# argmaxinc/WhisperKit

Measured on AMD Instinct MI355X. Metric: audio-sec/sec (1/RTF), 30 s chunks: host PCM -> log-mel + encoder + greedy decode -> segments, higher is better.
Workload: dtype f16

## Files before the change

### include/whisperhip.h

```cpp
#ifndef WHISPERHIP_H
#define WHISPERHIP_H

#include <stddef.h>
#include <stdint.h>

#ifdef __cplusplus
extern "C" {
#endif

typedef struct wh_model wh_model;
typedef struct wh_session wh_session;
typedef struct wh_transcription wh_transcription;
typedef struct wh_tokenizer wh_tokenizer;

typedef enum wh_status {
    WH_OK = 0,
    WH_ERR_TOKENIZER_UNAVAILABLE = 1,
    WH_ERR_MODELS_UNAVAILABLE = 2,
    WH_ERR_PREFILL_FAILED = 3,
    WH_ERR_AUDIO_PROCESSING_FAILED = 4,
    WH_ERR_DECODING_LOGITS_FAILED = 5,
    WH_ERR_SEGMENTING_FAILED = 6,
    WH_ERR_LOAD_AUDIO_FAILED = 7,
    WH_ERR_PREPARE_DECODER_INPUTS_FAILED = 8,
// ... 88 lines not shown

typedef struct wh_word_timing {
    int32_t token_offset, n_tokens;
    float start, end, probability;
} wh_word_timing;

typedef struct wh_timings {
    double audio_processing, logmels, encoding, decoding_init, decoding_predictions, decoding_filtering,
        decoding_sampling, decoding_kv_caching, decoding_word_timestamps, decoding_fallback, decoding_windowing,
        decoding_loop, full_pipeline, input_audio_seconds;
    double total_decoding_loops, total_decoding_windows, total_decoding_fallbacks, total_encoding_runs,
        total_logmel_runs;
    double pipeline_start, first_token_time, model_loading, prewarm_load_time, encoder_load_time, decoder_load_time,
        encoder_specialization_time, decoder_specialization_time, tokenizer_load_time, audio_loading, decoding_non_prediction,
        total_audio_processing_runs, total_kv_update_runs, total_timestamp_alignment_runs;
} wh_timings;

const char* wh_last_error(void);
const char* wh_version(void);

int wh_model_create(const void* blob, size_t nbytes, int device, wh_model** out);
int wh_model_load(const char* path, int device, wh_model** out);
void wh_model_destroy(wh_model* m);
int wh_model_dims(const wh_model* m, wh_dims* out);
int wh_model_set_alignment_heads(wh_model* m, const int32_t* layer_head_pairs, int n_pairs);

int wh_mel_count(const wh_model* m);
int wh_window_samples(const wh_model* m);
int wh_embed_size(const wh_model* m);
int wh_logits_size(const wh_model* m);
int wh_kv_cache_embed_dim(const wh_model* m);
int wh_kv_cache_max_sequence_length(const wh_model* m);
int wh_window_size(const wh_model* m);
int wh_is_model_multilingual(const wh_model* m);
int wh_supports_word_timestamps(const wh_model* m);
int wh_special_tokens_default(const wh_model* m, wh_special_tokens* out);
void wh_decoding_options_default(wh_decoding_options* out);

int wh_session_create(wh_model* m, int max_batch , wh_session** out);
void wh_session_destroy(wh_session* s);
int wh_session_max_batch(const wh_session* s);
int wh_session_cross_attention_mode(const wh_session* s);
int wh_xabs_auto_min_slots(void);
int wh_xabs_auto_splits(int max_batch);
int wh_xabs_supports(int n_state, int n_head);
int wh_session_cross_attention_splits(const wh_session* s);
int wh_session_create_with_mode(wh_model* m, int max_batch, int cross_attention_mode, wh_session** out);
int wh_session_create_tuned(wh_model* m, int max_batch, int cross_attention_mode, int cross_attention_splits, wh_session** out);
typedef struct wh_session_options {
    int32_t cross_attention_mode;
    int32_t cross_attention_splits;
    int32_t cross_attention_slots_per_workgroup;
    int32_t encoder_precision;
    int32_t reserved_[3];
    int32_t fallback_compaction;
} wh_session_options;
void wh_session_options_default(wh_session_options* out);
int wh_session_create_with_options(wh_model* m, int max_batch, const wh_session_options* opt, wh_session** out);
int wh_session_cross_attention_slots_per_workgroup(const wh_session* s);
int wh_session_encoder_precision(const wh_session* s);
int wh_debug_peek(wh_session* s, const char* name, void* out_host, size_t nbytes);
long long wh_debug_live_allocations(void);
int wh_session_step_graph_count(const wh_session* s);
int wh_session_synchronize(wh_session* s);
void* wh_session_stream(wh_session* s);

int wh_set_audio(wh_session* s, int b, const float* pcm_host, int n_samples);
int wh_set_audio_device(wh_session* s, int b, const float* pcm_device, int n_samples);

int wh_log_mel_spectrogram(wh_session* s, int batch);
int wh_get_mel(wh_session* s, int b, float* out_host );
int wh_set_mel(wh_session* s, int b, const float* mel_host );

int wh_encode_features(wh_session* s, int batch);
int wh_get_encoder_output(wh_session* s, int b, float* out_host );
int wh_set_encoder_output(wh_session* s, int b, const float* enc_host );

int wh_prepare_decoder_inputs(wh_session* s, int batch);
int wh_reset_decoder_inputs(wh_session* s, int batch);

int wh_predict_logits(wh_session* s, int batch, const int32_t* tokens, const int32_t* positions,
                      float* logits_out_host );
int wh_get_alignment_weights(wh_session* s, int b, float* out_host );

int wh_session_set_alignment_postprocess(wh_session* s, int z_normalize, int median_filter_width);

int wh_session_set_word_alignment(wh_session* s, int mode);
int wh_session_word_alignment(const wh_session* s);
int wh_alignment_paths(wh_session* s, int batch, const int32_t* rows, int32_t* text_idx, int32_t* time_idx, int32_t* lengths,
                       int capacity_per_slot);
int wh_session_word_alignment_stats(const wh_session* s, int64_t* dtw_launches, int64_t* alignment_d2h_bytes);

enum { WH_DTYPE_F32 = 0, WH_DTYPE_F16 = 1 };
typedef struct wh_tensor {
    void* data;
    int32_t dtype;
    int32_t ndim;
    int64_t shape[4];
    int32_t device;
    int32_t reserved_;
} wh_tensor;
int wh_get_mel_tensor(wh_session* s, int b, wh_tensor* out);
int wh_get_encoder_output_tensor(wh_session* s, int b, int dtype, wh_tensor* out);
int wh_get_logits_tensor(wh_session* s, wh_tensor* out);
int wh_get_mel_device(wh_session* s, int b, const float** mel_dev);
int wh_get_encoder_output_device(wh_session* s, int b, const float** enc_f32_dev, const void** enc_f16_dev);
int wh_get_logits_device(wh_session* s, const float** logits_dev);
int wh_session_set_cancel_flag(wh_session* s, const volatile int32_t* flag);

int wh_filter_logits(wh_session* s, const wh_decoding_options* opt, const wh_special_tokens* st,
                     const int32_t* tokens, int n_tokens, int prefilled_index, int initial_prompt_index,
                     int language_filter, float* logits_inout_host, int n_logits);
int wh_sample_token(wh_session* s, const float* logits_host, int n_logits, float temperature, int top_k,
// ... 256 lines not shown
```

### whisperkit_amd/_lib.py

```python
from __future__ import annotations

import ctypes as C
import os

HERE = os.path.dirname(os.path.abspath(__file__))
LIB_PATH = os.environ.get("WHISPERHIP_LIB") or os.path.join(HERE, "libwhisperhip.so")

WH_MAX_RESULT_TOKENS = 232
WINDOW_SAMPLES = 480000
MEL_FRAMES = 3000
AUDIO_CTX = 1500
MAX_TOKEN_CONTEXT = 224


class WhDims(C.Structure):
    _fields_ = [(n, C.c_int32) for n in ("n_mels", "n_audio_ctx", "n_audio_state", "n_audio_head", "n_audio_layer",
                                           "n_vocab", "n_text_ctx", "n_text_state", "n_text_head", "n_text_layer")]


class WhSpecialTokens(C.Structure):
    _fields_ = [(n, C.c_int32) for n in ("end_token", "english_token", "no_speech_token", "no_timestamps_token",
                                           "special_token_begin", "start_of_previous_token", "start_of_transcript_token",
                                           "time_token_begin", "transcribe_token", "translate_token", "whitespace_token",
                                           "language_token_begin", "n_language_tokens")]


class WhDecodingOptions(C.Structure):
    _fields_ = [
        ("task", C.c_int32), ("language_token", C.c_int32), ("temperature", C.c_float),
        ("temperature_increment_on_fallback", C.c_float), ("temperature_fallback_count", C.c_int32),
        ("sample_length", C.c_int32), ("top_k", C.c_int32), ("use_prefill_prompt", C.c_int32),
        ("detect_language", C.c_int32), ("skip_special_tokens", C.c_int32), ("without_timestamps", C.c_int32),
        ("word_timestamps", C.c_int32), ("max_initial_timestamp", C.c_float), ("max_window_seek", C.c_int32),
        ("clip_timestamps", C.POINTER(C.c_float)), ("n_clip_timestamps", C.c_int32), ("window_clip_time", C.c_float),
        ("prompt_tokens", C.POINTER(C.c_int32)), ("n_prompt_tokens", C.c_int32),
        ("prefix_tokens", C.POINTER(C.c_int32)), ("n_prefix_tokens", C.c_int32),
        ("suppress_blank", C.c_int32), ("suppress_tokens", C.POINTER(C.c_int32)), ("n_suppress_tokens", C.c_int32),
        ("compression_ratio_threshold", C.c_float), ("log_prob_threshold", C.c_float),
        ("first_token_log_prob_threshold", C.c_float), ("no_speech_threshold", C.c_float), ("seed", C.c_uint64),
        ("float16_logits", C.c_int32), ("beam_size", C.c_int32), ("beam_patience", C.c_float), ("reserved_", C.c_int32),
    ]


class WhDecodingResult(C.Structure):
    _fields_ = [
        ("n_tokens", C.c_int32), ("tokens", C.c_int32 * WH_MAX_RESULT_TOKENS), ("token_logprobs", C.c_float * WH_MAX_RESULT_TOKENS),
        ("avg_logprob", C.c_float), ("no_speech_prob", C.c_float), ("temperature", C.c_float), ("compression_ratio", C.c_float),
        ("language_token", C.c_int32), ("fallback_reason", C.c_int32), ("needs_fallback", C.c_int32),
        ("is_first_token_logprob_too_low", C.c_int32), ("steps", C.c_int32),
    ]


class WhSessionOptions(C.Structure):
    _fields_ = [("cross_attention_mode", C.c_int32), ("cross_attention_splits", C.c_int32), ("cross_attention_slots_per_workgroup", C.c_int32),
                ("encoder_precision", C.c_int32), ("reserved_", C.c_int32 * 3), ("fallback_compaction", C.c_int32)]


class WhTensor(C.Structure):
    _fields_ = [("data", C.c_void_p), ("dtype", C.c_int32), ("ndim", C.c_int32), ("shape", C.c_int64 * 4), ("device", C.c_int32),
                ("reserved_", C.c_int32)]


class WhSegment(C.Structure):
    _fields_ = [("id", C.c_int32), ("seek", C.c_int32), ("start", C.c_float), ("end", C.c_float),
                ("token_offset", C.c_int32), ("n_tokens", C.c_int32), ("temperature", C.c_float), ("avg_logprob", C.c_float),
                ("compression_ratio", C.c_float), ("no_speech_prob", C.c_float), ("word_offset", C.c_int32), ("n_words", C.c_int32)]


class WhWordTiming(C.Structure):
    _fields_ = [("token_offset", C.c_int32), ("n_tokens", C.c_int32), ("start", C.c_float), ("end", C.c_float), ("probability", C.c_float)]


class WhProgress(C.Structure):
    _fields_ = [("slot", C.c_int32), ("n_tokens", C.c_int32), ("tokens", C.POINTER(C.c_int32)), ("avg_logprob", C.c_float),
                ("compression_ratio", C.c_float), ("text", C.c_char_p)]


PROGRESS_FN = C.CFUNCTYPE(C.c_int, C.c_void_p, C.POINTER(WhProgress))
WINDOW_PRE_FN = C.CFUNCTYPE(None, C.c_void_p, C.c_int, C.POINTER(C.c_float), C.c_int, C.c_int)
WINDOW_POST_FN = C.CFUNCTYPE(C.c_int, C.c_void_p, C.c_int, C.c_int, C.c_int, C.c_void_p, C.c_int, C.c_int)
SEGMENT_DISCOVERY_FN = C.CFUNCTYPE(None, C.c_void_p, C.c_int, C.c_void_p, C.c_int, C.c_int)


class WhWindowHooks(C.Structure):
    _fields_ = [("window_preprocess", WINDOW_PRE_FN), ("window_postprocess", WINDOW_POST_FN), ("segment_discovery", SEGMENT_DISCOVERY_FN),
                ("user", C.c_void_p)]
LOGITS_FILTER_FN = C.CFUNCTYPE(None, C.c_void_p, C.POINTER(C.c_float), C.c_int32, C.POINTER(C.c_int32), C.c_int32)
TOKEN_SAMPLER_FN = C.CFUNCTYPE(C.c_int32, C.c_void_p, C.POINTER(C.c_float), C.c_int32, C.POINTER(C.c_int32), C.POINTER(C.c_float), C.c_int32,
                               C.POINTER(C.c_int32), C.POINTER(C.c_float))


class WhChunkRecord(C.Structure):
    _fields_ = [("tokens", C.c_int32 * 232), ("n_tokens", C.c_int32), ("chunk_index", C.c_int32), ("seek", C.c_int32), ("steps", C.c_int32),
                ("avg_logprob", C.c_float), ("temperature", C.c_float), ("compression_ratio", C.c_float), ("no_speech_prob", C.c_float)]


COMM_RCCL, COMM_TCP, COMM_ID_BYTES = 0, 1, 128


class WhTimings(C.Structure):
    _fields_ = [(n, C.c_double) for n in (
        "audio_processing", "logmels", "encoding", "decoding_init", "decoding_predictions", "decoding_filtering",
        "decoding_sampling", "decoding_kv_caching", "decoding_word_timestamps", "decoding_fallback", "decoding_windowing",
        "decoding_loop", "full_pipeline", "input_audio_seconds", "total_decoding_loops", "total_decoding_windows",
        "total_decoding_fallbacks", "total_encoding_runs", "total_logmel_runs",
        "pipeline_start", "first_token_time", "model_loading", "prewarm_load_time", "encoder_load_time", "decoder_load_time",
        "encoder_specialization_time", "decoder_specialization_time", "tokenizer_load_time", "audio_loading",
        "decoding_non_prediction", "total_audio_processing_runs", "total_kv_update_runs", "total_timestamp_alignment_runs")]


VP, I, F, U64 = C.c_void_p, C.c_int, C.c_float, C.c_uint64
PF, PI32, PU8 = C.POINTER(C.c_float), C.POINTER(C.c_int32), C.POINTER(C.c_uint8)
PVP = C.POINTER(C.c_void_p)
POPT, PST = C.POINTER(WhDecodingOptions), C.POINTER(WhSpecialTokens)
SYMBOLS = {
    "wh_last_error": (C.c_char_p, []),
    "wh_version": (C.c_char_p, []),
    "wh_model_create": (I, [VP, C.c_size_t, I, PVP]),
    "wh_model_load": (I, [C.c_char_p, I, PVP]),
    "wh_model_destroy": (None, [VP]),
    "wh_model_dims": (I, [VP, C.POINTER(WhDims)]),
    "wh_model_set_alignment_heads": (I, [VP, PI32, I]),
    "wh_mel_count": (I, [VP]), "wh_window_samples": (I, [VP]), "wh_embed_size": (I, [VP]), "wh_logits_size": (I, [VP]),
    "wh_kv_cache_embed_dim": (I, [VP]), "wh_kv_cache_max_sequence_length": (I, [VP]), "wh_window_size": (I, [VP]),
    "wh_is_model_multilingual": (I, [VP]), "wh_supports_word_timestamps": (I, [VP]),
    "wh_special_tokens_default": (I, [VP, PST]),
    "wh_decoding_options_default": (None, [POPT]),
    "wh_session_create": (I, [VP, I, PVP]),
    "wh_session_destroy": (None, [VP]),
    "wh_session_max_batch": (I, [VP]),
    "wh_session_cross_attention_mode": (I, [VP]),
    "wh_session_cross_attention_splits": (I, [VP]),
    "wh_xabs_auto_min_slots": (I, []),
    "wh_xabs_auto_splits": (I, [I]),
    "wh_xabs_supports": (I, [I, I]),
    "wh_session_step_graph_count": (I, [VP]),
    "wh_session_set_window_hooks": (I, [VP, C.POINTER(WhWindowHooks)]),
    "wh_transcription_set_segment_times": (I, [VP, I, F, F]),
    "wh_session_create_with_mode": (I, [VP, I, I, PVP]),
    "wh_session_create_tuned": (I, [VP, I, I, I, PVP]),
    "wh_session_options_default": (None, [C.POINTER(WhSessionOptions)]),
    "wh_session_create_with_options": (I, [VP, I, C.POINTER(WhSessionOptions), PVP]),
    "wh_session_cross_attention_slots_per_workgroup": (I, [VP]),
    "wh_session_encoder_precision": (I, [VP]),
    "wh_debug_peek": (I, [VP, C.c_char_p, VP, C.c_size_t]),
    "wh_debug_live_allocations": (C.c_longlong, []),
    "wh_session_synchronize": (I, [VP]),
    "wh_session_stream": (VP, [VP]),
    "wh_set_audio": (I, [VP, I, VP, I]),
    "wh_set_audio_device": (I, [VP, I, VP, I]),
    "wh_log_mel_spectrogram": (I, [VP, I]),
    "wh_get_mel": (I, [VP, I, VP]),
    "wh_set_mel": (I, [VP, I, VP]),
    "wh_encode_features": (I, [VP, I]),
    "wh_get_encoder_output": (I, [VP, I, VP]),
    "wh_set_encoder_output": (I, [VP, I, VP]),
    "wh_prepare_decoder_inputs": (I, [VP, I]),
    "wh_reset_decoder_inputs": (I, [VP, I]),
    "wh_predict_logits": (I, [VP, I, PI32, PI32, VP]),
    "wh_get_alignment_weights": (I, [VP, I, VP]),
    "wh_filter_logits": (I, [VP, POPT, PST, PI32, I, I, I, I, VP, I]),
    "wh_sample_token": (I, [VP, VP, I, F, I, U64, I, PI32, PF]),
    "wh_decode_text": (I, [VP, I, POPT, PST, PI32, I, PF, PI32, U64, C.POINTER(WhDecodingResult)]),
    "wh_decode_text_languages": (I, [VP, I, POPT, PST, PI32, I, PI32, PF, PI32, U64, C.POINTER(WhDecodingResult)]),
    "wh_decode_text_custom": (I, [VP, POPT, PST, PI32, I, F, U64, C.POINTER(LOGITS_FILTER_FN), PVP, I, TOKEN_SAMPLER_FN, VP,
                                  C.POINTER(WhDecodingResult)]),
    "wh_detect_language": (I, [VP, I, PST, PI32, PF]),
    "wh_decode_text_beam": (I, [VP, I, I, F, POPT, PST, PI32, I, PI32, C.POINTER(WhDecodingResult)]),
    "wh_beam_sampler_create": (I, [I, C.c_int32, F, PVP]),
    "wh_beam_sampler_destroy": (None, [VP]),
    "wh_beam_sampler_reset": (None, [VP]),
    "wh_beam_sampler_max_candidates": (I, [VP]),
    "wh_beam_sampler_finished_count": (I, [VP]),
    "wh_beam_sampler_update": (I, [VP, I, I, PI32, PF, PF, PF, PI32, I, PI32, PF, PF, PI32, PI32, PI32]),
    "wh_beam_sampler_finalize": (I, [VP, I, I, PI32, PF, PF, I, I, PI32, PF, PI32, PF, PI32]),
    "wh_get_mel_device": (I, [VP, I, PVP]),
    "wh_get_mel_tensor": (I, [VP, I, C.POINTER(WhTensor)]),
    "wh_get_encoder_output_tensor": (I, [VP, I, I, C.POINTER(WhTensor)]),
    "wh_get_logits_tensor": (I, [VP, C.POINTER(WhTensor)]),
    "wh_get_encoder_output_device": (I, [VP, I, PVP, PVP]),
    "wh_get_logits_device": (I, [VP, PVP]),
    "wh_session_set_cancel_flag": (I, [VP, VP]),
    "wh_session_set_alignment_postprocess": (I, [VP, I, I]),
    "wh_session_set_fallback_compaction": (I, [VP, I]),
# ... 136 lines not shown
```

### whisperkit_amd/api.py

```python
from __future__ import annotations

import ctypes as C
import dataclasses
import math
import weakref
from typing import List, Optional, Sequence, Tuple, Union

import numpy as np

from . import _lib as L
from .weights import MODEL_DIMS, WhisperDims, pack_blob, synthetic_state_dict


class WhisperError(RuntimeError):

    def __init__(self, code: int, message: str):
        super().__init__(f"[wh_status {code}] {message}")
        self.code = code


def _check(code: int):
    if code != 0:
        raise WhisperError(code, L.load().wh_last_error().decode())

# ... 342 lines not shown
        if blob is None:
            blob = pack_blob(dims, state_dict, alignment_heads=alignment_heads)
        self.handle = C.c_void_p()
        arr = np.frombuffer(blob, dtype=np.uint8)
        _check(self.lib.wh_model_create(C.c_void_p(arr.ctypes.data), arr.nbytes, device, C.byref(self.handle)))
        st = L.WhSpecialTokens()
        _check(self.lib.wh_special_tokens_default(self.handle, C.byref(st)))
        self.specialTokens = st

    @classmethod
    def from_pretrained(cls, src: str, device: int = 0):
        from .checkpoint import load_checkpoint
        dims, sd, heads = load_checkpoint(src)
        return cls(dims, sd, device=device, alignment_heads=heads)

    @classmethod
    def synthetic(cls, name: str, seed: int = 0, device: int = 0, **kw):
        dims = MODEL_DIMS[name]
        return cls(dims, synthetic_state_dict(dims, seed=seed, **kw), device=device)

    melCount = property(lambda s: s.lib.wh_mel_count(s.handle))
    windowSamples = property(lambda s: s.lib.wh_window_samples(s.handle))
    embedSize = property(lambda s: s.lib.wh_embed_size(s.handle))
    logitsSize = property(lambda s: s.lib.wh_logits_size(s.handle))
    kvCacheEmbedDim = property(lambda s: s.lib.wh_kv_cache_embed_dim(s.handle))
    kvCacheMaxSequenceLength = property(lambda s: s.lib.wh_kv_cache_max_sequence_length(s.handle))
    windowSize = property(lambda s: s.lib.wh_window_size(s.handle))
    isModelMultilingual = property(lambda s: bool(s.lib.wh_is_model_multilingual(s.handle)))
    supportsWordTimestamps = property(lambda s: bool(s.lib.wh_supports_word_timestamps(s.handle)))

    def setAlignmentHeads(self, pairs):
        a = np.ascontiguousarray(np.array(list(pairs), dtype=np.int32).reshape(-1))
        _check(self.lib.wh_model_set_alignment_heads(self.handle, a.ctypes.data_as(L.PI32), len(a) // 2))

    def close(self):
        if self.handle:
            self.lib.wh_model_destroy(self.handle)
            self.handle = C.c_void_p()

    def __del__(self):
        try:
            self.close()
        except Exception:
            pass


def xabsSupports(nState: int, nHead: int) -> bool:
    return bool(L.load().wh_xabs_supports(int(nState), int(nHead)))


class Session:

    ENCODER_PRECISIONS = {None: 0, "f16": 0, "split": 1}

    def __init__(self, model: Model, maxBatch: int = 1, crossAttentionMode: Optional[int] = None, crossAttentionSplits: Optional[int] = None,
                 crossAttentionSlotsPerWorkgroup: Optional[int] = None, encoderPrecision: Optional[str] = None):
        self.model, self.lib, self.B = model, model.lib, maxBatch
        self.handle = C.c_void_p()
        if encoderPrecision not in self.ENCODER_PRECISIONS:
            raise ValueError(f"encoderPrecision {encoderPrecision!r}: expected None, 'f16' or 'split'")
        if crossAttentionSlotsPerWorkgroup is not None or encoderPrecision is not None:
            o = L.WhSessionOptions()
            self.lib.wh_session_options_default(C.byref(o))
            o.cross_attention_mode = -1 if crossAttentionMode is None else int(crossAttentionMode)
            o.cross_attention_splits = 0 if crossAttentionSplits is None else int(crossAttentionSplits)
            o.cross_attention_slots_per_workgroup = int(crossAttentionSlotsPerWorkgroup or 0)
            o.encoder_precision = self.ENCODER_PRECISIONS[encoderPrecision]
            _check(self.lib.wh_session_create_with_options(model.handle, maxBatch, C.byref(o), C.byref(self.handle)))
        elif crossAttentionMode is None and crossAttentionSplits is None:
            _check(self.lib.wh_session_create(model.handle, maxBatch, C.byref(self.handle)))
        else:
            _check(self.lib.wh_session_create_tuned(model.handle, maxBatch, -1 if crossAttentionMode is None else int(crossAttentionMode),
                                                    int(crossAttentionSplits or 0), C.byref(self.handle)))

    @staticmethod
    def xabsAutoMinSlots() -> int:
        return int(L.load().wh_xabs_auto_min_slots())

    @staticmethod
    def xabsAutoSplits(maxBatch: int) -> int:
        return int(L.load().wh_xabs_auto_splits(int(maxBatch)))

    @staticmethod
    def xabsSupports(nState: int, nHead: int) -> bool:
        return xabsSupports(nState, nHead)

    @property
    def crossAttentionSlotsPerWorkgroup(self) -> int:
        return int(self.lib.wh_session_cross_attention_slots_per_workgroup(self.handle))

    @property
    def encoderPrecision(self) -> str:
        return {0: "f16", 1: "split"}[int(self.lib.wh_session_encoder_precision(self.handle))]

    @property
    def crossAttentionMode(self) -> int:
        return int(self.lib.wh_session_cross_attention_mode(self.handle))

    @property
    def crossAttentionSplits(self) -> int:
        return int(self.lib.wh_session_cross_attention_splits(self.handle))

    @property
    def stepGraphCount(self) -> int:
        return int(self.lib.wh_session_step_graph_count(self.handle))

    def close(self):
        if self.handle:
            self.lib.wh_session_destroy(self.handle)
            self.handle = C.c_void_p()

    def __del__(self):
        try:
            self.close()
        except Exception:
            pass

    def synchronize(self):
        _check(self.lib.wh_session_synchronize(self.handle))

    def _stash(self, exc: BaseException):
        if getattr(self, "_callback_error", None) is None:
            self._callback_error = exc

    def _raise_pending(self):
        exc, self._callback_error = getattr(self, "_callback_error", None), None
        if exc is not None:
            raise exc

    def _guarded(self, fn, *args) -> int:
        self._callback_error = None
        rc = fn(*args)
        self._raise_pending()
        _check(rc)
        return rc

    def setTokenizer(self, tokenizer: Optional["Tokenizer"]):
        self.tokenizer = tokenizer
        _check(self.lib.wh_session_set_tokenizer(self.handle, tokenizer.handle if tokenizer is not None else None))

    def setProgressCallback(self, callback):
        if callback is None:
            self._progress = None
            _check(self.lib.wh_session_set_progress_callback(self.handle, L.PROGRESS_FN(0), None))
            return

# ... 896 lines not shown
```

### whisperkit_amd/csrc/capi.hip

```cpp
#include <math.h>
#include <stdarg.h>
#include <stdio.h>
#include <string.h>

#include <algorithm>
#include <cstdlib>

#include "internal.h"
#include "knobs.h"

using namespace wh;

namespace wh { thread_local KernelProfiler* g_prof = nullptr; unsigned long long* debug_buffer(); }

namespace whi {
static thread_local char g_err[512] = "";
int set_error(int code, const char* fmt, ...) {
    va_list ap;
    va_start(ap, fmt);
    vsnprintf(g_err, sizeof(g_err), fmt, ap);
    va_end(ap);
    return code;
}
}
// ... 325 lines not shown
    o->end_token = eot; o->english_token = lang0; o->no_speech_token = translate + 4; o->no_timestamps_token = translate + 5;
    o->special_token_begin = eot; o->start_of_previous_token = translate + 3; o->start_of_transcript_token = sot;
    o->time_token_begin = translate + 6; o->transcribe_token = translate + 1; o->translate_token = translate; o->whitespace_token = 220;
    o->language_token_begin = lang0; o->n_language_tokens = nlang;
    return WH_OK;
}

extern "C" void wh_decoding_options_default(wh_decoding_options* o) {
    if (!o) return;
    memset(o, 0, sizeof(*o));
    o->task = 0; o->language_token = -1; o->temperature = 0.0f; o->temperature_increment_on_fallback = 0.2f;
    o->temperature_fallback_count = 5; o->sample_length = WH_MAX_TOKEN_CONTEXT; o->top_k = 5; o->use_prefill_prompt = 1;
    o->detect_language = -1; o->skip_special_tokens = 0; o->without_timestamps = 0; o->word_timestamps = 0;
    o->max_initial_timestamp = NAN; o->max_window_seek = -1; o->clip_timestamps = nullptr; o->n_clip_timestamps = 0;
    o->window_clip_time = 1.0f; o->prompt_tokens = nullptr; o->n_prompt_tokens = 0; o->prefix_tokens = nullptr; o->n_prefix_tokens = 0;
    o->suppress_blank = 0; o->suppress_tokens = nullptr; o->n_suppress_tokens = 0;
    o->compression_ratio_threshold = 2.4f; o->log_prob_threshold = -1.0f; o->first_token_log_prob_threshold = -1.5f;
    o->no_speech_threshold = 0.6f; o->seed = 0; o->float16_logits = 0; o->beam_size = 0; o->beam_patience = 1.0f;
}

#define DALLOC(ptr, n) WH_HIP(s->mem.alloc(&(ptr), (size_t)(n), true))

static int session_create_impl(wh_model* m, int max_batch, int cross_attention_mode, int cross_attention_splits, int slots_per_workgroup, wh_session** out,
                               int encoder_precision = 0);
extern "C" int wh_session_create(wh_model* m, int max_batch, wh_session** out) { return session_create_impl(m, max_batch, -1, 0, 0, out); }
extern "C" int wh_session_create_tuned(wh_model* m, int max_batch, int cross_attention_mode, int cross_attention_splits, wh_session** out) {
    wh_session_options o{};
    o.cross_attention_mode = cross_attention_mode; o.cross_attention_splits = cross_attention_splits;
    return wh_session_create_with_options(m, max_batch, &o, out);
}
extern "C" void wh_session_options_default(wh_session_options* o) {
    if (!o) return;
    memset(o, 0, sizeof(*o));
    o->cross_attention_mode = -1;
}
extern "C" int wh_session_create_with_options(wh_model* m, int max_batch, const wh_session_options* opt, wh_session** out) {
    wh_session_options dflt;
    wh_session_options_default(&dflt);
    if (!opt) opt = &dflt;
    const int cross_attention_mode = opt->cross_attention_mode, cross_attention_splits = opt->cross_attention_splits;
    if (opt->cross_attention_slots_per_workgroup < 0 || opt->cross_attention_slots_per_workgroup > kXabsMaxSlotsPerWorkgroup)
        return set_error(WH_ERR_INVALID_ARGUMENT, "wh_session_create: cross_attention_slots_per_workgroup %d (expected 0 auto, 1 .. %d)", opt->cross_attention_slots_per_workgroup, kXabsMaxSlotsPerWorkgroup);
    if (cross_attention_mode < -1 || cross_attention_mode > 1)
        return set_error(WH_ERR_INVALID_ARGUMENT, "wh_session_create: cross_attention_mode %d (expected -1 auto, 0 K / V rows, 1 absorbed)", cross_attention_mode);
    if (cross_attention_splits < 0 || cross_attention_splits > kXabsSplits)
        return set_error(WH_ERR_INVALID_ARGUMENT, "wh_session_create: cross_attention_splits %d (expected 0 auto, 1 .. %d)", cross_attention_splits, kXabsSplits);
    if (opt->encoder_precision < 0 || opt->encoder_precision > 1)
        return set_error(WH_ERR_INVALID_ARGUMENT, "wh_session_create: encoder_precision %d (expected 0 Float16 operands, 1 split hi | lo)", opt->encoder_precision);
    if (opt->encoder_precision == 1 && cross_attention_mode == 1)
        return set_error(WH_ERR_INVALID_ARGUMENT, "wh_session_create: encoder_precision 1 (split) needs the K / V-row cross-attention (cross_attention_mode -1 or 0): "
                         "the absorbed kernel streams the Float16 encoder output, and a hi | lo stream would double its bytes");
    if (opt->fallback_compaction < 0 || opt->fallback_compaction > 1)
        return set_error(WH_ERR_INVALID_ARGUMENT, "wh_session_create: fallback_compaction %d (expected 0 off, 1 on)", opt->fallback_compaction);
    if (cross_attention_mode == 1 && m && !xabs_supported(m->dims.n_text_state, m->dims.n_text_head))
        return set_error(WH_ERR_INVALID_ARGUMENT, "wh_session_create: the absorbed cross-attention needs a model width of 384 / 512 / 768 / 1024 / 1280 (this model: %d)", m->dims.n_text_state);
    const int r = session_create_impl(m, max_batch, opt->encoder_precision == 1 ? 0 : cross_attention_mode, cross_attention_splits,
                                      opt->cross_attention_slots_per_workgroup, out, opt->encoder_precision);
    if (r == WH_OK) (*out)->fallback_compaction = opt->fallback_compaction;
    return r;
}
extern "C" int wh_session_create_with_mode(wh_model* m, int max_batch, int cross_attention_mode, wh_session** out) {
    return wh_session_create_tuned(m, max_batch, cross_attention_mode, 0, out);
}

static hipError_t create_session_stream(hipStream_t* st) {
    static std::atomic<int> counter{0};
    const int parts = knob::now<knob::WH_CU_PARTS>();
    if (const char* pr = knob::text<knob::WH_STREAM_PRIORITIES>()) {
        int p[8], n = 0;
        for (const char* c = pr; *c && n < 8;) { p[n++] = atoi(c); while (*c && *c != ',') ++c; if (*c == ',') ++c; }
        if (n > 0) return hipStreamCreateWithPriority(st, hipStreamNonBlocking, p[counter.fetch_add(1) % n]);
    }
    if (parts < 2) return hipStreamCreateWithFlags(st, hipStreamNonBlocking);
    int dev = 0, n_cu = 256;
    (void)hipGetDevice(&dev);
    (void)hipDeviceGetAttribute(&n_cu, hipDeviceAttributeMultiprocessorCount, dev);
    const int extra = knob::now<knob::WH_CU_PART_EXTRA>(), k = counter.fetch_add(1) % parts, w = n_cu / parts;
    uint32_t mask[16] = {};
    for (int i = k * w; i < k * w + w + extra; ++i) { const int c = ((i % n_cu) + n_cu) % n_cu; mask[c >> 5] |= 1u << (c & 31); }
    return hipExtStreamCreateWithCUMask(st, (uint32_t)((n_cu + 31) / 32), mask);
}
static int session_build(wh_session* s, wh_model* m, int max_batch, int cross_attention_mode, int cross_attention_splits, int slots_per_workgroup, int encoder_precision) {
    s->B = max_batch;
    const wh_dims& D = m->dims;
    const size_t B = max_batch, d = D.n_audio_state, L = D.n_text_layer, V = D.n_vocab, H = D.n_text_head;
    if (create_session_stream(&s->st) != hipSuccess) return set_error(WH_ERR_HIP, "hipStreamCreate failed");
    s->m = m;
    m->n_sessions.fetch_add(1);
    DALLOC(s->pcm, B * kWindowSamples); DALLOC(s->n_valid, B);
    DALLOC(s->logspec, B * D.n_mels * kFrames); DALLOC(s->maxkey, B);
    DALLOC(s->mel_t, B * kFramesPad * D.n_mels); DALLOC(s->mel_f32, B * D.n_mels * kFrames);
    DALLOC(s->h1, B * kFramesPad * d); DALLOC(s->x, B * kCtx * d); DALLOC(s->xn, B * kCtx * d);
    DALLOC(s->q16, B * kCtx * d); DALLOC(s->k16, B * kCtx * d); DALLOC(s->vt16, B * d * kCtxPad); DALLOC(s->att16, B * kCtx * d);
    DALLOC(s->hmlp, B * kCtx * 4 * d); DALLOC(s->enc16, B * kCtx * d); DALLOC(s->enc32, B * kCtx * d);
    s->encoder_precision = encoder_precision;
    if (encoder_precision == 1) {
        DALLOC(s->mel_t_lo, B * kFramesPad * D.n_mels); DALLOC(s->h1_lo, B * kFramesPad * d); DALLOC(s->xn_lo, B * kCtx * d);
        DALLOC(s->att_lo, B * kCtx * d); DALLOC(s->hmlp_lo, B * kCtx * 4 * d); DALLOC(s->enc_lo, B * kCtx * d);
    }
    {
        const int xabs_mode = knob::now<knob::WH_XABS>();
        if (cross_attention_mode >= 0) s->use_xabs = cross_attention_mode != 0 && xabs_supported((int)d, (int)H);
        else {
            s->use_xabs = xabs_auto_width((int)d, (int)H) && (xabs_mode < 0 ? max_batch >= wh_xabs_auto_min_slots() : xabs_mode != 0);
        }
        if (s->use_xabs) { const int r_ = build_xabs(m); if (r_) return r_; }
    }
    if (s->use_xabs) {
        Xabs probe{};
        const size_t bytes = mem::carve_session_xabs(nullptr, d, H, B, probe);
        char* blob = nullptr;
// ... 2 lines not shown
        s->xabs.layers_host = m->xabs.data();
        s->xabs.n_split = cross_attention_splits > 0 ? cross_attention_splits : xabs_splits(max_batch);
        s->xabs.spw = slots_per_workgroup > 0 ? slots_per_workgroup : 1;
        if (const int v = knob::now<knob::WH_XABS_SPW>()) s->xabs.spw = v;
    } else {
        DALLOC(s->cross_k_hi, L * B * kCtx * d); DALLOC(s->cross_v_hi, L * B * kCtx * d);
        DALLOC(s->cross_k_lo, L * B * kCtx * d); DALLOC(s->cross_v_lo, L * B * kCtx * d);
    }
    DALLOC(s->self_k, L * B * kMaxTok * d); DALLOC(s->self_v, L * B * kMaxTok * d);
    DALLOC(s->part, B * H * kMaxSplit * kPartStride); DALLOC(s->ticket, B * H);
    DALLOC(s->logits, B * V);
    DALLOC(s->align_mean, B * kMaxTok * kCtx);
    DALLOC(s->seq, B); DALLOC(s->cfg_dev, kMaxOptionClasses); DALLOC(s->suppress_dev, kMaxOptionClasses * kMaxSuppress); DALLOC(s->sup_mask_dev, kMaxOptionClasses * (size_t)plan::option_mask_stride((int)V)); DALLOC(s->stats, B * kStatBlocks * 8);
    DALLOC(s->tok_out_dev, B); DALLOC(s->lp_out_dev, B); DALLOC(s->scratch_logits, V);
    {
        Dec32& q = s->d32;
        Dec32 probe{};
        const size_t bytes = mem::carve_session_d32(nullptr, d, B, probe);
        char* blob = nullptr;
        if (s->mem.alloc(&blob, bytes, true) != hipSuccess) return set_error(WH_ERR_HIP, "hipMalloc(%zu) for the decode-step buffers failed", bytes);
        mem::carve_session_d32(blob, d, B, q);
        q.layers_host = m->dec32.data(); q.emb_t = m->emb_t; q.lg_g = m->lg_g; q.lg_c = m->lg_c; q.n_bt = (int)((B + 31) / 32);
        q.part_floats = kD32PartFloats;
    }
    if (s->mem.alloc_pinned(&s->seq_host, B) != hipSuccess) return set_error(WH_ERR_HIP, "hipHostMalloc failed");
    for (auto& e : s->ev) hipEventCreate(&e);
    (void)wh::debug_buffer();
    if (hipDeviceSynchronize() != hipSuccess) return set_error(WH_ERR_HIP, "hipDeviceSynchronize failed after session allocation");
    return WH_OK;
}
static int session_create_impl(wh_model* m, int max_batch, int cross_attention_mode, int cross_attention_splits, int slots_per_workgroup, wh_session** out,
                               int encoder_precision) {
    if (!m || !out) return set_error(WH_ERR_MODELS_UNAVAILABLE, "wh_session_create: model is null");
    if (max_batch < 1 || max_batch > kMaxSessionSlots) return set_error(WH_ERR_INVALID_ARGUMENT, "max_batch %d out of range [1, %d]", max_batch, kMaxSessionSlots);
    WH_HIP(hipSetDevice(m->device));
    wh_session* s = new wh_session();
    const int r = session_build(s, m, max_batch, cross_attention_mode, cross_attention_splits, slots_per_workgroup, encoder_precision);
    if (r) { wh_session_destroy(s); return r; }
    *out = s;
    return WH_OK;
}

extern "C" void wh_session_destroy(wh_session* s) {
    if (!s) return;
    if (s->m) s->m->n_sessions.fetch_sub(1);
    if (s->st) hipStreamSynchronize(s->st);
    whi::drop_session_graphs(s);
    for (auto& e : s->ev) if (e) hipEventDestroy(e);
    if (s->st) hipStreamDestroy(s->st);
    delete s;
}
extern "C" int wh_session_max_batch(const wh_session* s) { return s ? s->B : -1; }
extern "C" int wh_session_cross_attention_mode(const wh_session* s) { return s ? (s->use_xabs ? 1 : 0) : -1; }
extern "C" int wh_session_encoder_precision(const wh_session* s) { return s ? s->encoder_precision : -1; }
extern "C" int wh_session_step_graph_count(const wh_session* s) { return s ? (int)s->graphs.size() : -1; }
extern "C" int wh_session_cross_attention_splits(const wh_session* s) { return s ? (s->use_xabs ? s->xabs.n_split : 0) : -1; }
extern "C" int wh_session_cross_attention_slots_per_workgroup(const wh_session* s) { return s ? (s->use_xabs ? s->xabs.spw : 0) : -1; }
extern "C" int wh_xabs_auto_splits(int max_batch) { return wh::xabs_auto_splits(max_batch); }
extern "C" int wh_xabs_supports(int n_state, int n_head) { return wh::xabs_supported(n_state, n_head) ? 1 : 0; }
extern "C" int wh_xabs_auto_min_slots(void) { return knob::now<knob::WH_XABS_MIN_SLOTS>(); }
static_assert(knob::kTable[knob::WH_XABS_MIN_SLOTS].dflt == wh::kXabsAutoMinSlots && knob::kTable[knob::WH_XABS_SPW].hi == wh::kXabsMaxSlotsPerWorkgroup &&
              knob::kTable[knob::WH_XABS_SPLITS].hi == wh::kXabsSplits, "knobs.h: the ranges of the absorbed cross-attention knobs");
extern "C" int wh_debug_peek(wh_session* s, const char* name, void* out, size_t nbytes) {
    CHECK_SESSION(s);
    if (!name || !out) return set_error(WH_ERR_INVALID_ARGUMENT, "wh_debug_peek: null argument");
    const std::string n(name);
    const void* src = nullptr;
    size_t have = 0;
    const size_t R = (size_t)s->d32.n_bt * 32, d = (size_t)s->m->dims.n_text_state, H = (size_t)s->m->dims.n_text_head, B = (size_t)s->B;
    const size_t nht = H > 16 ? 2 : 1;
    if (n == "x") { src = s->d32.x; have = R * d * 4; } else if (n == "q") { src = s->d32.q; have = R * d * 4; }
    else if (n == "za_hi") { src = s->d32.za_hi; have = R * d * 2; } else if (n == "za_lo") { src = s->d32.za_lo; have = R * d * 2; }
    else if (n == "zb_hi") { src = s->d32.zb_hi; have = R * d * 2; } else if (n == "zb_lo") { src = s->d32.zb_lo; have = R * d * 2; }
    else if (s->use_xabs && n == "qf_hi") { src = s->xabs.qf_hi; have = B * nht * 16 * d * 2; }
    else if (s->use_xabs && n == "qf_lo") { src = s->xabs.qf_lo; have = B * nht * 16 * d * 2; }
    else if (s->use_xabs && n == "part") { src = s->xabs.part; have = (size_t)kXabsSplits * H * d * B * 4; }
    else if (s->use_xabs && n == "ml") { src = s->xabs.ml; have = (size_t)kXabsSplits * H * B * 8; }
    else if (n == "enc16") { src = s->enc16; have = B * kCtx * d * 2; }
    else if (s->enc_lo && n == "enc_lo") { src = s->enc_lo; have = B * kCtx * (size_t)s->m->dims.n_audio_state * 2; }
    if (!src) return set_error(WH_ERR_INVALID_ARGUMENT, "wh_debug_peek: no buffer named '%s' in this session", name);
    if (nbytes > have) return set_error(WH_ERR_INVALID_ARGUMENT, "wh_debug_peek: '%s' holds %zu bytes, %zu requested", name, have, nbytes);
    WH_HIP(hipStreamSynchronize(s->st));
    WH_HIP(hipMemcpy(out, src, nbytes, hipMemcpyDeviceToHost));
    return WH_OK;
}
extern "C" long long wh_debug_live_allocations(void) { return wh::mem::g_live.load(std::memory_order_relaxed); }
extern "C" int wh_session_synchronize(wh_session* s) {
    if (!s) return set_error(WH_ERR_INVALID_ARGUMENT, "session is null");
    WH_HIP(hipStreamSynchronize(s->st));
    return WH_OK;
}
extern "C" void* wh_session_stream(wh_session* s) { return s ? (void*)s->st : nullptr; }


static int set_audio_common(wh_session* s, int b, const float* pcm, int n, hipMemcpyKind kind) {
    CHECK_SESSION(s); CHECK_SLOT(s, b);
    if (n < 0 || (!pcm && n > 0)) return set_error(WH_ERR_AUDIO_PROCESSING_FAILED, "wh_set_audio: invalid buffer (n=%d)", n);
    int m = std::min(n, kWindowSamples);
    float* dst = s->pcm + (size_t)b * kWindowSamples;
    if (m > 0) WH_HIP(hipMemcpyAsync(dst, pcm, sizeof(float) * m, kind, s->st));
    if (m < kWindowSamples) WH_HIP(hipMemsetAsync(dst + m, 0, sizeof(float) * (kWindowSamples - m), s->st));
    WH_HIP(hipMemcpyAsync(s->n_valid + b, &m, sizeof(int), hipMemcpyHostToDevice, s->st));
    WH_HIP(hipStreamSynchronize(s->st));
    return WH_OK;
}
extern "C" int wh_set_audio(wh_session* s, int b, const float* pcm_host, int n) { return set_audio_common(s, b, pcm_host, n, hipMemcpyHostToDevice); }
// ... 98 lines not shown
        g = GemmArgs{};
        g.A = s->att16; g.W = w.o_w; g.bias = w.o_b; g.M = M; g.N = d; g.K = d; g.lda = d; g.a_rows_per_batch = M; g.ldc = d; g.out32 = s->x;
        g.prof_kind = KK_ENC_O;
        launch_gemm(EPI_RESID_F32, g, st);
        launch_layernorm(s->x, w.ln2_g, w.ln2_b, M, d, s->xn, nullptr, st);
        g = GemmArgs{};
        g.A = s->xn; g.W = w.fc1_w; g.bias = w.fc1_b; g.M = M; g.N = 4 * d; g.K = d; g.lda = d; g.a_rows_per_batch = M; g.ldc = 4 * d; g.out16 = s->hmlp;
        g.prof_kind = KK_ENC_FC1;
        launch_gemm(EPI_GELU_F16, g, st);
        g = GemmArgs{};
        g.A = s->hmlp; g.W = w.fc2_w; g.bias = w.fc2_b; g.M = M; g.N = d; g.K = 4 * d; g.lda = 4 * d; g.a_rows_per_batch = M; g.ldc = d; g.out32 = s->x;
        g.prof_kind = KK_ENC_FC2;
        launch_gemm(EPI_RESID_F32, g, st);
    }
    launch_layernorm(s->x, m->lnp_g, m->lnp_b, M, d, s->enc16, s->enc32, st);
    WH_CHECK_LAUNCH();
    return WH_OK;
}
extern "C" int wh_get_encoder_output(wh_session* s, int b, float* out) {
    CHECK_SESSION(s); CHECK_SLOT(s, b);
    if (!out) return set_error(WH_ERR_INVALID_ARGUMENT, "wh_get_encoder_output: null output");
    size_t n = (size_t)kCtx * s->m->dims.n_audio_state;
    WH_HIP(hipMemcpyAsync(out, s->enc32 + b * n, n * 4, hipMemcpyDeviceToHost, s->st));
    WH_HIP(hipStreamSynchronize(s->st));
    return WH_OK;
}
extern "C" int wh_set_encoder_output(wh_session* s, int b, const float* enc) {
    CHECK_SESSION(s); CHECK_SLOT(s, b);
    if (!enc) return set_error(WH_ERR_INVALID_ARGUMENT, "wh_set_encoder_output: null input");
    size_t n = (size_t)kCtx * s->m->dims.n_audio_state;
    WH_HIP(hipMemcpyAsync(s->enc32 + b * n, enc, n * 4, hipMemcpyHostToDevice, s->st));
    if (s->enc_lo) launch_f32_to_f16_split(s->enc32 + b * n, s->enc16 + b * n, s->enc_lo + b * n, n, s->st);
    else launch_f32_to_f16(s->enc32 + b * n, s->enc16 + b * n, n, s->st);
    WH_CHECK_LAUNCH();
    WH_HIP(hipStreamSynchronize(s->st));
    return WH_OK;
}

constexpr bool kXattnGateDefault = false;
namespace whi {
DecodeBuffers decode_buffers(wh_session* s, int batch, int max_position) {
    const wh_model* m = s->m;
    DecodeBuffers db{};
    db.cross_div = 1;
    db.self_rows = std::min(std::max(max_position, 0), kMaxTok - 1) + 1;
    db.self_owner = nullptr;
    db.batch = batch; db.max_batch = s->B; db.d = m->dims.n_text_state; db.n_head = m->dims.n_text_head; db.n_layer = m->dims.n_text_layer; db.n_vocab = m->dims.n_vocab;
    db.emb = m->emb; db.pos = m->dec_pos; db.layers_host = m->dec.data(); db.lnf_g = m->lnf_g; db.lnf_b = m->lnf_b;
    db.self_k = s->self_k; db.self_v = s->self_v; db.cross_k_hi = s->cross_k_hi; db.cross_v_hi = s->cross_v_hi; db.cross_k_lo = s->cross_k_lo; db.cross_v_lo = s->cross_v_lo;
    db.part = s->part; db.ticket = s->ticket; db.logits = s->logits; db.seq = s->seq;
    db.mixed = s->pass_mixed ? 1 : 0; db.stats = s->stats; db.sup_mask = s->sup_mask_dev; db.fused_greedy = s->fused_greedy ? 1 : 0;
    db.align = s->align_enabled ? s->align : nullptr; db.align_slot = m->align_slot_dev; db.n_align = s->n_align_alloc;
    db.d32 = &s->d32; db.x = s->d32.x; db.q = s->d32.q;
    if (s->use_xabs) { s->xabs.enc = s->enc16; db.xabs = &s->xabs; }
    if (s->pass_mapped) {
        db.slot_home = s->slot_home_dev;
        if (s->use_xabs) { s->xabs_pass = s->xabs; s->xabs_pass.spw = s->pass_spw; db.xabs = &s->xabs_pass; }
    }
    if (s->pass_owner) { db.self_owner = s->inpass_dev + s->B; db.owner_slots = s->B; }
    const int gate_mode = knob::once<knob::WH_XATT_GATE>();
    const bool gate_on = gate_mode < 0 ? kXattnGateDefault && m->n_sessions.load() > 1 : gate_mode != 0;
    db.xattn_gate = gate_on ? m->xattn_gate : nullptr;
    return db;
}
}

namespace whi {
int ensure_align(wh_session* s) {
    if (s->align && s->n_align_alloc != s->m->n_align) {
        WH_HIP(hipStreamSynchronize(s->st));
        drop_session_graphs(s);
        s->mem.release(s->align);
        s->align = nullptr;
        s->n_align_alloc = 0;
    }
    if (!s->align && s->m->n_align > 0) {
        size_t n = (size_t)s->B * kMaxTok * s->m->n_align * kCtx;
        WH_HIP(s->mem.alloc(&s->align, n, false));
        WH_HIP(hipMemsetAsync(s->align, 0, n * sizeof(float), s->st));
        s->n_align_alloc = s->m->n_align;
    }
    return WH_OK;
}

int reset_decoder_inputs_masked(wh_session* s, int batch, const int32_t* active) {
    for (int b = 0; b < batch; ++b) {
        if (active && !active[b]) continue;
        WH_HIP(hipMemsetAsync(s->seq + b, 0, sizeof(SeqState), s->st));
        if (s->align) WH_HIP(hipMemsetAsync(s->align + (size_t)b * kMaxTok * s->n_align_alloc * kCtx, 0, (size_t)kMaxTok * s->n_align_alloc * kCtx * sizeof(float), s->st));
    }
    return WH_OK;
}
}
using whi::ensure_align;

extern "C" int wh_reset_decoder_inputs(wh_session* s, int batch) {
    CHECK_SESSION(s); CHECK_BATCH(s, batch);
    return whi::reset_decoder_inputs_masked(s, batch, nullptr);
}

extern "C" int wh_prepare_decoder_inputs(wh_session* s, int batch) {
    CHECK_SESSION(s); CHECK_BATCH(s, batch);
    const wh_model* m = s->m;
    const int d = m->dims.n_text_state, L = m->dims.n_text_layer;
    if (!s->use_xabs) {
        GemmArgs g{};
// ... 370 lines not shown
```

### whisperkit_amd/csrc/decoder.hip

```cpp
#include <algorithm>
#include <cstdlib>

#include "dec_shared.h"
#include "knobs.h"

namespace wh {

__device__ __forceinline__ void compute_filter_rules(const SamplerCfg& cfg, const SeqState* sq, int n_tok, int V, int* r, int last_ts_hint = -2) {
    const int tb = cfg.time_token_begin;
    int blank = 0, ts_active = 0, r1lo = 0, r1hi = 0, r2lo = 0, r2hi = 0;
    blank = cfg.suppress_blank && (n_tok == cfg.prefilled_index);
    if (cfg.timestamp_rules) {
        int sb = -1;
        if (cfg.is_multilingual) {
            for (int i = 0; i < 3 && i < n_tok; ++i)
                if (sq->tokens[i] == cfg.transcribe_token || sq->tokens[i] == cfg.translate_token) { sb = max(i + 1, cfg.initial_prompt_index); break; }
        } else sb = cfg.initial_prompt_index;
        if (sb >= 0 && sb <= n_tok) {
            ts_active = 1;
            if (n_tok > sb) {
                int cnt = n_tok - sb;
                bool lastTs = sq->tokens[n_tok - 1] >= tb;
                bool penTs = cnt < 2 || sq->tokens[n_tok - 2] >= tb;
                if (lastTs) {
// ... 658 lines not shown
    const int nofence = knob::once<knob::WH_XATT_NOFENCE>();
    AttnArgs at = at_in;
    at.no_fence = nofence;
    ProfScope ps_(KK_DEC_CROSS_ATTN, st);
    const dim3 grid(S, H, B);
    const int gate_lead = knob::once<knob::WH_XATT_GATE_LEAD>();
    at.gate_wg = std::max(0, S * H * B - 1 - gate_lead);
    const int xlds = knob::once<knob::WH_XATT_LDS>();
    const int nt = knob::once<knob::WH_XATT_NT>();
    const bool ntl = nt && at.cross_div <= 1;
#define XATT(P_) do { if (at.mapped) { if (nt) dec_cross_attn_kernel<P_, true, true><<<grid, 256, xlds, st>>>(at); else dec_cross_attn_kernel<P_, false, true><<<grid, 256, xlds, st>>>(at); } \
                      else if (ntl) dec_cross_attn_kernel<P_, true><<<grid, 256, xlds, st>>>(at); else dec_cross_attn_kernel<P_, false><<<grid, 256, xlds, st>>>(at); } while (0)
    if (S == 6) XATT(8);
    else if (S == 8) XATT(6);
    else if (S == 12) XATT(4);
    else XATT(2);
#undef XATT
}

void launch_decoder_step(const DecodeBuffers& db, const SamplerCfg* cfg_dev, const int* suppress_dev, bool sample, hipStream_t st) {
    const Dec32& D = *db.d32;
    const int d = db.d, B = db.batch, H = db.n_head, L = db.n_layer, V = db.n_vocab;
    const int n_bt = (B + 31) / 32;
    const size_t self_stride = (size_t)db.max_batch * H * kMaxTok * kHeadDim;
    const size_t cross_stride = (size_t)db.max_batch * H * kCtx * kHeadDim;
    const int S = plan::cross_attn_plan(H, knob::once<knob::WH_XATT_PASSES>(), kCtx).splits;
    launch_dec32_embed(db.emb, db.pos, db.seq, B, d, V, n_bt, D.x, db.layers_host[0].ln1_g, D.za_hi, D.za_lo, D.stat, st);
    P32Args base{};
    base.batch = B; base.d = d; base.n_head = H; base.n_vocab = V; base.seq = db.seq; base.part = D.part; base.ticket = D.ticket;
    base.x = D.x; base.stat_in = D.stat; base.n_stat = d / 32;
    for (int l = 0; l < L; ++l) {
        const DecLayerW& w = db.layers_host[l];
        const Dec32LayerW& t = D.layers_host[l];
        P32Args a = base;
        a.N = 3 * d; a.K = d; a.Wt = t.qkv_t; a.zhi = D.za_hi; a.zlo = D.za_lo; a.fold_g = t.qkv_g; a.fold_c = t.qkv_c; a.q = D.q;
        a.self_k = db.self_k + (size_t)l * self_stride; a.self_v = db.self_v + (size_t)l * self_stride; a.prof_kind = KK_DEC_QKV;
        launch_dec32_proj(P32_QKV, a, n_bt, st);
        AttnArgs at{};
        at.batch = B; at.d = d; at.n_head = H; at.layer = l; at.n_layer = L; at.n_split = S; at.q = D.q; at.cross_div = db.cross_div;
        at.self_k = a.self_k; at.self_v = a.self_v;
        at.cross_k_hi = db.cross_k_hi + (size_t)l * cross_stride; at.cross_k_lo = db.cross_k_lo + (size_t)l * cross_stride;
        at.cross_v_hi = db.cross_v_hi + (size_t)l * cross_stride; at.cross_v_lo = db.cross_v_lo + (size_t)l * cross_stride;
        at.att_hi = D.zb_hi; at.att_lo = D.zb_lo; at.part = db.part; at.ticket = db.ticket; at.seq = db.seq;
        at.align = db.align; at.align_slot = db.align_slot; at.n_align = db.n_align; at.gate = db.xattn_gate;
        at.self_rows = db.self_rows; at.self_owner = db.self_owner;
        if (db.self_owner && db.owner_slots > B) {
            AttnArgs sa = at;
            sa.batch = db.owner_slots;
            launch_self_attn(sa, H, B, st);
        } else launch_self_attn(at, H, B, st);
        a = base;
        a.N = d; a.K = d; a.Wt = t.o_t; a.zhi = D.zb_hi; a.zlo = D.zb_lo; a.bias = w.o_b; a.gamma_next = w.ln2_g;
        a.zhi_out = D.za_hi; a.zlo_out = D.za_lo; a.stat_out = D.stat; a.prof_kind = KK_DEC_OPROJ;
        launch_dec32_proj(P32_RESID, a, n_bt, st);
        a = base;
        a.N = d; a.K = d; a.Wt = t.cq_t; a.zhi = D.za_hi; a.zlo = D.za_lo; a.fold_g = t.cq_g; a.fold_c = t.cq_c; a.q = D.q; a.prof_kind = KK_DEC_CQ;
        a.gate = db.xabs ? nullptr : db.xattn_gate;
        launch_dec32_proj(P32_Q, a, n_bt, st);
        if (db.xabs) {
            const Xabs& X = *db.xabs;
            XabsArgs xa{};
            xa.batch = B; xa.max_batch = db.max_batch; xa.d = d; xa.n_head = H; xa.layer = l; xa.n_split = X.n_split; xa.cross_div = db.cross_div;
            xa.enc = X.enc; xa.q = D.q; xa.wkT = X.layers_host[l].wkT; xa.wv_t = X.layers_host[l].wv_t; xa.bv = X.layers_host[l].bv;
            xa.qf_hi = X.qf_hi; xa.qf_lo = X.qf_lo; xa.part = X.part; xa.ml = X.ml; xa.att_hi = D.zb_hi; xa.att_lo = D.zb_lo;
            xa.align = db.align; xa.align_slot = db.align_slot; xa.n_align = db.n_align; xa.seq = db.seq; xa.kpart = D.part; xa.ticket = D.ticket;
            xa.gate = db.xattn_gate;
            xa.spw = X.spw;
            xa.dbg = debug_buffer() ? debug_buffer() + (size_t)KK_DEC_CROSS_ATTN * 4096 * 8 : nullptr;
            if (db.slot_home) { xa.mapped = 1; xa.slot_home = db.slot_home; }
            launch_xabs_qk(xa, n_bt, st);
            launch_xabs_attn(xa, st);
            launch_xabs_vup(xa, n_bt, st);
        } else {
            at.dbg = debug_buffer() ? debug_buffer() + (size_t)KK_DEC_CROSS_ATTN * 4096 * 8 : nullptr;
            if (db.slot_home) { at.mapped = 1; at.slot_home = db.slot_home; }
            launch_cross_attn(at, S, H, B, st);
        }
        a = base;
        a.N = d; a.K = d; a.Wt = t.co_t; a.zhi = D.zb_hi; a.zlo = D.zb_lo; a.bias = w.co_b; a.gamma_next = w.ln3_g;
        a.zhi_out = D.za_hi; a.zlo_out = D.za_lo; a.stat_out = D.stat; a.prof_kind = KK_DEC_COPROJ;
        launch_dec32_proj(P32_RESID, a, n_bt, st);
        a = base;
        a.N = 4 * d; a.K = d; a.Wt = t.fc1_t; a.zhi = D.za_hi; a.zlo = D.za_lo; a.fold_g = t.fc1_g; a.fold_c = t.fc1_c; a.h_out = D.h; a.h_out_lo = D.h_lo; a.prof_kind = KK_DEC_FC1;
        launch_dec32_proj(P32_FC1, a, n_bt, st);
        a = base;
        a.N = d; a.K = 4 * d; a.Wt = t.fc2_t; a.zhi = D.h; a.zlo = D.h_lo; a.bias = w.fc2_b;
        a.gamma_next = (l + 1 < L) ? db.layers_host[l + 1].ln1_g : db.lnf_g;
        a.zhi_out = D.za_hi; a.zlo_out = D.za_lo; a.stat_out = D.stat; a.prof_kind = KK_DEC_FC2;
        launch_dec32_proj(P32_RESID, a, n_bt, st);
    }
    const bool fused = sample && db.fused_greedy;
    P32Args a = base;
    a.N = V; a.K = d; a.Wt = D.emb_t; a.zhi = D.za_hi; a.zlo = D.za_lo; a.fold_g = D.lg_g; a.fold_c = D.lg_c;
    a.logits = fused ? nullptr : db.logits; a.prof_kind = KK_DEC_LOGITS;
    if (sample) a.cfg = cfg_dev;
    if (fused) { a.stats = db.stats; a.sup_mask = db.sup_mask; }
    const bool mixed = sample && db.mixed;
    launch_dec32_proj(P32_LOGITS, a, n_bt, st, mixed && fused);
    if (fused) {
        ProfScope ps_(KK_SAMPLER, st);
        if (mixed) sampler_final_mixed_kernel<<<B, 256, 0, st>>>(cfg_dev, db.seq, db.stats, (V + 31) / 32);
        else sampler_final_kernel<<<B, 256, 0, st>>>(cfg_dev, db.seq, db.stats, (V + 31) / 32);
    } else if (sample) {
        ProfScope ps_(KK_SAMPLER, st);
        if (mixed) sampler_kernel<1, 1, 2, 0><<<B, SAMP_T, 0, st>>>(cfg_dev, suppress_dev, db.seq, db.logits, 0, nullptr, nullptr);
        else sampler_kernel<1, 1, 1, 0><<<B, SAMP_T, 0, st>>>(cfg_dev, suppress_dev, db.seq, db.logits, 0, nullptr, nullptr);
    }
}

void launch_filter_only(const SamplerCfg* cfg_dev, const int* suppress_dev, SeqState* seq, float* logits, int n_vocab, hipStream_t st) {
    sampler_kernel<1, 0, 0, 1><<<1, SAMP_T, 0, st>>>(cfg_dev, suppress_dev, seq, logits, 0, nullptr, nullptr);
}
void launch_sample_only(const SamplerCfg* cfg_dev, SeqState* seq, float* logits, int n_vocab, int counter, int* token_out, float* logprob_out, hipStream_t st) {
    sampler_kernel<0, 1, 0, 0><<<1, SAMP_T, 0, st>>>(cfg_dev, nullptr, seq, logits, counter, token_out, logprob_out);
}


void launch_beam_filter_topk(const SamplerCfg* cfg_dev, const int* suppress_dev, SeqState* seq, float* logits, int batch, int K, float* lp_out,
                             int* tok_out, hipStream_t st) {
    sampler_kernel<1, 0, 0, 0, 1><<<batch, SAMP_T, 0, st>>>(cfg_dev, suppress_dev, seq, logits, K, tok_out, lp_out);
}

void launch_filter_sample(const SamplerCfg* cfg_dev, const int* suppress_dev, SeqState* seq, float* logits, int batch, int* token_out, float* logprob_out, hipStream_t st) {
    sampler_kernel<1, 1, 0, 0><<<batch, SAMP_T, 0, st>>>(cfg_dev, suppress_dev, seq, logits, 0, token_out, logprob_out);
}

__global__ __launch_bounds__(256) void alignment_mean_kernel(const float* __restrict__ align, int n_align, float* __restrict__ out) {
    __shared__ float acc[4][kCtx];
    const size_t row = blockIdx.x;
    const int lane = threadIdx.x & 63, wave = threadIdx.x >> 6;
    const float* src = align + row * n_align * kCtx;
    for (int t = lane; t < kCtx; t += 64) acc[wave][t] = 0.0f;
    for (int j = wave; j < n_align; j += 4) {
        const float* sp = src + (size_t)j * kCtx;
        float v[24];
        float mx = -INFINITY, amax = 0.0f;
#pragma unroll
        for (int i = 0; i < 24; ++i) {
            int t = lane + 64 * i;
            v[i] = t < kCtx ? sp[t] : -INFINITY;
            mx = fmaxf(mx, v[i]);
            if (t < kCtx) amax = fmaxf(amax, fabsf(v[i]));
// ... 115 lines not shown
```

### whisperkit_amd/csrc/decoder32.hip

```cpp
#include "dec_shared.h"
#include "knobs.h"

namespace wh {

typedef unsigned u32x4 __attribute__((ext_vector_type(4)));

__global__ void d32_tile_weights_kernel(const f16* __restrict__ W, int N, int K, u32x4* __restrict__ out, size_t n_out) {
    const size_t o = (size_t)blockIdx.x * blockDim.x + threadIdx.x;
    if (o >= n_out) return;
    const int KT = K >> 4;
    const int lane = (int)(o & 63);
    const size_t tile = o >> 6;
    const int kt = (int)(tile % KT), rt = (int)(tile / KT);
    const int row = rt * 32 + (lane & 31), k = kt * 16 + 8 * (lane >> 5);
    u32x4 v = {0, 0, 0, 0};
    if (row < N) v = *reinterpret_cast<const u32x4*>(W + (size_t)row * K + k);
    out[o] = v;
}
void dec32_tile_weights(const f16* W, int N, int K, f16* out, hipStream_t st) {
    const size_t n_out = (size_t)((N + 31) / 32) * (K / 16) * 64;
    d32_tile_weights_kernel<<<(unsigned)((n_out + 255) / 256), 256, 0, st>>>(W, N, K, reinterpret_cast<u32x4*>(out), n_out);
}

__global__ __launch_bounds__(256) void d32_fold_kernel(const f16* __restrict__ W, int N, int K, const float* __restrict__ gamma,
                                                       const float* __restrict__ beta, const float* __restrict__ bias,
                                                       float* __restrict__ g, float* __restrict__ c) {
    const int lane = threadIdx.x & 63, row = blockIdx.x * 4 + (threadIdx.x >> 6);
    if (row >= N) return;
    double sg = 0.0, sc = 0.0;
    for (int k = lane; k < K; k += 64) {
        const double w = (double)(float)W[(size_t)row * K + k];
        sg += w * (double)gamma[k];
        sc += w * (double)beta[k];
    }
#pragma unroll
    for (int o = 32; o > 0; o >>= 1) { sg += __shfl_xor(sg, o, 64); sc += __shfl_xor(sc, o, 64); }
    if (lane == 0) { g[row] = (float)sg; c[row] = (float)(sc + (bias ? (double)bias[row] : 0.0)); }
}
void dec32_fold_vectors(const f16* W, int N, int K, const float* gamma, const float* beta, const float* bias, float* g, float* c, hipStream_t st) {
    d32_fold_kernel<<<(N + 3) / 4, 256, 0, st>>>(W, N, K, gamma, beta, bias, g, c);
}

__device__ __forceinline__ void d32_resid_tail(const float (&xn)[4], bool valid, int bt, int rt, int n_rt, int n, int j, int gb, int tid,
                                               int d, float* x, const float* gamma_next, f16* zhi, f16* zlo, float2* stat_out,
                                               float (*xs)[33]) {
    const float4 gm = *reinterpret_cast<const float4*>(gamma_next + n);
    if (valid) {
        *reinterpret_cast<float4*>(x + (size_t)gb * d + n) = float4{xn[0], xn[1], xn[2], xn[3]};
        const float z[4] = {gm.x * xn[0], gm.y * xn[1], gm.z * xn[2], gm.w * xn[3]};
        f16x4 hi, lo;
#pragma unroll
        for (int i = 0; i < 4; ++i) { f16 h_, l_; split_hilo(z[i], h_, l_); hi[i] = h_; lo[i] = l_; }
        const size_t o = plane_index(gb, n, d);
        *reinterpret_cast<f16x4*>(zhi + o) = hi;
        *reinterpret_cast<f16x4*>(zlo + o) = lo;
    }
    const int nl = n & 31;
#pragma unroll
    for (int i = 0; i < 4; ++i) xs[nl + i][j] = xn[i];
    __syncthreads();
    if (tid < 32) {
        float s = 0.0f;
#pragma unroll
        for (int r = 0; r < 32; ++r) s += xs[r][tid];
        const float mean = s * (1.0f / 32.0f);
        float m2 = 0.0f;
#pragma unroll
        for (int r = 0; r < 32; ++r) { const float e = xs[r][tid] - mean; m2 = fmaf(e, e, m2); }
        stat_out[((size_t)bt * n_rt + rt) * 32 + tid] = float2{mean, m2};
    }
}

template <int K>
__device__ __forceinline__ void chan32_k(float& cm, float& cM2, float mb, float M2b) {
    constexpr float w = 1.0f / (float)(K + 1), w2 = 32.0f * (float)K / (float)(K + 1);
    const float delta = mb - cm;
    cm = fmaf(delta, w, cm);
    cM2 += fmaf(delta * delta, w2, M2b);
}
__device__ __forceinline__ void chan_merge(float& cn, float& cm, float& cM2, float nb, float mb, float M2b) {
    if (nb == 0.0f) return;
    const float nn = cn + nb, rn = __frcp_rn(nn);
    const float delta = mb - cm;
    cm = fmaf(delta, nb * rn, cm);
    cM2 += fmaf(delta * delta, cn * nb * rn, M2b);
    cn = nn;
}

template <int MODE, bool HILO, int TC, bool NTW, int RT>
__global__ __launch_bounds__(256, 2) void dec32_proj_kernel(const P32Args a) {
    constexpr bool kMix = MODE == P32_LOGITS_MIXED, kLogits = MODE == P32_LOGITS || kMix;
    constexpr bool kLN = MODE == P32_QKV || MODE == P32_Q || MODE == P32_FC1 || kLogits;
    constexpr int kXs = kLogits ? 256 * 6 : 32 * 33;
    __shared__ float red[RT][4][16][64];
    __shared__ float st_l[8][32][3];
    __shared__ float xs_raw[kXs];
    __shared__ int last_flag;
    const int tid = threadIdx.x, lane = tid & 63, wave = tid >> 6;
    const int n_rt = (a.N + 31) >> 5;
    const int n_rtp = (n_rt + RT - 1) / RT;
    const int grp8 = blockIdx.x / (8 * a.n_bt), in8 = blockIdx.x % (8 * a.n_bt);
    const int xw = grp8 * 8 + (in8 & 7), bt = in8 >> 3;
    if (xw >= n_rtp * a.ks) return;
    const int rt0 = (xw % n_rtp) * RT, ksi = xw / n_rtp;
    const int n_mine = min(RT, n_rt - rt0);
    const int KT = a.K >> 4;
    const int kt0 = (ksi * 4 + wave) * a.tw;
    const u32x4* wp[RT];
#pragma unroll
    for (int t = 0; t < RT; ++t) wp[t] = reinterpret_cast<const u32x4*>(a.Wt) + ((size_t)min(rt0 + t, n_rt - 1) * KT + kt0) * 64 + lane;
    const size_t zoff = ((size_t)bt * KT + kt0) * 64 + lane;
    const u32x4* hp = reinterpret_cast<const u32x4*>(a.zhi) + zoff;
    const u32x4* lp = HILO ? reinterpret_cast<const u32x4*>(a.zlo) + zoff : nullptr;
    const int j = tid & 31, sub = tid >> 5;
    const int gb = bt * 32 + j;
    const bool valid = gb < a.batch;
    const int xw_dbg = xw;

#define D32_STAMP(i) do { if (a.dbg && tid == 0 && bt == 0) a.dbg[(size_t)(xw_dbg & 4095) * 8 + (i)] = wall_clock64(); } while (0)
    D32_STAMP(0);
    float2 sp[5] = {};
    if constexpr (kLN) {
#pragma unroll
        for (int i = 0; i < 5; ++i) {
            const int idx = min(sub + 8 * i, a.n_stat - 1);
            sp[i] = a.stat_in[((size_t)bt * a.n_stat + idx) * 32 + j];
        }
    }
    constexpr bool kLateOperands = RT >= 4;
    constexpr int NB = RT >= 4 ? 3 : 2;
    float4 e0[RT], e1[RT];
    int pos_l = 0, live_l = 0;
    auto load_operands = [&]() {
#pragma unroll
        for (int t = 0; t < RT; ++t) {
            const int n = min(rt0 + t, n_rt - 1) * 32 + 4 * sub;
            if constexpr (kLN) {
                e0[t] = *reinterpret_cast<const float4*>(a.fold_g + n);
                e1[t] = *reinterpret_cast<const float4*>(a.fold_c + n);
            } else {
                e0[t] = *reinterpret_cast<const float4*>(a.bias + n);
                e1[t] = *reinterpret_cast<const float4*>(a.x + (size_t)gb * a.d + n);
            }
        }
    };
    if constexpr (!kLateOperands) load_operands();
    if (valid) { live_l = slot_live(a.seq + gb); if constexpr (MODE == P32_QKV) pos_l = a.seq[gb].token_index; }
    int rules[6] = {0, 0, 0, 0, 0, 0};
    unsigned masked4[RT];
    int tb = 0, ws_tok = 0, eot_tok = 0, nots_tok = 0, r16 = 0;
#pragma unroll
    for (int t = 0; t < RT; ++t) masked4[t] = 0xffffffffu;
    if constexpr (kLogits) {
        if (a.cfg) r16 = a.cfg->f16_logits;
        if (a.stats) {
            if (valid) {
#pragma unroll
                for (int i = 0; i < 6; ++i) rules[i] = a.seq[gb].f_rules[i];
            }
            const unsigned char* sup_mask = a.sup_mask;
            if constexpr (kMix) { if (valid) sup_mask += (size_t)seq_class(a.seq[gb].rng_lane) * plan::option_mask_stride(a.N); }
#pragma unroll
            for (int t = 0; t < RT; ++t) {
                const int n = min(rt0 + t, n_rt - 1) * 32 + 4 * sub;
                if (n + 3 < a.N) masked4[t] = *reinterpret_cast<const unsigned*>(sup_mask + n);
                else {
                    masked4[t] = 0;
#pragma unroll
                    for (int i = 0; i < 4; ++i) masked4[t] |= (unsigned)(n + i < a.N ? sup_mask[n + i] : 1) << (8 * i);
                }
            }
            tb = a.cfg->time_token_begin; ws_tok = a.cfg->whitespace_token; eot_tok = a.cfg->end_token; nots_tok = a.cfg->no_timestamps_token;
        }
    }

    f32x16 acc_h[RT], acc_l[RT];
#pragma unroll
    for (int t = 0; t < RT; ++t)
#pragma unroll
        for (int r = 0; r < 16; ++r) { acc_h[t][r] = 0.0f; acc_l[t][r] = 0.0f; }
    auto stats_to_lds = [&]() {
        if constexpr (kLN) {
            float cm = sp[0].x, cM2 = sp[0].y;
            const int mine = sub < a.n_stat ? (a.n_stat - sub + 7) >> 3 : 0;
            if (mine > 1) chan32_k<1>(cm, cM2, sp[1].x, sp[1].y);
            if (mine > 2) chan32_k<2>(cm, cM2, sp[2].x, sp[2].y);
            if (mine > 3) chan32_k<3>(cm, cM2, sp[3].x, sp[3].y);
            if (mine > 4) chan32_k<4>(cm, cM2, sp[4].x, sp[4].y);
            st_l[sub][j][0] = 32.0f * (float)mine; st_l[sub][j][1] = cm; st_l[sub][j][2] = cM2;
        }
    };
    {
        u32x4 w_[NB][RT][TC], h_[NB][TC], l_[NB][HILO ? TC : 1];
        auto ld = [&](u32x4 (&w)[RT][TC], u32x4 (&h)[TC], u32x4 (&l)[HILO ? TC : 1], int c) {
#pragma unroll
            for (int t = 0; t < RT; ++t)
#pragma unroll
                for (int i = 0; i < TC; ++i) w[t][i] = NTW ? __builtin_nontemporal_load(wp[t] + (size_t)(c * TC + i) * 64) : wp[t][(size_t)(c * TC + i) * 64];
#pragma unroll
            for (int i = 0; i < TC; ++i) h[i] = hp[(size_t)(c * TC + i) * 64];
            if constexpr (HILO) {
#pragma unroll
                for (int i = 0; i < TC; ++i) l[i] = lp[(size_t)(c * TC + i) * 64];
            }
        };
        auto mm = [&](const u32x4 (&w)[RT][TC], const u32x4 (&h)[TC], const u32x4 (&l)[HILO ? TC : 1]) {
#pragma unroll
            for (int i = 0; i < TC; ++i) {
#pragma unroll
                for (int t = 0; t < RT; ++t) {
                    const f16x8 wf = __builtin_bit_cast(f16x8, w[t][i]);
                    acc_h[t] = __builtin_amdgcn_mfma_f32_32x32x16_f16(wf, __builtin_bit_cast(f16x8, h[i]), acc_h[t], 0, 0, 0);
                    if constexpr (HILO) acc_l[t] = __builtin_amdgcn_mfma_f32_32x32x16_f16(wf, __builtin_bit_cast(f16x8, l[i]), acc_l[t], 0, 0, 0);
                }
            }
        };
        const int nch = a.tw / TC;
#pragma unroll
        for (int u = 0; u + 1 < NB; ++u)
            if (u < nch) ld(w_[u], h_[u], l_[u], u);
        D32_STAMP(1);
#pragma unroll 1
        for (int c = 0; c < nch; c += NB) {
#pragma unroll
            for (int u = 0; u < NB; ++u) {
                constexpr int kAhead = NB - 1;
                if (c + u + kAhead < nch) ld(w_[(u + kAhead) % NB], h_[(u + kAhead) % NB], l_[(u + kAhead) % NB], c + u + kAhead);
                __builtin_amdgcn_sched_barrier(0);
                if (c + u < nch) mm(w_[u], h_[u], l_[u]);
                if (u == 0 && c == 0) D32_STAMP(2);
            }
        }
    }
    if constexpr (kLateOperands) load_operands();
    stats_to_lds();
    D32_STAMP(3);
#pragma unroll
    for (int t = 0; t < RT; ++t)
#pragma unroll
        for (int r = 0; r < 16; ++r) red[t][wave][r][lane] = HILO ? fmaf(acc_l[t][r], 1.0f / 2048.0f, acc_h[t][r]) : acc_h[t][r];
    __syncthreads();
    D32_STAMP(4);
    float v[RT][4];
#pragma unroll
    for (int t = 0; t < RT; ++t)
#pragma unroll
        for (int i = 0; i < 4; ++i) v[t][i] = ((red[t][0][4 * wave + i][lane] + red[t][1][4 * wave + i][lane]) + red[t][2][4 * wave + i][lane]) + red[t][3][4 * wave + i][lane];

    if (a.ks > 1) {
        float* base = a.part + (((size_t)bt * n_rt + rt0) * a.ks) * 1024 + tid * 4;
#pragma unroll
        for (int t = 0; t < RT; ++t) {
            if (t < n_mine) {
                const f32x4 pv4 = {v[t][0], v[t][1], v[t][2], v[t][3]};
                float* mine = base + ((size_t)t * a.ks + ksi) * 1024;
                asm volatile("global_store_dwordx4 %0, %1, off sc1\n\ts_nop 1" ::"v"(mine), "v"(pv4) : "memory");
            }
        }
        asm volatile("s_waitcnt vmcnt(0)" ::: "memory");
        __syncthreads();
        if (tid == 0) {
            int* cnt = a.ticket + bt * n_rt + rt0;
            const int t = __hip_atomic_fetch_add(cnt, 1, __ATOMIC_RELAXED, __HIP_MEMORY_SCOPE_AGENT);
            const int last = (t == a.ks - 1);
            if (last) __hip_atomic_store(cnt, 0, __ATOMIC_RELAXED, __HIP_MEMORY_SCOPE_AGENT);
            last_flag = last;
        }
        __syncthreads();
        if (!last_flag) {
            if constexpr (MODE == P32_Q) { if (a.gate && blockIdx.x == 0 && tid == 0) xattn_gate_acquire(a.gate); }
            return;
        }
        float pv[RT][8][4];
#pragma unroll
        for (int t = 0; t < RT; ++t)
#pragma unroll
            for (int s = 0; s < 8; ++s) {
                const float* p = base + ((size_t)(t < n_mine ? t : 0) * a.ks + (s < a.ks ? s : 0)) * 1024;
#pragma unroll
                for (int i = 0; i < 4; ++i) pv[t][s][i] = __hip_atomic_load(p + i, __ATOMIC_RELAXED, __HIP_MEMORY_SCOPE_AGENT);
            }
#pragma unroll
        for (int t = 0; t < RT; ++t)
#pragma unroll
            for (int i = 0; i < 4; ++i) {
                float x_ = pv[t][0][i];
#pragma unroll
                for (int s = 1; s < 8; ++s) x_ += (s < a.ks) ? pv[t][s][i] : 0.0f;
                v[t][i] = x_;
            }
    }

    D32_STAMP(5);
    float mu = 0.0f, rstd = 0.0f;
    if constexpr (kLN) {
        float cn = 0.0f, cm = 0.0f, cM2 = 0.0f;
#pragma unroll
        for (int s = 0; s < 8; ++s) chan_merge(cn, cm, cM2, st_l[s][j][0], st_l[s][j][1], st_l[s][j][2]);
        mu = cm; rstd = rsqrtf(cM2 / (float)a.d + 1e-5f);
    }
#pragma unroll
  for (int t = 0; t < RT; ++t) {
    if (t >= n_mine) break;
    if constexpr (MODE == P32_RESID || kLogits) { if (t > 0) __syncthreads(); }
    const int rt = rt0 + t, n = rt * 32 + 4 * sub;
    float y[4];
    if constexpr (kLN) {
        const float g4[4] = {e0[t].x, e0[t].y, e0[t].z, e0[t].w}, c4[4] = {e1[t].x, e1[t].y, e1[t].z, e1[t].w};
#pragma unroll
        for (int i = 0; i < 4; ++i) y[i] = fmaf(rstd, v[t][i] - mu * g4[i], c4[i]);
    }
    if constexpr (MODE == P32_QKV) {
        if (valid && live_l) {
            const int d = a.d;
            if (n < d) *reinterpret_cast<float4*>(a.q + (size_t)gb * d + n) = float4{y[0], y[1], y[2], y[3]};
            else {
                int c = n - d;
                f16* dst = a.self_k;
                if (c >= d) { c -= d; dst = a.self_v; }
                const int pos = min(max(pos_l, 0), kMaxTok - 1);
                *reinterpret_cast<f16x4*>(dst + (((size_t)gb * a.n_head + (c >> 6)) * kMaxTok + pos) * kHeadDim + (c & 63)) =
                    f16x4{(f16)y[0], (f16)y[1], (f16)y[2], (f16)y[3]};
            }
        }
    } else if constexpr (MODE == P32_Q) {
        if (valid && live_l) *reinterpret_cast<float4*>(a.q + (size_t)gb * a.d + n) = float4{y[0], y[1], y[2], y[3]};
    } else if constexpr (MODE == P32_FC1) {
        if (valid) {
            f16x4 hi, lo;
#pragma unroll
            for (int i = 0; i < 4; ++i) { f16 h_, l_; split_hilo(gelu_erf(y[i]), h_, l_); hi[i] = h_; lo[i] = l_; }
            const size_t o = plane_index(gb, n, a.N);
            *reinterpret_cast<f16x4*>(a.h_out + o) = hi;
            *reinterpret_cast<f16x4*>(a.h_out_lo + o) = lo;
        }
    } else if constexpr (MODE == P32_RESID) {
        const float b4[4] = {e0[t].x, e0[t].y, e0[t].z, e0[t].w}, x4[4] = {e1[t].x, e1[t].y, e1[t].z, e1[t].w};
        float xn[4];
#pragma unroll
        for (int i = 0; i < 4; ++i) xn[i] = x4[i] + (v[t][i] + b4[i]);
        d32_resid_tail(xn, valid && live_l, bt, rt, n_rt, n, j, gb, tid, a.d, a.x, a.gamma_next, a.zhi_out, a.zlo_out, a.stat_out,
                       reinterpret_cast<float (*)[33]>(xs_raw));
    } else {
        if (r16) {
#pragma unroll
            for (int i = 0; i < 4; ++i) y[i] = (float)(f16)y[i];
        }
        if (a.logits && valid && live_l) {
            float* lo = a.logits + (size_t)gb * a.N + n;
            if (n + 3 < a.N) {
                *reinterpret_cast<float2*>(lo) = float2{y[0], y[1]};
                *reinterpret_cast<float2*>(lo + 2) = float2{y[2], y[3]};
            } else {
#pragma unroll
                for (int i = 0; i < 4; ++i) if (n + i < a.N) lo[i] = y[i];
            }
        }
        if (a.stats) {
            SoftStat t_{-INFINITY, 0.0f, 0x7fffffff}, u_{-INFINITY, 0.0f, 0x7fffffff};
            const int blank = rules[0], ts_active = rules[1];
#pragma unroll
            for (int i = 0; i < 4; ++i) {
                const int id = n + i;
                bool masked = ((masked4[t] >> (8 * i)) & 0xff) != 0 || id >= a.N;
                masked |= blank && (id == ws_tok || id == eot_tok);
                masked |= ts_active && (id == nots_tok || (id >= rules[2] && id < rules[3]) || (id >= rules[4] && id < rules[5]));
                if (!masked) { if (id < tb) stat_merge(t_, y[i], 1.0f, id); else stat_merge(u_, y[i], 1.0f, id); }
            }
            float* xr = xs_raw;
            float* rec = xr + (size_t)(sub * 32 + j) * 6;
            rec[0] = t_.m; rec[1] = t_.s; rec[2] = __int_as_float(t_.i); rec[3] = u_.m; rec[4] = u_.s; rec[5] = __int_as_float(u_.i);
            __syncthreads();
            if (tid < 32 && valid && live_l) {
                SoftStat T{-INFINITY, 0.0f, 0x7fffffff}, U{-INFINITY, 0.0f, 0x7fffffff};
#pragma unroll
                for (int s = 0; s < 8; ++s) {
                    const float* r_ = xr + (size_t)(s * 32 + tid) * 6;
                    stat_merge(T, r_[0], r_[1], __float_as_int(r_[2]));
                    stat_merge(U, r_[3], r_[4], __float_as_int(r_[5]));
                }
                float* o = a.stats + ((size_t)gb * kStatBlocks + rt) * 8;
                *reinterpret_cast<float4*>(o) = float4{T.m, T.s, __int_as_float(T.i), U.m};
                *reinterpret_cast<float2*>(o + 4) = float2{U.s, __int_as_float(U.i)};
            }
        }
    }
  }
    D32_STAMP(6);
    if constexpr (MODE == P32_Q) { if (a.gate && blockIdx.x == 0 && tid == 0) xattn_gate_acquire(a.gate); }
}


__global__ __launch_bounds__(256) void dec32_embed_kernel(const f16* __restrict__ emb, const float* __restrict__ pos, const SeqState* __restrict__ seq,
                                                          int batch, int d, int n_vocab, float* x, const float* gamma_next, f16* zhi, f16* zlo,
                                                          float2* stat_out) {
    __shared__ float xs[32][33];
    const int tid = threadIdx.x, j = tid & 31, sub = tid >> 5;
    const int rt = blockIdx.x, bt = blockIdx.y, n_rt = gridDim.x;
    const int n = rt * 32 + 4 * sub, gb = bt * 32 + j;
    const bool valid = gb < batch;
    float xn[4] = {0, 0, 0, 0};
    bool live = false;
    if (valid) {
        live = slot_live(seq + gb);
        const int tok = min(max(seq[gb].next_token, 0), n_vocab - 1);
        const int p = min(max(seq[gb].token_index, 0), kMaxTok - 1);
        const f16x4 e = *reinterpret_cast<const f16x4*>(emb + (size_t)tok * d + n);
        const float4 pz = *reinterpret_cast<const float4*>(pos + (size_t)p * d + n);
        xn[0] = (float)e[0] + pz.x; xn[1] = (float)e[1] + pz.y; xn[2] = (float)e[2] + pz.z; xn[3] = (float)e[3] + pz.w;
    }
    d32_resid_tail(xn, valid && live, bt, rt, n_rt, n, j, gb, tid, d, x, gamma_next, zhi, zlo, stat_out, xs);
}
void launch_dec32_embed(const f16* emb, const float* pos, const SeqState* seq, int batch, int d, int n_vocab, int n_bt, float* x,
                        const float* gamma_next, f16* zhi, f16* zlo, float2* stat, hipStream_t st) {
    ProfScope ps_(KK_DEC_EMBED, st);
    dec32_embed_kernel<<<dim3(d / 32, n_bt), 256, 0, st>>>(emb, pos, seq, batch, d, n_vocab, x, gamma_next, zhi, zlo, stat);
}

template <int MODE, bool HILO>
static void launch_planned(const P32Args& a, const plan::Dec32Plan& p, hipStream_t st) {
    const dim3 grid(p.grid);
#define D32_GO(TC_, RT_) do { \
        if (p.ntw) dec32_proj_kernel<MODE, HILO, TC_, true, RT_><<<grid, 256, 0, st>>>(a); \
        else dec32_proj_kernel<MODE, HILO, TC_, false, RT_><<<grid, 256, 0, st>>>(a); \
        return; } while (0)
    if constexpr (MODE != P32_LOGITS && MODE != P32_LOGITS_MIXED && MODE != P32_Q) {
        if (p.rt == 4) D32_GO(1, 4);
    }
    if (p.rt >= 2) {
        if (p.tc == 4) D32_GO(4, 2);
        if (p.tc == 2) D32_GO(2, 2);
        D32_GO(1, 2);
    }
    switch (p.tc) {
        case 5: D32_GO(5, 1);
        case 4: D32_GO(4, 1);
        case 3: D32_GO(3, 1);
        case 2: D32_GO(2, 1);
        default: D32_GO(1, 1);
    }
#undef D32_GO
}

unsigned long long* debug_buffer();
void launch_dec32_proj(int mode, const P32Args& a_in, int n_bt, hipStream_t st, bool mixed) {
    using namespace knob;
    P32Args a = a_in;
    a.dbg = (debug_buffer() && a.prof_kind >= 0) ? debug_buffer() + (size_t)a.prof_kind * 4096 * 8 : nullptr;
    const plan::Dec32Knobs k{once<WH_D32_KS_RESID>(), once<WH_D32_KS_FC2>(), once<WH_D32_KS_Q>(), once<WH_D32_KS_WIDE>(), once<WH_D32_TILE_KB>(), once<WH_D32_TC>(),
                             once<WH_D32_TC_BT>(), once<WH_D32_RT2_TC>(), once<WH_D32_NTW>(), once<WH_D32_RT_BT>(), once<WH_D32_RT4_BT>(), once<WH_D32_RT4_MODES>()};
    const plan::Dec32Plan p = plan::dec32_plan(mode, a.N, a.K, n_bt, k);
    a.ks = p.ks; a.tw = p.tw; a.rt = p.rt; a.n_bt = n_bt;
    ProfScope ps_(a.prof_kind, st);
    switch (mode) {
        case P32_QKV: launch_planned<P32_QKV, true>(a, p, st); break;
        case P32_Q: launch_planned<P32_Q, true>(a, p, st); break;
        case P32_FC1: launch_planned<P32_FC1, true>(a, p, st); break;
        case P32_LOGITS:
            if (mixed && a.stats && a.sup_mask) launch_planned<P32_LOGITS_MIXED, true>(a, p, st);
            else launch_planned<P32_LOGITS, true>(a, p, st);
            break;
        default:
            if (a.zlo != nullptr) launch_planned<P32_RESID, true>(a, p, st);
            else launch_planned<P32_RESID, false>(a, p, st);
    }
}

}
```

### whisperkit_amd/csrc/internal.h

```cpp
#pragma once
#include <map>
#include <new>
#include <stdexcept>
#include <string>
#include <tuple>
#include <unordered_map>
#include <vector>

#include "devmem.h"
#include "kernels.h"
#include "text.h"
#include "whisperhip.h"

struct HipMem {
    using Err = hipError_t;
    static constexpr Err ok = hipSuccess, out_of_memory = hipErrorOutOfMemory;
    static Err dev_malloc(void** p, size_t n) { return hipMalloc(p, n); }
    static Err dev_free(void* p) { return hipFree(p); }
    static Err host_malloc(void** p, size_t n) { return hipHostMalloc(p, n); }
    static Err host_free(void* p) { return hipHostFree(p); }
    static Err dev_memset(void* p, int v, size_t n) { return hipMemset(p, v, n); }
};
using DevMem = wh::mem::Owned<HipMem>;

// ... 56 lines not shown

struct wh_session {
    DevMem mem;
    wh_model* m = nullptr;
    int B = 0;
    hipStream_t st = nullptr;
    float* pcm = nullptr; int* n_valid = nullptr;
    float* logspec = nullptr; unsigned* maxkey = nullptr; f16* mel_t = nullptr; float* mel_f32 = nullptr;
    f16* h1 = nullptr; float* x = nullptr; f16* xn = nullptr; f16 *q16 = nullptr, *k16 = nullptr, *vt16 = nullptr, *att16 = nullptr;
    f16* hmlp = nullptr; f16* enc16 = nullptr; float* enc32 = nullptr;
    int encoder_precision = 0;
    f16 *mel_t_lo = nullptr, *h1_lo = nullptr, *xn_lo = nullptr, *att_lo = nullptr, *hmlp_lo = nullptr, *enc_lo = nullptr;
    f16 *cross_k_hi = nullptr, *cross_v_hi = nullptr;
    signed char *cross_k_lo = nullptr, *cross_v_lo = nullptr;
    f16 *self_k = nullptr, *self_v = nullptr;
    float *part = nullptr, *logits = nullptr;
    int* ticket = nullptr;
    float *align = nullptr, *align_mean = nullptr;
    int n_align_alloc = 0;
    int align_znorm = 0, align_median = 0;
    float* align_tmp = nullptr; int align_tmp_heads = 0;
    int word_alignment = 0;
    int* dtw_dev = nullptr;
    int32_t* dtw_host = nullptr;
    long long dtw_launches = 0, align_d2h_bytes = 0;
    std::map<WhGraphKey, hipGraphExec_t> graphs;
    std::map<WhGraphKey, unsigned long long> graph_use;
    unsigned long long graph_tick = 0;
    const volatile int32_t* cancel_flag = nullptr;
    bool use_xabs = false;
    wh::Xabs xabs{};
    wh::Dec32 d32{};
    wh::SeqState* seq = nullptr;
    wh::SeqState* seq_host = nullptr;
    wh::SamplerCfg* cfg_dev = nullptr;
    int* suppress_dev = nullptr;
    unsigned char* sup_mask_dev = nullptr;
    int option_mixing = 0;
    bool pass_mixed = false;
    long long mix_groups_run = 0, mix_mixed_passes = 0, mix_max_classes = 0;
    float* stats = nullptr;
    bool fused_greedy = false;
    int *tok_out_dev = nullptr; float* lp_out_dev = nullptr;
    float* scratch_logits = nullptr;
    int *beam_owner = nullptr, *beam_tok = nullptr; float* beam_lp = nullptr;
    int beam_ranking = 0;
    wh::SeqState* beam_seq_alt = nullptr; int* beam_owner_alt = nullptr; float* beam_sum = nullptr;
    wh::BeamAudioState* beam_audio = nullptr;
    wh::BeamAudioState* beam_audio_host = nullptr;
    int* beam_fin_tok = nullptr; float *beam_fin_lp = nullptr, *beam_fin_sum = nullptr;
    int* beam_fin_len = nullptr;
    long long beam_rank_launches = 0, beam_loop_syncs = 0;
    int fallback_compaction = 0;
    int32_t *slot_home_dev = nullptr, *slot_home_host = nullptr;
    bool pass_mapped = false; int pass_spw = 1;
    wh::Xabs xabs_pass{};
    long long decode_passes = 0, compacted_passes = 0, slot_steps = 0;
    int inpass_compaction = 0;
    wh::SeqState *seq_home = nullptr, *seq_snap = nullptr;
    int32_t *inpass_dev = nullptr, *inpass_stage = nullptr;
    bool pass_owner = false;
    long long inpass_switches = 0, inpass_slot_steps_saved = 0;
    hipEvent_t ev[8]{};
    bool align_enabled = false;
    wh_timings last_timings{};
    const wh_tokenizer* tok = nullptr;
    wh_progress_fn progress_cb = nullptr;
    void* progress_user = nullptr;
    wh_window_hooks hooks{};
    bool skip_special_in_progress = false;
    const int32_t* skip_special_by_slot = nullptr;
    int special_begin_in_progress = 1 << 30;
    std::vector<int> item_status;
    std::vector<std::string> item_error;
};

struct wh_device_audio {
    DevMem mem;
    int device = 0;
    int n = 0;
    float* data = nullptr;
    hipStream_t st = nullptr;
    double *sums_dev = nullptr, *sums_pin = nullptr; size_t sums_cap = 0;
    long long vad_launches = 0;
    mutable long long d2h_bytes = 0;
};

namespace whi {
int set_error(int code, const char* fmt, ...);
int device_audio_new(int device, int n, wh_device_audio** out);
int vad_chunks_device(wh_device_audio* a, int max_chunk, const wh_decoding_options* opt, std::vector<std::pair<int, int>>& out);
#define WH_HIP(expr)                                                                               \
    do {                                                                                           \
        hipError_t _e = (expr);                                                                    \
        if (_e != hipSuccess) return whi::set_error(WH_ERR_HIP, "%s failed: %s", #expr, hipGetErrorString(_e)); \
    } while (0)
#define WH_CHECK_LAUNCH() WH_HIP(hipGetLastError())
#define CHECK_SESSION(s) do { if (!(s) || !(s)->m) return whi::set_error(WH_ERR_MODELS_UNAVAILABLE, "%s: session/model is null (modelsUnavailable)", __func__); \
                              if (hipSetDevice((s)->m->device) != hipSuccess) return whi::set_error(WH_ERR_HIP, "%s: hipSetDevice(%d) failed", __func__, (s)->m->device); } while (0)
#define CHECK_SLOT(s, b) do { if ((b) < 0 || (b) >= (s)->B) return whi::set_error(WH_ERR_INVALID_ARGUMENT, "%s: slot %d out of range [0,%d)", __func__, (b), (s)->B); } while (0)
#define CHECK_BATCH(s, n) do { if ((n) < 1 || (n) > (s)->B) return whi::set_error(WH_ERR_INVALID_ARGUMENT, "%s: batch %d out of range [1,%d]", __func__, (n), (s)->B); } while (0)
#define WH_TRY try {
#define WH_CATCH(name) } catch (const std::bad_alloc&) { return whi::set_error(WH_ERR_OUT_OF_MEMORY, "%s: out of host memory", name); } \
                         catch (const std::exception& e_) { return whi::set_error(WH_ERR_INVALID_ARGUMENT, "%s: %s", name, e_.what()); }

wh::DecodeBuffers decode_buffers(wh_session* s, int batch, int max_position = wh::kMaxTok - 1);
// ... 9 lines not shown
```

### whisperkit_amd/csrc/kernels.h

```cpp
#pragma once
#include "common.h"
#include "launch_plan.h"
#include "option_mix.h"

#include <atomic>
#include <mutex>
#include <vector>

namespace wh {

struct PerDeviceOnce {
    std::atomic<unsigned long long> done{0};
    std::mutex mu;
    template <class F> void run(F f) {
        int dev = 0;
        (void)hipGetDevice(&dev);
        const unsigned long long bit = 1ull << (dev & 63);
        if (done.load(std::memory_order_acquire) & bit) return;
        std::lock_guard<std::mutex> lk(mu);
        if (done.load(std::memory_order_relaxed) & bit) return;
        f();
        done.fetch_or(bit, std::memory_order_release);
    }
};
// ... 119 lines not shown
constexpr int kMaxPrompt = 232;

struct SeqState {
    int tokens[kMaxTok + 8];
    float logprobs[kMaxTok + 8];
    int n_tokens;
    int token_index;
    int next_token;
    int done;
    int first_token_too_low;
    int steps;
    int active;
    float temperature;
    int prompt_len;
    int f_rules[6];
    int rng_lane;
};
constexpr int kSeqClassShift = 16;
constexpr int seq_lane(int rng_lane) { return rng_lane & ((1 << kSeqClassShift) - 1); }
constexpr int seq_class(int rng_lane) { return (rng_lane >> kSeqClassShift) & (kMaxOptionClasses - 1); }
constexpr int seq_pack_lane(int lane, int cls) { return lane | (cls << kSeqClassShift); }

struct DecodeBuffers {
    int batch, max_batch, d, n_head, n_layer, n_vocab;
    const f16* emb;
    const float* pos;
    const DecLayerW* layers_host;
    const float *lnf_g, *lnf_b;
    f16* self_k;
    f16* self_v;
    const f16 *cross_k_hi, *cross_v_hi;
    const signed char *cross_k_lo, *cross_v_lo;
    float* x;
    float* q;
    float* part;
    int* ticket;
    float* logits;
    float* stats;
    const unsigned char* sup_mask;
    int fused_greedy;
    float* align;
    const int* align_slot;
    int n_align;
    SeqState* seq;
    int cross_div;
    int* xattn_gate;
    int self_rows;
    const int* self_owner;
    const struct Dec32* d32;
    const struct Xabs* xabs;
    const int* slot_home;
    int mixed;
    int owner_slots;
};
constexpr int kStatBlocks = 1792;
constexpr int kMaxVocab = 52224;
static_assert(kMaxVocab <= kStatBlocks * 32, "fused greedy sampler: one statistics record per 32-row logits tile");
constexpr int kMaxSplit = 24;
constexpr int kPartStride = 96;

struct Dec32LayerW {
    const f16 *qkv_t, *o_t, *cq_t, *co_t, *fc1_t, *fc2_t;
    const float *qkv_g, *qkv_c, *cq_g, *cq_c, *fc1_g, *fc1_c;
};
struct Dec32 {
    const Dec32LayerW* layers_host;
    const f16* emb_t; const float *lg_g, *lg_c;
    int n_bt;
    float* x;
    float* q;
    f16 *za_hi, *za_lo;
    f16 *zb_hi, *zb_lo;
    f16 *h, *h_lo;
    float2* stat;
    float* part; int* ticket;
    size_t part_floats;
};
struct P32Args {
    int batch, N, K, d, n_head, n_vocab;
    int ks, tw;
    int n_bt;
    int rt;
    const f16* Wt;
    const f16 *zhi, *zlo;
    const float2* stat_in; int n_stat; const float *fold_g, *fold_c;
    const float* bias; float* x; const float* gamma_next; f16 *zhi_out, *zlo_out; float2* stat_out;
    float* q; f16 *self_k, *self_v;
    f16 *h_out, *h_out_lo;
    float* logits; float* stats; const unsigned char* sup_mask; const SamplerCfg* cfg;
    float* part; int* ticket;
    const SeqState* seq;
    int* gate;
    int prof_kind;
    unsigned long long* dbg;
};
void launch_dec32_proj(int mode, const P32Args& a, int n_bt, hipStream_t st, bool mixed = false);
void launch_dec32_embed(const f16* emb, const float* pos, const SeqState* seq, int batch, int d, int n_vocab, int n_bt, float* x,
                        const float* gamma_next, f16* zhi, f16* zlo, float2* stat, hipStream_t st);
void dec32_tile_weights(const f16* W, int N, int K, f16* out, hipStream_t st);
void dec32_fold_vectors(const f16* W, int N, int K, const float* gamma, const float* beta, const float* bias, float* g, float* c, hipStream_t st);

constexpr int kXabsMaxSlotsPerWorkgroup = 16;
constexpr int kMaxSessionSlots = 256;
static_assert((kMaxOptionClasses & (kMaxOptionClasses - 1)) == 0 && kMaxSessionSlots <= (1 << kSeqClassShift), "SeqState.rng_lane: lane | class");
constexpr int kXabsAutoMinSlots = 28;
int xabs_splits(int max_batch);
using plan::xabs_auto_splits;
struct XabsLayerW {
    const f16* wkT;
    const f16* wv_t;
    const float* bv;
};
struct Xabs {
    const XabsLayerW* layers_host;
    const f16* enc;
    f16 *qf_hi, *qf_lo;
    float* part;
    float2* ml;
    int n_split;
    int spw;
};
struct XabsArgs {
    int batch, max_batch, d, n_head, layer, n_split, cross_div;
    int mapped;
    const f16* enc; const float* q;
    const f16 *wkT, *wv_t; const float* bv;
    f16 *qf_hi, *qf_lo; float* part; float2* ml;
    f16 *att_hi, *att_lo;
    float* align; const int* align_slot; int n_align;
    const SeqState* seq;
    float* kpart; int* ticket;
    union { unsigned long long* dbg; const int* slot_home; };
    int ablate;
    int* gate;
    int spw;
};
using plan::xabs_supported;
using plan::xabs_auto_width;
void xabs_tile_wk(const f16* Wk, int d, int H, f16* out, hipStream_t st);
void launch_xabs_qk(const XabsArgs& a, int n_bt, hipStream_t st);
void launch_xabs_attn(const XabsArgs& a, hipStream_t st);
void launch_xabs_vup(const XabsArgs& a, int n_bt, hipStream_t st);

void launch_decoder_step(const DecodeBuffers& db, const SamplerCfg* cfg_dev, const int* suppress_dev, bool sample, hipStream_t st);
void launch_rules_init(const SamplerCfg* cfg_dev, SeqState* seq, int batch, hipStream_t st, bool mixed = false);
void launch_seq_park(const SeqState* seq, SeqState* seq_home, const int* home, int width, int n_slots, hipStream_t st);
void launch_seq_gather(const SeqState* seq_home, SeqState* seq, const int* home, const int* live, int width, int n_slots, hipStream_t st);
void launch_filter_only(const SamplerCfg* cfg_dev, const int* suppress_dev, SeqState* seq, float* logits, int n_vocab, hipStream_t st);
void launch_sample_only(const SamplerCfg* cfg_dev, SeqState* seq, float* logits, int n_vocab, int counter, int* token_out, float* logprob_out, hipStream_t st);
void launch_filter_sample(const SamplerCfg* cfg_dev, const int* suppress_dev, SeqState* seq, float* logits, int batch, int* token_out, float* logprob_out, hipStream_t st);
constexpr int kBeamTopK = 16;
void launch_beam_filter_topk(const SamplerCfg* cfg_dev, const int* suppress_dev, SeqState* seq, float* logits, int batch, int K, float* lp_out,
                             int* tok_out, hipStream_t st);
constexpr int kBeamRankThreads = 256;
constexpr int kBeamFinishedCap = 32;
constexpr int kBeamSeqStride = kMaxTok + 8;
struct BeamAudioState {
    int live;
    int n_beams;
    int finished;
    int steps, first_token_too_low;
    int parity;
    int n_added, completed;
};
struct BeamRankArgs {
    int n_audio, beam_size, max_candidates, eot, len, topk_stride;
    const float* topk_lp; const int* topk_tok;
    const int* tok_in; const float* lp_in; const float* sum_in;
    int* tok_out; float* lp_out; float* sum_out;
    long long in_stride, out_stride;
    BeamAudioState* audio;
    int* sources;
    int* fin_tok; float* fin_lp; float* fin_sum; int* fin_len;
    int fin_cap, fin_stride, fin_append;
    const SeqState* seq_in; SeqState* seq_out;
    const int* owner_in; int* owner_out;
    int token_index, prompt_len, parity_out;
    int has_first_token_threshold, threshold_position; float first_token_log_prob_threshold;
};
int launch_beam_rank(const BeamRankArgs& a, hipStream_t st);
void launch_alignment_mean(const float* align, int batch, int n_align, float* out, hipStream_t st);
void launch_alignment_postprocess(const float* align, int n_align, float* prob_tmp, float* stat_tmp, int* row_written, int znorm, int median_width,
                                  float* out, hipStream_t st);
constexpr int kDtwThreads = 256, kDtwMaxRows = 256, kDtwMaxCols = 1500;
constexpr int kDtwPathCap = kDtwMaxRows + kDtwMaxCols;
int launch_dtw_batch(const float* m, const int* rows_dev, int n, int max_rows, int rows_stride, int cols, int* text_idx, int* time_idx, int* lengths,
                     int capacity, hipStream_t st);
void launch_f32_to_f16(const float* in, f16* out, size_t n, hipStream_t st);
void launch_f32_to_f16_split(const float* in, f16* hi, f16* lo, size_t n, hipStream_t st);
void launch_f16_to_f32(const f16* in, float* out, size_t n, hipStream_t st);

}
```

### whisperkit_amd/csrc/launch_plan.h

```cpp
#pragma once
#include <cstdint>

namespace wh {

enum GemmEpi {
    EPI_F16 = 0,
    EPI_GELU_F16 = 1,
    EPI_RESID_F32 = 2,
    EPI_QKV_ENC = 3,
    EPI_CONV1 = 4,
    EPI_CONV2 = 5,
    EPI_F32 = 6,
    EPI_CROSS_KV = 7,
};

constexpr int kD32PartFloats = 2 * 1024 * 1024;
enum { P32_QKV = 0, P32_Q = 1, P32_RESID = 2, P32_FC1 = 3, P32_LOGITS = 4,
       P32_LOGITS_MIXED = 5 };

constexpr int kXabsSplits = 4;

namespace plan {

constexpr bool has_staged_epilogue(int epi) { return epi == EPI_F16 || epi == EPI_GELU_F16 || epi == EPI_RESID_F32 || epi == EPI_QKV_ENC; }

enum GemmFamily { GEMM_256, GEMM_256P, GEMM_128, GEMM_64 };
struct GemmKnobs { int no256, epi_mode, persist, persist_wgs, cus; };
struct GemmPlan { GemmFamily family; int mode; unsigned grid_x, grid_y; long long tiles256; };

inline GemmPlan gemm_plan(int M, int N, int K, int lda, long long a_batch_stride, int ldc, int d_model, int epi, bool split, uintptr_t out_bases,
                          const GemmKnobs& k) {
    GemmPlan p{};
    p.tiles256 = (long long)((M + 255) / 256) * ((N + 255) / 256);
    const int k_tile = split ? 32 : 64;
    if (!k.no256 && p.tiles256 >= 64 && K % k_tile == 0 && lda % 8 == 0 && a_batch_stride % 8 == 0 && N % 4 == 0) {
        p.family = (k.persist && !split) ? GEMM_256P : GEMM_256;
        p.mode = 0;
        if (has_staged_epilogue(epi)) {
            const bool aligned = (out_bases & 15) == 0;
            const bool shape_ok = aligned && N % 64 == 0 && M % 4 == 0 && ldc % 8 == 0 && d_model % 64 == 0;
            if (shape_ok && (k.epi_mode == 1 || k.epi_mode == 2)) p.mode = k.epi_mode;
        }
        const long long tiles8 = (p.tiles256 + 7) / 8 * 8;
        const long long want = k.persist_wgs ? k.persist_wgs : k.cus;
        p.grid_x = (unsigned)(p.family == GEMM_256P ? (want < tiles8 ? want : tiles8) : p.tiles256);
        p.grid_y = 1;
        return p;
    }
    const long long tiles128 = (long long)((M + 127) / 128) * ((N + 127) / 128);
    const int t = tiles128 >= 192 ? 128 : 64;
    p.family = t == 128 ? GEMM_128 : GEMM_64;
    p.grid_x = (unsigned)((N + t - 1) / t);
    p.grid_y = (unsigned)((M + t - 1) / t);
    return p;
}

enum LnKernel { LN_SCALAR, LN_V4, LN_V4_NT };
inline LnKernel layernorm_plan(int d, uintptr_t f32_bases, uintptr_t y16, uintptr_t y16_lo, bool has_lo, int v4) {
    bool aligned = d % 4 == 0 && f32_bases % 16 == 0 && y16 % 8 == 0;
    if (has_lo) aligned = aligned && y16_lo % 8 == 0;
    if (v4 == 2 && aligned) return LN_V4_NT;
    if (v4 && aligned) return LN_V4;
    return LN_SCALAR;
}

struct Dec32Knobs { int ks_resid, ks_fc2, ks_q, ks_wide, tile_kb, tc, tc_bt, rt2_tc, ntw, rt_bt, rt4_bt, rt4_modes; };
struct Dec32Plan { int ks, tw, rt, tc; bool ntw; unsigned grid; };
inline Dec32Plan dec32_plan(int mode, int N, int K, int n_bt, const Dec32Knobs& k) {
    Dec32Plan p{};
    const bool fc2 = mode == P32_RESID && K > N;
    const int n_rt = (N + 31) / 32;
    {
        int want = (mode == P32_RESID) ? (fc2 ? k.ks_fc2 : k.ks_resid) : (mode == P32_Q ? k.ks_q : k.ks_wide);
        if (want <= 0) want = (K / 16 + k.tile_kb - 1) / k.tile_kb;
        const int groups = K / 64;
        want = want < 1 ? 1 : (want > 8 ? 8 : want);
        while (want > 1 && groups % want) --want;
        if ((long long)n_rt * want * 1024 > kD32PartFloats) want = 1;
        p.ks = want;
    }
    p.tw = K / (64 * p.ks);
    p.rt = n_bt >= k.rt_bt ? 2 : 1;
    {
        const int bit = mode == P32_QKV ? 1 : mode == P32_FC1 ? 2 : fc2 ? 4 : 0;
        if (n_bt >= k.rt4_bt && (k.rt4_modes & bit) && n_rt % 4 == 0) p.rt = 4;
    }
    if (p.rt == 4) {
        p.tc = 1;
    } else if (p.rt == 2) {
        p.tc = (p.tw % 4 == 0 && k.rt2_tc >= 4) ? 4 : (p.tw % 2 == 0 && k.rt2_tc >= 2) ? 2 : 1;
    } else {
        const int tc_cap = k.tc > 0 ? k.tc : (n_bt >= k.tc_bt ? 2 : 5);
        p.tc = (p.tw % 5 == 0 && tc_cap >= 5) ? 5 : (p.tw % 4 == 0 && tc_cap >= 4) ? 4 : (p.tw % 3 == 0 && tc_cap >= 3) ? 3 : (p.tw % 2 == 0) ? 2 : 1;
    }
    p.ntw = k.ntw < 0 ? n_bt == 1 : k.ntw != 0;
    const int nx = ((n_rt + p.rt - 1) / p.rt) * p.ks;
    p.grid = (unsigned)(((nx + 7) / 8) * 8 * n_bt);
    return p;
}

inline int self_attn_passes(int self_rows) {
    const int passes = self_rows > 0 ? (self_rows + 31) / 32 : 7;
    return passes > 7 ? 7 : passes;
}
struct CrossAttnPlan { int passes, splits; };
inline CrossAttnPlan cross_attn_plan(int n_head, int forced, int ctx) {
    int passes = forced ? forced : (n_head >= 12 ? 4 : 2);
    passes = passes > 6 ? 8 : passes > 4 ? 6 : passes > 2 ? 4 : 2;
    return {passes, (ctx + passes * 32 - 1) / (passes * 32)};
}

inline bool xabs_supported(int d, int n_head) { return (d == 384 || (d % 256 == 0 && d >= 512 && d <= 1280)) && n_head <= 32 && n_head * 64 == d; }
inline bool xabs_auto_width(int d, int n_head) { return xabs_supported(d, n_head) && d >= 512; }

inline int xabs_auto_splits(int max_batch) {
    const int s = 256 / (max_batch > 0 ? max_batch : 1);
    return s < 1 ? 1 : (s > kXabsSplits ? kXabsSplits : s);
}
inline unsigned xabs_attn_grid(int batch, int spw, int n_split) {
    const int s = spw > 1 ? spw : 1, b1 = (batch + s - 1) / s;
    const int n_grp = (b1 + 3) / 4 * n_split;
    return (unsigned)((n_grp + 7) / 8 * 32);
}
struct XabsVupPlan { int ks; unsigned grid; };
inline XabsVupPlan xabs_vup_plan(int d, int n_head, int n_bt) {
    const int ks = d == 384 ? 3 : 4;
    const int nx = n_head * ks;
    return {ks, (unsigned)(((nx + 7) / 8) * 8 * n_bt)};
}

constexpr int kCompactLadder[] = {32, 64, 128};
constexpr int kCompactRungs = (int)(sizeof(kCompactLadder) / sizeof(kCompactLadder[0]));
struct CompactPassPlan { bool compact; int width, spw; };
inline CompactPassPlan compact_pass_plan(int n_live, int batch, int max_batch, int slots_per_workgroup) {
    const int spw0 = slots_per_workgroup > 1 ? slots_per_workgroup : 1;
    CompactPassPlan p{false, batch, spw0};
    if (n_live < 1 || n_live >= batch) return p;
    for (int r = 0; r < kCompactRungs; ++r) {
        const int w = kCompactLadder[r];
        if (w < n_live) continue;
        if ((w + 31) / 32 >= (batch + 31) / 32) break;
        const int wgs = ((max_batch > batch ? max_batch : batch) + spw0 - 1) / spw0;
        p.compact = true; p.width = w; p.spw = (w + wgs - 1) / wgs;
        break;
    }
    return p;
}
inline int compact_slot_map(const int32_t* active, int batch, int width, int32_t* home, int32_t* live) {
    int n = 0;
    for (int b = 0; b < batch; ++b) {
        if (active && !active[b]) continue;
        if (n >= width) return -1;
        home[n] = b; live[n] = 1; ++n;
    }
    for (int i = n; i < width; ++i) { home[i] = i < batch ? i : 0; live[i] = 0; }
    return n;
}

constexpr int kInpassMinStepsLeft = 16;
constexpr int kInpassMaxSwitches = kCompactRungs;
inline CompactPassPlan inpass_compact_plan(int n_live, int width_now, int max_batch, int slots_per_workgroup, int steps_left) {
    const int spw0 = slots_per_workgroup > 1 ? slots_per_workgroup : 1;
    const CompactPassPlan none{false, width_now, spw0};
    if (steps_left < kInpassMinStepsLeft) return none;
    const CompactPassPlan p = compact_pass_plan(n_live, width_now, max_batch, spw0);
    return (p.compact && p.width < width_now) ? p : none;
}
inline int inpass_compose(const int32_t* home_old, const int32_t* live_old, const int32_t* owner_old, int width_old, const int32_t* keep, int width_new,
                          int t, int rows, int n_slots, int32_t* home_new, int32_t* live_new, int32_t* owner_new) {
    if (width_new < 1 || width_new > n_slots || width_old > n_slots || rows < 1) return -1;
    const int tt = t < 0 ? 0 : (t > rows ? rows : t);
    int n = 0;
    for (int i = 0; i < width_old; ++i) {
        if (!keep[i] || (live_old && !live_old[i])) continue;
        if (n >= width_new) return -1;
        const int h = home_old ? home_old[i] : i;
        if (h < 0 || h >= n_slots) return -1;
        home_new[n] = h; live_new[n] = 1;
        for (int r = 0; r < rows; ++r) {
            const int own = r >= tt ? n : (owner_old ? owner_old[(long long)i * rows + r] : i);
            if (own < 0 || own >= n_slots) return -1;
// ... 14 lines not shown
```

### whisperkit_amd/csrc/xabs.hip

```cpp
#include "dec_shared.h"
#include "knobs.h"

namespace wh {

typedef unsigned u32x4 __attribute__((ext_vector_type(4)));
typedef short s16x4 __attribute__((ext_vector_type(4)));
typedef f16 f16x2 __attribute__((ext_vector_type(2)));

__host__ __device__ __forceinline__ int xswz(int key) { return ((key & 3) << 2) | ((0x78 >> (2 * ((key >> 2) & 3))) & 3); }

__global__ void xabs_tile_wk_kernel(const f16* __restrict__ Wk, int d, int H, f16* __restrict__ out, size_t n_units) {
    const size_t o = (size_t)blockIdx.x * blockDim.x + threadIdx.x;
    if (o >= n_units) return;
    const int lane = (int)(o & 63);
    size_t t = o >> 6;
    const int kt = (int)(t & 3); t >>= 2;
    const int RT = d >> 5;
    const int rt = (int)(t % RT), h = (int)(t / RT);
    const int c = rt * 32 + (lane & 31), j0 = h * 64 + kt * 16 + 8 * (lane >> 5);
    f16x8 v;
#pragma unroll
    for (int i = 0; i < 8; ++i) v[i] = Wk[(size_t)(j0 + i) * d + c];
    *reinterpret_cast<f16x8*>(out + o * 8) = v;
}
// ... 283 lines not shown
    __syncthreads();
    s_phase(s_base(0), sreg);
    write_partials(sreg);
    if (n > 1) wait_tile(1);
    __syncthreads();
    XPHASE(11);
#define XSTAMP(k) do { if constexpr (DBG) if (a.dbg && (i == 10 || i == 11) && lane == 0 && (wave == 0 || wave == 5) && blockIdx.x < 64) \
        a.dbg[((blockIdx.x * 2 + (wave == 5)) * 2 + (i - 10)) * 16 + (k)] = __builtin_amdgcn_s_memtime(); } while (0)
    for (int i = 0; i < n; ++i) {
        XSTAMP(0);
        const bool work = !DBG || !(a.ablate & 2), fetch = !DBG || !(a.ablate & 1);
        if (work && i + 1 < n) s_phase(s_base(i + 1), sreg);
        XSTAMP(1);
        if (work && owner) softmax(i);
        XSTAMP(2);
        __syncthreads();
        XSTAMP(3);
        if (work && i + 1 < n) write_partials(sreg);
        XSTAMP(4);
        if (work) pv(t_base(i));
        XSTAMP(5);
        if (fetch && i + 2 < n) wait_tile(i + 2);
        XSTAMP(6);
        __syncthreads();
        XSTAMP(7);
        const int nx = i + 3 + (1 - half_w);
        if (fetch && nx < n) issue(nx);
        XSTAMP(8);
    }
#undef XSTAMP
    asm volatile("s_waitcnt vmcnt(0)" ::: "memory");
    XPHASE(12);
    if (owner && o_key == 0 && o_head < H) a.ml[((size_t)sp * H + o_head) * a.max_batch + b] = float2{m_run, l_run};
    {
        const int head = lane & 31, hl = lane >> 5;
        if (head < H) {
            float* pb = a.part + (((size_t)sp * H + head) * (D / 8)) * a.max_batch * 8 + (size_t)b * 8 + 4 * hl;
#pragma unroll
            for (int mt = 0; mt < CW; ++mt)
#pragma unroll
                for (int g = 0; g < 4; ++g) {
                    const int c8 = (wave * CW + mt) * 4 + g;
                    *reinterpret_cast<float4*>(pb + (size_t)c8 * a.max_batch * 8) = float4{acc[mt][4 * g], acc[mt][4 * g + 1], acc[mt][4 * g + 2], acc[mt][4 * g + 3]};
                }
        }
    }
    if constexpr (DBG) asm volatile("s_waitcnt vmcnt(0)" ::: "memory");
    XPHASE(13);
  }
#undef XPHASE
}


template <int S, int TW>
__global__ __launch_bounds__(256, 1) void xabs_vup_kernel(const XabsArgs a, int ks, int n_bt) {
    __shared__ float red[4][2][16][64];
    __shared__ int last_flag;
    const int tid = threadIdx.x, lane = tid & 63, wave = tid >> 6;
    const int d = a.d, H = a.n_head, KT = d >> 4;
    const int grp8 = blockIdx.x / (8 * n_bt), in8 = blockIdx.x % (8 * n_bt);
    const int xw = grp8 * 8 + (in8 & 7), bt = in8 >> 3;
    if (xw >= H * ks) return;
    const int h = xw % H, ksi = xw / H;
    const int kt0 = (ksi * 4 + wave) * TW;
    const int j = lane & 31, hl = lane >> 5;
    const int gbl = min(bt * 32 + j, a.max_batch - 1);
    float2 ml[S];
#pragma unroll
    for (int s = 0; s < S; ++s) ml[s] = a.ml[((size_t)s * H + h) * a.max_batch + gbl];
    const u32x4* wp = reinterpret_cast<const u32x4*>(a.wv_t) + ((size_t)(2 * h) * KT + kt0) * 64 + lane;
    const size_t sstride = (size_t)H * (d / 8) * a.max_batch * 8;
    const float* pp = a.part + ((size_t)h * (d / 8) + kt0 * 2 + hl) * a.max_batch * 8 + (size_t)gbl * 8;
    u32x4 w0[TW], w1[TW];
    f32x4 p0[TW][S], p1[TW][S];
#pragma unroll
    for (int i = 0; i < TW; ++i) { w0[i] = __builtin_nontemporal_load(wp + (size_t)i * 64); w1[i] = __builtin_nontemporal_load(wp + ((size_t)KT + i) * 64); }
#pragma unroll
    for (int i = 0; i < TW; ++i)
#pragma unroll
        for (int s = 0; s < S; ++s) {
            const float* q = pp + (size_t)s * sstride + (size_t)i * 2 * a.max_batch * 8;
            p0[i][s] = *reinterpret_cast<const f32x4*>(q);
            p1[i][s] = *reinterpret_cast<const f32x4*>(q + 4);
        }
#pragma unroll
    for (int i = 0; i < TW; ++i) {
        asm volatile("" : "+v"(w0[i]), "+v"(w1[i]));
#pragma unroll
        for (int s = 0; s < S; ++s) asm volatile("" : "+v"(p0[i][s]), "+v"(p1[i][s]));
    }
    float wn[S];
    {
        float mg = ml[0].x;
#pragma unroll
        for (int s = 1; s < S; ++s) mg = fmaxf(mg, ml[s].x);
        float lg = 0.0f;
#pragma unroll
        for (int s = 0; s < S; ++s) { wn[s] = __expf(ml[s].x - mg); lg = fmaf(wn[s], ml[s].y, lg); }
        const float inv = 1.0f / lg;
#pragma unroll
        for (int s = 0; s < S; ++s) wn[s] *= inv;
    }
    f32x16 acc_h[2] = {{0}, {0}}, acc_l[2] = {{0}, {0}};
#pragma unroll
    for (int i = 0; i < TW; ++i) {
        float z[8] = {0, 0, 0, 0, 0, 0, 0, 0};
#pragma unroll
        for (int s = 0; s < S; ++s) {
#pragma unroll
            for (int e = 0; e < 4; ++e) { z[e] = fmaf(wn[s], p0[i][s][e], z[e]); z[4 + e] = fmaf(wn[s], p1[i][s][e], z[4 + e]); }
        }
        f16x8 zh, zl;
#pragma unroll
        for (int e = 0; e < 8; ++e) { f16 h_, l_; split_hilo(z[e], h_, l_); zh[e] = h_; zl[e] = l_; }
        const f16x8 wf0 = __builtin_bit_cast(f16x8, w0[i]), wf1 = __builtin_bit_cast(f16x8, w1[i]);
        acc_h[0] = __builtin_amdgcn_mfma_f32_32x32x16_f16(wf0, zh, acc_h[0], 0, 0, 0);
        acc_l[0] = __builtin_amdgcn_mfma_f32_32x32x16_f16(wf0, zl, acc_l[0], 0, 0, 0);
        acc_h[1] = __builtin_amdgcn_mfma_f32_32x32x16_f16(wf1, zh, acc_h[1], 0, 0, 0);
        acc_l[1] = __builtin_amdgcn_mfma_f32_32x32x16_f16(wf1, zl, acc_l[1], 0, 0, 0);
    }
#pragma unroll
    for (int t = 0; t < 2; ++t)
#pragma unroll
        for (int r = 0; r < 16; ++r) red[wave][t][r][lane] = fmaf(acc_l[t][r], 1.0f / 2048.0f, acc_h[t][r]);
    __syncthreads();
    const int sub = tid >> 5, gb = bt * 32 + (tid & 31);
    float v[2][4];
#pragma unroll
    for (int t = 0; t < 2; ++t)
#pragma unroll
        for (int i = 0; i < 4; ++i) v[t][i] = ((red[0][t][4 * wave + i][lane] + red[1][t][4 * wave + i][lane]) + red[2][t][4 * wave + i][lane]) + red[3][t][4 * wave + i][lane];
    if (ks > 1) {
        float* base = a.kpart + (((size_t)bt * H + h) * ks) * 2048 + tid * 4;
#pragma unroll
        for (int t = 0; t < 2; ++t) {
            const f32x4 pv4 = {v[t][0], v[t][1], v[t][2], v[t][3]};
            float* mine = base + (size_t)ksi * 2048 + t * 1024;
            asm volatile("global_store_dwordx4 %0, %1, off sc1\n\ts_nop 1" ::"v"(mine), "v"(pv4) : "memory");
        }
        asm volatile("s_waitcnt vmcnt(0)" ::: "memory");
        __syncthreads();
        if (tid == 0) {
            int* cnt = a.ticket + bt * H + h;
            const int t = __hip_atomic_fetch_add(cnt, 1, __ATOMIC_RELAXED, __HIP_MEMORY_SCOPE_AGENT);
            const int last = (t == ks - 1);
            if (last) __hip_atomic_store(cnt, 0, __ATOMIC_RELAXED, __HIP_MEMORY_SCOPE_AGENT);
            last_flag = last;
        }
        __syncthreads();
        if (!last_flag) return;
        float pv[4][2][4];
#pragma unroll
        for (int s = 0; s < 4; ++s)
#pragma unroll
            for (int t = 0; t < 2; ++t) {
                const float* p = base + (size_t)(s < ks ? s : 0) * 2048 + t * 1024;
#pragma unroll
                for (int i = 0; i < 4; ++i) pv[s][t][i] = __hip_atomic_load(p + i, __ATOMIC_RELAXED, __HIP_MEMORY_SCOPE_AGENT);
            }
#pragma unroll
        for (int t = 0; t < 2; ++t)
#pragma unroll
            for (int i = 0; i < 4; ++i) {
                float x = pv[0][t][i];
#pragma unroll
                for (int s = 1; s < 4; ++s) x += (s < ks) ? pv[s][t][i] : 0.0f;
                v[t][i] = x;
            }
    }
    if (gb < a.batch && slot_live(a.seq + gb)) {
#pragma unroll
        for (int t = 0; t < 2; ++t) {
            const int nn = (2 * h + t) * 32 + 4 * sub;
            const float4 bv = *reinterpret_cast<const float4*>(a.bv + nn);
            const float y[4] = {v[t][0] + bv.x, v[t][1] + bv.y, v[t][2] + bv.z, v[t][3] + bv.w};
            f16x4 hi, lo;
#pragma unroll
            for (int i = 0; i < 4; ++i) { f16 h_, l_; split_hilo(y[i], h_, l_); hi[i] = h_; lo[i] = l_; }
            const size_t o = plane_index(gb, nn, d);
            *reinterpret_cast<f16x4*>(a.att_hi + o) = hi;
            *reinterpret_cast<f16x4*>(a.att_lo + o) = lo;
        }
    }
}

int xabs_splits(int max_batch) {
    const int e = knob::now<knob::WH_XABS_SPLITS>();
    return e ? e : xabs_auto_splits(max_batch);
}

void launch_xabs_qk(const XabsArgs& a, int n_bt, hipStream_t st) {
    ProfScope ps_(KK_DEC_XQK, st);
    if (a.d == 384) { xabs_qk_kernel<1, 2><<<dim3(3, a.n_head, n_bt), 128, 0, st>>>(a); return; }
    const dim3 grid(a.d / 256, a.n_head, n_bt);
    if (a.n_head > 16) xabs_qk_kernel<2><<<grid, 256, 0, st>>>(a);
    else xabs_qk_kernel<1><<<grid, 256, 0, st>>>(a);
}

template <int CW, int NHT, bool DBG, bool NTL, bool MAP = false>
static void launch_attn_k(const XabsArgs& a, hipStream_t st) {
    constexpr int lds = xabs_lds_bytes(CW);
    static PerDeviceOnce once;
    once.run([] { (void)hipFuncSetAttribute(reinterpret_cast<const void*>(&xabs_attn_kernel<CW, NHT, DBG, NTL, 8, MAP>), hipFuncAttributeMaxDynamicSharedMemorySize, lds); });
    xabs_attn_kernel<CW, NHT, DBG, NTL, 8, MAP><<<dim3(plan::xabs_attn_grid(a.batch, a.spw, a.n_split)), 512, lds, st>>>(a);
}
template <int KSW, bool DBG, bool NTL, bool MAP = false>
static void launch_attn_w4_k(const XabsArgs& a, hipStream_t st) {
    constexpr int lds = xabs_lds_bytes_w(4, KSW);
    static PerDeviceOnce once;
    once.run([] { (void)hipFuncSetAttribute(reinterpret_cast<const void*>(&xabs_attn_kernel<KSW, 1, DBG, NTL, 4, MAP>), hipFuncAttributeMaxDynamicSharedMemorySize, lds); });
    xabs_attn_kernel<KSW, 1, DBG, NTL, 4, MAP><<<dim3(plan::xabs_attn_grid(a.batch, a.spw, a.n_split)), 256, lds, st>>>(a);
}
template <int CW, int NHT, bool DBG, bool NTL, bool MAP = false>
static void launch_attn_any(const XabsArgs& a, hipStream_t st) {
    if constexpr (CW == 0) launch_attn_w4_k<3, DBG, NTL, MAP>(a, st); else launch_attn_k<CW, NHT, DBG, NTL, MAP>(a, st);
}
template <int CW, int NHT>
static void launch_attn_t(const XabsArgs& a, hipStream_t st) {
    const int nt = knob::once<knob::WH_XABS_NT>();
    const int ablate = knob::once<knob::WH_XABS_ABLATE>();
    if (a.mapped) { if (nt) launch_attn_any<CW, NHT, false, true, true>(a, st); else launch_attn_any<CW, NHT, false, false, true>(a, st); return; }
    if (a.dbg || ablate) { XabsArgs b = a; b.ablate = ablate; launch_attn_any<CW, NHT, true, false>(b, st); return; }
    if (nt && a.cross_div <= 1) launch_attn_any<CW, NHT, false, true>(a, st); else launch_attn_any<CW, NHT, false, false>(a, st);
}
void launch_xabs_attn(const XabsArgs& a, hipStream_t st) {
    ProfScope ps_(KK_DEC_CROSS_ATTN, st);
    const bool two = a.n_head > 16;
    switch (a.d / 256) {
        case 1: launch_attn_t<0, 1>(a, st); break;
        case 2: two ? launch_attn_t<2, 2>(a, st) : launch_attn_t<2, 1>(a, st); break;
        case 3: two ? launch_attn_t<3, 2>(a, st) : launch_attn_t<3, 1>(a, st); break;
        case 4: two ? launch_attn_t<4, 2>(a, st) : launch_attn_t<4, 1>(a, st); break;
        default: two ? launch_attn_t<5, 2>(a, st) : launch_attn_t<5, 1>(a, st); break;
    }
}

void launch_xabs_vup(const XabsArgs& a, int n_bt, hipStream_t st) {
    ProfScope ps_(KK_DEC_XVUP, st);
    const plan::XabsVupPlan p = plan::xabs_vup_plan(a.d, a.n_head, n_bt);
    const int ks = p.ks;
    const unsigned grid = p.grid;
#define XVUP(S_) do { switch (a.d / 256) { \
        case 1: xabs_vup_kernel<S_, 2><<<grid, 256, 0, st>>>(a, ks, n_bt); break; \
        case 2: xabs_vup_kernel<S_, 2><<<grid, 256, 0, st>>>(a, ks, n_bt); break; \
        case 3: xabs_vup_kernel<S_, 3><<<grid, 256, 0, st>>>(a, ks, n_bt); break; \
        case 4: xabs_vup_kernel<S_, 4><<<grid, 256, 0, st>>>(a, ks, n_bt); break; \
        default: xabs_vup_kernel<S_, 5><<<grid, 256, 0, st>>>(a, ks, n_bt); break; } } while (0)
    switch (a.n_split) {
        case 1: XVUP(1); break;
        case 2: XVUP(2); break;
        case 3: XVUP(3); break;
        default: XVUP(4); break;
    }
#undef XVUP
}

}
```

Measured before the change: 2645.

## Fold split-K slices into a single workgroup for decoder residual and V-up projections

```diff
diff --git a/include/whisperhip.h b/include/whisperhip.h
--- a/include/whisperhip.h
+++ b/include/whisperhip.h
@@ -164,13 +164,15 @@
     int32_t cross_attention_splits;
     int32_t cross_attention_slots_per_workgroup;
     int32_t encoder_precision;
-    int32_t reserved_[3];
+    int32_t reserved_[2];
+    int32_t k_slice_folding;
     int32_t fallback_compaction;
 } wh_session_options;
 void wh_session_options_default(wh_session_options* out);
 int wh_session_create_with_options(wh_model* m, int max_batch, const wh_session_options* opt, wh_session** out);
 int wh_session_cross_attention_slots_per_workgroup(const wh_session* s);
 int wh_session_encoder_precision(const wh_session* s);
+int wh_session_k_slice_folding(const wh_session* s);
 int wh_debug_peek(wh_session* s, const char* name, void* out_host, size_t nbytes);
 long long wh_debug_live_allocations(void);
 int wh_session_step_graph_count(const wh_session* s);
diff --git a/whisperkit_amd/_lib.py b/whisperkit_amd/_lib.py
--- a/whisperkit_amd/_lib.py
+++ b/whisperkit_amd/_lib.py
@@ -53,7 +53,7 @@
 
 class WhSessionOptions(C.Structure):
     _fields_ = [("cross_attention_mode", C.c_int32), ("cross_attention_splits", C.c_int32), ("cross_attention_slots_per_workgroup", C.c_int32),
-                ("encoder_precision", C.c_int32), ("reserved_", C.c_int32 * 3), ("fallback_compaction", C.c_int32)]
+                ("encoder_precision", C.c_int32), ("reserved_", C.c_int32 * 2), ("k_slice_folding", C.c_int32), ("fallback_compaction", C.c_int32)]
 
 
 class WhTensor(C.Structure):
@@ -130,6 +130,7 @@
     "wh_session_destroy": (None, [VP]),
     "wh_session_max_batch": (I, [VP]),
     "wh_session_cross_attention_mode": (I, [VP]),
+    "wh_session_k_slice_folding": (I, [VP]),
     "wh_session_cross_attention_splits": (I, [VP]),
     "wh_xabs_auto_min_slots": (I, []),
     "wh_xabs_auto_splits": (I, [I]),
diff --git a/whisperkit_amd/api.py b/whisperkit_amd/api.py
--- a/whisperkit_amd/api.py
+++ b/whisperkit_amd/api.py
@@ -418,20 +418,24 @@
 class Session:
 
     ENCODER_PRECISIONS = {None: 0, "f16": 0, "split": 1}
+    K_SLICE_FOLDINGS = {None: 0, "auto": 0, "off": 1, "on": 2}
 
     def __init__(self, model: Model, maxBatch: int = 1, crossAttentionMode: Optional[int] = None, crossAttentionSplits: Optional[int] = None,
-                 crossAttentionSlotsPerWorkgroup: Optional[int] = None, encoderPrecision: Optional[str] = None):
+                 crossAttentionSlotsPerWorkgroup: Optional[int] = None, encoderPrecision: Optional[str] = None, kSliceFolding: Optional[str] = None):
+        if kSliceFolding not in self.K_SLICE_FOLDINGS:
+            raise ValueError(f"kSliceFolding {kSliceFolding!r}: expected None, 'auto', 'off' or 'on'")
         self.model, self.lib, self.B = model, model.lib, maxBatch
         self.handle = C.c_void_p()
         if encoderPrecision not in self.ENCODER_PRECISIONS:
             raise ValueError(f"encoderPrecision {encoderPrecision!r}: expected None, 'f16' or 'split'")
-        if crossAttentionSlotsPerWorkgroup is not None or encoderPrecision is not None:
+        if crossAttentionSlotsPerWorkgroup is not None or encoderPrecision is not None or kSliceFolding is not None:
             o = L.WhSessionOptions()
             self.lib.wh_session_options_default(C.byref(o))
             o.cross_attention_mode = -1 if crossAttentionMode is None else int(crossAttentionMode)
             o.cross_attention_splits = 0 if crossAttentionSplits is None else int(crossAttentionSplits)
             o.cross_attention_slots_per_workgroup = int(crossAttentionSlotsPerWorkgroup or 0)
             o.encoder_precision = self.ENCODER_PRECISIONS[encoderPrecision]
+            o.k_slice_folding = self.K_SLICE_FOLDINGS[kSliceFolding]
             _check(self.lib.wh_session_create_with_options(model.handle, maxBatch, C.byref(o), C.byref(self.handle)))
         elif crossAttentionMode is None and crossAttentionSplits is None:
             _check(self.lib.wh_session_create(model.handle, maxBatch, C.byref(self.handle)))
@@ -458,6 +462,10 @@
     @property
     def encoderPrecision(self) -> str:
         return {0: "f16", 1: "split"}[int(self.lib.wh_session_encoder_precision(self.handle))]
+
+    @property
+    def kSliceFolding(self) -> str:
+        return {0: "auto", 1: "off", 2: "on"}[int(self.lib.wh_session_k_slice_folding(self.handle))]
 
     @property
     def crossAttentionMode(self) -> int:
diff --git a/whisperkit_amd/csrc/capi.hip b/whisperkit_amd/csrc/capi.hip
--- a/whisperkit_amd/csrc/capi.hip
+++ b/whisperkit_amd/csrc/capi.hip
@@ -401,11 +401,13 @@
                          "the absorbed kernel streams the Float16 encoder output, and a hi | lo stream would double its bytes");
     if (opt->fallback_compaction < 0 || opt->fallback_compaction > 1)
         return set_error(WH_ERR_INVALID_ARGUMENT, "wh_session_create: fallback_compaction %d (expected 0 off, 1 on)", opt->fallback_compaction);
+    if (opt->k_slice_folding < 0 || opt->k_slice_folding > 2)
+        return set_error(WH_ERR_INVALID_ARGUMENT, "wh_session_create: k_slice_folding %d (expected 0 automatic, 1 off, 2 on)", opt->k_slice_folding);
     if (cross_attention_mode == 1 && m && !xabs_supported(m->dims.n_text_state, m->dims.n_text_head))
         return set_error(WH_ERR_INVALID_ARGUMENT, "wh_session_create: the absorbed cross-attention needs a model width of 384 / 512 / 768 / 1024 / 1280 (this model: %d)", m->dims.n_text_state);
     const int r = session_create_impl(m, max_batch, opt->encoder_precision == 1 ? 0 : cross_attention_mode, cross_attention_splits,
                                       opt->cross_attention_slots_per_workgroup, out, opt->encoder_precision);
-    if (r == WH_OK) (*out)->fallback_compaction = opt->fallback_compaction;
+    if (r == WH_OK) { (*out)->fallback_compaction = opt->fallback_compaction; (*out)->k_slice_folding = opt->k_slice_folding; }
     return r;
 }
 extern "C" int wh_session_create_with_mode(wh_model* m, int max_batch, int cross_attention_mode, wh_session** out) {
@@ -514,6 +516,7 @@
 }
 extern "C" int wh_session_max_batch(const wh_session* s) { return s ? s->B : -1; }
 extern "C" int wh_session_cross_attention_mode(const wh_session* s) { return s ? (s->use_xabs ? 1 : 0) : -1; }
+extern "C" int wh_session_k_slice_folding(const wh_session* s) { return s ? s->k_slice_folding : -1; }
 extern "C" int wh_session_encoder_precision(const wh_session* s) { return s ? s->encoder_precision : -1; }
 extern "C" int wh_session_step_graph_count(const wh_session* s) { return s ? (int)s->graphs.size() : -1; }
 extern "C" int wh_session_cross_attention_splits(const wh_session* s) { return s ? (s->use_xabs ? s->xabs.n_split : 0) : -1; }
@@ -718,6 +721,7 @@
     db.mixed = s->pass_mixed ? 1 : 0; db.stats = s->stats; db.sup_mask = s->sup_mask_dev; db.fused_greedy = s->fused_greedy ? 1 : 0;
     db.align = s->align_enabled ? s->align : nullptr; db.align_slot = m->align_slot_dev; db.n_align = s->n_align_alloc;
     db.d32 = &s->d32; db.x = s->d32.x; db.q = s->d32.q;
+    db.k_slice_fold = s->k_slice_folding == 0 ? -1 : s->k_slice_folding - 1;
     if (s->use_xabs) { s->xabs.enc = s->enc16; db.xabs = &s->xabs; }
     if (s->pass_mapped) {
         db.slot_home = s->slot_home_dev;
diff --git a/whisperkit_amd/csrc/dec32_proj_body.inc b/whisperkit_amd/csrc/dec32_proj_body.inc
--- /dev/null
+++ b/whisperkit_amd/csrc/dec32_proj_body.inc
@@ -0,0 +1,384 @@
+    static_assert(SL == 1 || MODE == P32_RESID, "folded K slices: the RESID form only");
+    constexpr bool kMix = MODE == P32_LOGITS_MIXED, kLogits = MODE == P32_LOGITS || kMix;
+    constexpr bool kLN = MODE == P32_QKV || MODE == P32_Q || MODE == P32_FC1 || kLogits;
+    constexpr int kXs = kLogits ? 256 * 6 : 32 * 33;
+    __shared__ float red[RT][4][16][64];
+    __shared__ float st_l[8][32][3];
+    __shared__ float xs_raw[kXs];
+    __shared__ int last_flag;
+    const int tid = threadIdx.x, lane = tid & 63, wave = tid >> 6;
+    const int n_rt = (a.N + 31) >> 5;
+    const int n_rtp = (n_rt + RT - 1) / RT;
+    const int grp8 = blockIdx.x / (8 * a.n_bt), in8 = blockIdx.x % (8 * a.n_bt);
+    const int xw = grp8 * 8 + (in8 & 7), bt = in8 >> 3;
+    if (xw >= n_rtp * (SL > 1 ? 1 : a.ks)) return;
+    const int rt0 = (xw % n_rtp) * RT, ksi = SL > 1 ? 0 : xw / n_rtp;
+    const int n_mine = min(RT, n_rt - rt0);
+    const int KT = a.K >> 4;
+    const int kt0 = (ksi * 4 + wave) * a.tw;
+    const u32x4* wp[RT];
+#pragma unroll
+    for (int t = 0; t < RT; ++t) wp[t] = reinterpret_cast<const u32x4*>(a.Wt) + ((size_t)min(rt0 + t, n_rt - 1) * KT + kt0) * 64 + lane;
+    const size_t zoff = ((size_t)bt * KT + kt0) * 64 + lane;
+    const u32x4* hp = reinterpret_cast<const u32x4*>(a.zhi) + zoff;
+    const u32x4* lp = HILO ? reinterpret_cast<const u32x4*>(a.zlo) + zoff : nullptr;
+    const int j = tid & 31, sub = tid >> 5;
+    const int gb = bt * 32 + j;
+    const bool valid = gb < a.batch;
+    const int xw_dbg = xw;
+
+#define D32_STAMP(i) do { if (a.dbg && tid == 0 && bt == 0) a.dbg[(size_t)(xw_dbg & 4095) * 8 + (i)] = wall_clock64(); } while (0)
+    D32_STAMP(0);
+    float2 sp[5] = {};
+    if constexpr (kLN) {
+#pragma unroll
+        for (int i = 0; i < 5; ++i) {
+            const int idx = min(sub + 8 * i, a.n_stat - 1);
+            sp[i] = a.stat_in[((size_t)bt * a.n_stat + idx) * 32 + j];
+        }
+    }
+    constexpr bool kLateOperands = RT >= 4 || SL > 1;
+    constexpr int NB = RT >= 4 ? 3 : 2;
+    float4 e0[RT], e1[RT];
+    float4 gm[SL > 1 ? RT : 1];
+    int pos_l = 0, live_l = 0;
+    auto load_operands = [&]() {
+#pragma unroll
+        for (int t = 0; t < RT; ++t) {
+            const int n = min(rt0 + t, n_rt - 1) * 32 + 4 * sub;
+            if constexpr (kLN) {
+                e0[t] = *reinterpret_cast<const float4*>(a.fold_g + n);
+                e1[t] = *reinterpret_cast<const float4*>(a.fold_c + n);
+            } else {
+                e0[t] = *reinterpret_cast<const float4*>(a.bias + n);
+                e1[t] = *reinterpret_cast<const float4*>(a.x + (size_t)gb * a.d + n);
+                if constexpr (SL > 1) gm[t] = *reinterpret_cast<const float4*>(a.gamma_next + n);
+            }
+        }
+    };
+    if constexpr (!kLateOperands) load_operands();
+    if (valid) { live_l = slot_live(a.seq + gb); if constexpr (MODE == P32_QKV) pos_l = a.seq[gb].token_index; }
+    int rules[6] = {0, 0, 0, 0, 0, 0};
+    unsigned masked4[RT];
+    int tb = 0, ws_tok = 0, eot_tok = 0, nots_tok = 0, r16 = 0;
+#pragma unroll
+    for (int t = 0; t < RT; ++t) masked4[t] = 0xffffffffu;
+    if constexpr (kLogits) {
+        if (a.cfg) r16 = a.cfg->f16_logits;
+        if (a.stats) {
+            if (valid) {
+#pragma unroll
+                for (int i = 0; i < 6; ++i) rules[i] = a.seq[gb].f_rules[i];
+            }
+            const unsigned char* sup_mask = a.sup_mask;
+            if constexpr (kMix) { if (valid) sup_mask += (size_t)seq_class(a.seq[gb].rng_lane) * plan::option_mask_stride(a.N); }
+#pragma unroll
+            for (int t = 0; t < RT; ++t) {
+                const int n = min(rt0 + t, n_rt - 1) * 32 + 4 * sub;
+                if (n + 3 < a.N) masked4[t] = *reinterpret_cast<const unsigned*>(sup_mask + n);
+                else {
+                    masked4[t] = 0;
+#pragma unroll
+                    for (int i = 0; i < 4; ++i) masked4[t] |= (unsigned)(n + i < a.N ? sup_mask[n + i] : 1) << (8 * i);
+                }
+            }
+            tb = a.cfg->time_token_begin; ws_tok = a.cfg->whitespace_token; eot_tok = a.cfg->end_token; nots_tok = a.cfg->no_timestamps_token;
+        }
+    }
+
+    f32x16 acc_h[RT], acc_l[RT];
+#pragma unroll
+    for (int t = 0; t < RT; ++t)
+#pragma unroll
+        for (int r = 0; r < 16; ++r) { acc_h[t][r] = 0.0f; acc_l[t][r] = 0.0f; }
+    auto stats_to_lds = [&]() {
+        if constexpr (kLN) {
+            float cm = sp[0].x, cM2 = sp[0].y;
+            const int mine = sub < a.n_stat ? (a.n_stat - sub + 7) >> 3 : 0;
+            if (mine > 1) chan32_k<1>(cm, cM2, sp[1].x, sp[1].y);
+            if (mine > 2) chan32_k<2>(cm, cM2, sp[2].x, sp[2].y);
+            if (mine > 3) chan32_k<3>(cm, cM2, sp[3].x, sp[3].y);
+            if (mine > 4) chan32_k<4>(cm, cM2, sp[4].x, sp[4].y);
+            st_l[sub][j][0] = 32.0f * (float)mine; st_l[sub][j][1] = cm; st_l[sub][j][2] = cM2;
+        }
+    };
+    float xf[SL > 1 ? RT : 1][4] = {};
+    if constexpr (SL > 1) {
+        u32x4 w_[NB][RT][TC], h_[NB][TC], l_[NB][HILO ? TC : 1];
+        const int nch = a.tw / TC, ntot = nch * a.ks;
+        int l_cc = 0, l_kt = 0;
+        auto ld = [&](u32x4 (&w)[RT][TC], u32x4 (&h)[TC], u32x4 (&l)[HILO ? TC : 1]) {
+#pragma unroll
+            for (int t = 0; t < RT; ++t)
+#pragma unroll
+                for (int i = 0; i < TC; ++i) w[t][i] = wp[t][(size_t)(l_kt + i) * 64];
+#pragma unroll
+            for (int i = 0; i < TC; ++i) h[i] = hp[(size_t)(l_kt + i) * 64];
+            if constexpr (HILO) {
+#pragma unroll
+                for (int i = 0; i < TC; ++i) l[i] = lp[(size_t)(l_kt + i) * 64];
+            }
+            l_kt += TC;
+            if (++l_cc == nch) { l_cc = 0; l_kt += 3 * a.tw; }
+        };
+        auto mm = [&](const u32x4 (&w)[RT][TC], const u32x4 (&h)[TC], const u32x4 (&l)[HILO ? TC : 1]) {
+#pragma unroll
+            for (int i = 0; i < TC; ++i) {
+#pragma unroll
+                for (int t = 0; t < RT; ++t) {
+                    const f16x8 wf = __builtin_bit_cast(f16x8, w[t][i]);
+                    acc_h[t] = __builtin_amdgcn_mfma_f32_32x32x16_f16(wf, __builtin_bit_cast(f16x8, h[i]), acc_h[t], 0, 0, 0);
+                    if constexpr (HILO) acc_l[t] = __builtin_amdgcn_mfma_f32_32x32x16_f16(wf, __builtin_bit_cast(f16x8, l[i]), acc_l[t], 0, 0, 0);
+                }
+            }
+        };
+        auto slice_end = [&](bool first) {
+#pragma unroll
+            for (int t = 0; t < RT; ++t)
+#pragma unroll
+                for (int r = 0; r < 16; ++r) {
+                    red[t][wave][r][lane] = HILO ? fmaf(acc_l[t][r], 1.0f / 2048.0f, acc_h[t][r]) : acc_h[t][r];
+                    acc_h[t][r] = 0.0f; acc_l[t][r] = 0.0f;
+                }
+            __syncthreads();
+#pragma unroll
+            for (int t = 0; t < RT; ++t)
+#pragma unroll
+                for (int i = 0; i < 4; ++i) {
+                    const float vs = ((red[t][0][4 * wave + i][lane] + red[t][1][4 * wave + i][lane]) + red[t][2][4 * wave + i][lane]) + red[t][3][4 * wave + i][lane];
+                    xf[t][i] = first ? vs : xf[t][i] + vs;
+                }
+            __syncthreads();
+        };
+        int m_cc = 0, m_s = 0;
+#pragma unroll
+        for (int u = 0; u + 1 < NB; ++u)
+            if (u < ntot) ld(w_[u], h_[u], l_[u]);
+        D32_STAMP(1);
+#pragma unroll 1
+        for (int c = 0; c < ntot; c += NB) {
+#pragma unroll
+            for (int u = 0; u < NB; ++u) {
+                constexpr int kAhead = NB - 1;
+                if (c + u + kAhead < ntot) ld(w_[(u + kAhead) % NB], h_[(u + kAhead) % NB], l_[(u + kAhead) % NB]);
+                __builtin_amdgcn_sched_barrier(0);
+                if (c + u < ntot) {
+                    mm(w_[u], h_[u], l_[u]);
+                    if (++m_cc == nch) {
+                        m_cc = 0;
+                        if (m_s + 1 < a.ks) slice_end(m_s == 0);
+                        ++m_s;
+                    }
+                }
+                if (u == 0 && c == 0) D32_STAMP(2);
+            }
+        }
+    } else {
+        u32x4 w_[NB][RT][TC], h_[NB][TC], l_[NB][HILO ? TC : 1];
+        auto ld = [&](u32x4 (&w)[RT][TC], u32x4 (&h)[TC], u32x4 (&l)[HILO ? TC : 1], int c) {
+#pragma unroll
+            for (int t = 0; t < RT; ++t)
+#pragma unroll
+                for (int i = 0; i < TC; ++i) w[t][i] = NTW ? __builtin_nontemporal_load(wp[t] + (size_t)(c * TC + i) * 64) : wp[t][(size_t)(c * TC + i) * 64];
+#pragma unroll
+            for (int i = 0; i < TC; ++i) h[i] = hp[(size_t)(c * TC + i) * 64];
+            if constexpr (HILO) {
+#pragma unroll
+                for (int i = 0; i < TC; ++i) l[i] = lp[(size_t)(c * TC + i) * 64];
+            }
+        };
+        auto mm = [&](const u32x4 (&w)[RT][TC], const u32x4 (&h)[TC], const u32x4 (&l)[HILO ? TC : 1]) {
+#pragma unroll
+            for (int i = 0; i < TC; ++i) {
+#pragma unroll
+                for (int t = 0; t < RT; ++t) {
+                    const f16x8 wf = __builtin_bit_cast(f16x8, w[t][i]);
+                    acc_h[t] = __builtin_amdgcn_mfma_f32_32x32x16_f16(wf, __builtin_bit_cast(f16x8, h[i]), acc_h[t], 0, 0, 0);
+                    if constexpr (HILO) acc_l[t] = __builtin_amdgcn_mfma_f32_32x32x16_f16(wf, __builtin_bit_cast(f16x8, l[i]), acc_l[t], 0, 0, 0);
+                }
+            }
+        };
+        const int nch = a.tw / TC;
+#pragma unroll
+        for (int u = 0; u + 1 < NB; ++u)
+            if (u < nch) ld(w_[u], h_[u], l_[u], u);
+        D32_STAMP(1);
+#pragma unroll 1
+        for (int c = 0; c < nch; c += NB) {
+#pragma unroll
+            for (int u = 0; u < NB; ++u) {
+                constexpr int kAhead = NB - 1;
+                if (c + u + kAhead < nch) ld(w_[(u + kAhead) % NB], h_[(u + kAhead) % NB], l_[(u + kAhead) % NB], c + u + kAhead);
+                __builtin_amdgcn_sched_barrier(0);
+                if (c + u < nch) mm(w_[u], h_[u], l_[u]);
+                if (u == 0 && c == 0) D32_STAMP(2);
+            }
+        }
+    }
+    if constexpr (kLateOperands) load_operands();
+    stats_to_lds();
+    D32_STAMP(3);
+#pragma unroll
+    for (int t = 0; t < RT; ++t)
+#pragma unroll
+        for (int r = 0; r < 16; ++r) red[t][wave][r][lane] = HILO ? fmaf(acc_l[t][r], 1.0f / 2048.0f, acc_h[t][r]) : acc_h[t][r];
+    __syncthreads();
+    D32_STAMP(4);
+    float v[RT][4];
+#pragma unroll
+    for (int t = 0; t < RT; ++t)
+#pragma unroll
+        for (int i = 0; i < 4; ++i) v[t][i] = ((red[t][0][4 * wave + i][lane] + red[t][1][4 * wave + i][lane]) + red[t][2][4 * wave + i][lane]) + red[t][3][4 * wave + i][lane];
+    if constexpr (SL > 1) {
+#pragma unroll
+        for (int t = 0; t < RT; ++t)
+#pragma unroll
+            for (int i = 0; i < 4; ++i) v[t][i] = xf[t][i] + v[t][i];
+        __syncthreads();
+    }
+
+    if (SL == 1 && a.ks > 1) {
+        float* base = a.part + (((size_t)bt * n_rt + rt0) * a.ks) * 1024 + tid * 4;
+#pragma unroll
+        for (int t = 0; t < RT; ++t) {
+            if (t < n_mine) {
+                const f32x4 pv4 = {v[t][0], v[t][1], v[t][2], v[t][3]};
+                float* mine = base + ((size_t)t * a.ks + ksi) * 1024;
+                asm volatile("global_store_dwordx4 %0, %1, off sc1\n\ts_nop 1" ::"v"(mine), "v"(pv4) : "memory");
+            }
+        }
+        asm volatile("s_waitcnt vmcnt(0)" ::: "memory");
+        __syncthreads();
+        if (tid == 0) {
+            int* cnt = a.ticket + bt * n_rt + rt0;
+            const int t = __hip_atomic_fetch_add(cnt, 1, __ATOMIC_RELAXED, __HIP_MEMORY_SCOPE_AGENT);
+            const int last = (t == a.ks - 1);
+            if (last) __hip_atomic_store(cnt, 0, __ATOMIC_RELAXED, __HIP_MEMORY_SCOPE_AGENT);
+            last_flag = last;
+        }
+        __syncthreads();
+        if (!last_flag) {
+            if constexpr (MODE == P32_Q) { if (a.gate && blockIdx.x == 0 && tid == 0) xattn_gate_acquire(a.gate); }
+            return;
+        }
+        float pv[RT][8][4];
+#pragma unroll
+        for (int t = 0; t < RT; ++t)
+#pragma unroll
+            for (int s = 0; s < 8; ++s) {
+                const float* p = base + ((size_t)(t < n_mine ? t : 0) * a.ks + (s < a.ks ? s : 0)) * 1024;
+#pragma unroll
+                for (int i = 0; i < 4; ++i) pv[t][s][i] = __hip_atomic_load(p + i, __ATOMIC_RELAXED, __HIP_MEMORY_SCOPE_AGENT);
+            }
+#pragma unroll
+        for (int t = 0; t < RT; ++t)
+#pragma unroll
+            for (int i = 0; i < 4; ++i) {
+                float x_ = pv[t][0][i];
+#pragma unroll
+                for (int s = 1; s < 8; ++s) x_ += (s < a.ks) ? pv[t][s][i] : 0.0f;
+                v[t][i] = x_;
+            }
+    }
+
+    D32_STAMP(5);
+    float mu = 0.0f, rstd = 0.0f;
+    if constexpr (kLN) {
+        float cn = 0.0f, cm = 0.0f, cM2 = 0.0f;
+#pragma unroll
+        for (int s = 0; s < 8; ++s) chan_merge(cn, cm, cM2, st_l[s][j][0], st_l[s][j][1], st_l[s][j][2]);
+        mu = cm; rstd = rsqrtf(cM2 / (float)a.d + 1e-5f);
+    }
+#pragma unroll
+  for (int t = 0; t < RT; ++t) {
+    if (t >= n_mine) break;
+    if constexpr ((MODE == P32_RESID && SL == 1) || kLogits) { if (t > 0) __syncthreads(); }
+    const int rt = rt0 + t, n = rt * 32 + 4 * sub;
+    float y[4];
+    if constexpr (kLN) {
+        const float g4[4] = {e0[t].x, e0[t].y, e0[t].z, e0[t].w}, c4[4] = {e1[t].x, e1[t].y, e1[t].z, e1[t].w};
+#pragma unroll
+        for (int i = 0; i < 4; ++i) y[i] = fmaf(rstd, v[t][i] - mu * g4[i], c4[i]);
+    }
+    if constexpr (MODE == P32_QKV) {
+        if (valid && live_l) {
+            const int d = a.d;
+            if (n < d) *reinterpret_cast<float4*>(a.q + (size_t)gb * d + n) = float4{y[0], y[1], y[2], y[3]};
+            else {
+                int c = n - d;
+                f16* dst = a.self_k;
+                if (c >= d) { c -= d; dst = a.self_v; }
+                const int pos = min(max(pos_l, 0), kMaxTok - 1);
+                *reinterpret_cast<f16x4*>(dst + (((size_t)gb * a.n_head + (c >> 6)) * kMaxTok + pos) * kHeadDim + (c & 63)) =
+                    f16x4{(f16)y[0], (f16)y[1], (f16)y[2], (f16)y[3]};
+            }
+        }
+    } else if constexpr (MODE == P32_Q) {
+        if (valid && live_l) *reinterpret_cast<float4*>(a.q + (size_t)gb * a.d + n) = float4{y[0], y[1], y[2], y[3]};
+    } else if constexpr (MODE == P32_FC1) {
+        if (valid) {
+            f16x4 hi, lo;
+#pragma unroll
+            for (int i = 0; i < 4; ++i) { f16 h_, l_; split_hilo(gelu_erf(y[i]), h_, l_); hi[i] = h_; lo[i] = l_; }
+            const size_t o = plane_index(gb, n, a.N);
+            *reinterpret_cast<f16x4*>(a.h_out + o) = hi;
+            *reinterpret_cast<f16x4*>(a.h_out_lo + o) = lo;
+        }
+    } else if constexpr (MODE == P32_RESID) {
+        const float b4[4] = {e0[t].x, e0[t].y, e0[t].z, e0[t].w}, x4[4] = {e1[t].x, e1[t].y, e1[t].z, e1[t].w};
+        float xn[4];
+#pragma unroll
+        for (int i = 0; i < 4; ++i) xn[i] = x4[i] + (v[t][i] + b4[i]);
+        if constexpr (SL > 1)
+            d32_resid_tail_gm(xn, gm[t], valid && live_l, bt, rt, n_rt, n, j, gb, tid, a.d, a.x, a.zhi_out, a.zlo_out, a.stat_out,
+                              reinterpret_cast<float (*)[33]>(&red[t][0][0][0]));
+        else
+            d32_resid_tail(xn, valid && live_l, bt, rt, n_rt, n, j, gb, tid, a.d, a.x, a.gamma_next, a.zhi_out, a.zlo_out, a.stat_out,
+                           reinterpret_cast<float (*)[33]>(xs_raw));
+    } else {
+        if (r16) {
+#pragma unroll
+            for (int i = 0; i < 4; ++i) y[i] = (float)(f16)y[i];
+        }
+        if (a.logits && valid && live_l) {
+            float* lo = a.logits + (size_t)gb * a.N + n;
+            if (n + 3 < a.N) {
+                *reinterpret_cast<float2*>(lo) = float2{y[0], y[1]};
+                *reinterpret_cast<float2*>(lo + 2) = float2{y[2], y[3]};
+            } else {
+#pragma unroll
+                for (int i = 0; i < 4; ++i) if (n + i < a.N) lo[i] = y[i];
+            }
+        }
+        if (a.stats) {
+            SoftStat t_{-INFINITY, 0.0f, 0x7fffffff}, u_{-INFINITY, 0.0f, 0x7fffffff};
+            const int blank = rules[0], ts_active = rules[1];
+#pragma unroll
+            for (int i = 0; i < 4; ++i) {
+                const int id = n + i;
+                bool masked = ((masked4[t] >> (8 * i)) & 0xff) != 0 || id >= a.N;
+                masked |= blank && (id == ws_tok || id == eot_tok);
+                masked |= ts_active && (id == nots_tok || (id >= rules[2] && id < rules[3]) || (id >= rules[4] && id < rules[5]));
+                if (!masked) { if (id < tb) stat_merge(t_, y[i], 1.0f, id); else stat_merge(u_, y[i], 1.0f, id); }
+            }
+            float* xr = xs_raw;
+            float* rec = xr + (size_t)(sub * 32 + j) * 6;
+            rec[0] = t_.m; rec[1] = t_.s; rec[2] = __int_as_float(t_.i); rec[3] = u_.m; rec[4] = u_.s; rec[5] = __int_as_float(u_.i);
+            __syncthreads();
+            if (tid < 32 && valid && live_l) {
+                SoftStat T{-INFINITY, 0.0f, 0x7fffffff}, U{-INFINITY, 0.0f, 0x7fffffff};
+#pragma unroll
+                for (int s = 0; s < 8; ++s) {
+                    const float* r_ = xr + (size_t)(s * 32 + tid) * 6;
+                    stat_merge(T, r_[0], r_[1], __float_as_int(r_[2]));
+                    stat_merge(U, r_[3], r_[4], __float_as_int(r_[5]));
+                }
+                float* o = a.stats + ((size_t)gb * kStatBlocks + rt) * 8;
+                *reinterpret_cast<float4*>(o) = float4{T.m, T.s, __int_as_float(T.i), U.m};
+                *reinterpret_cast<float2*>(o + 4) = float2{U.s, __int_as_float(U.i)};
+            }
+        }
+    }
+  }
+    D32_STAMP(6);
+    if constexpr (MODE == P32_Q) { if (a.gate && blockIdx.x == 0 && tid == 0) xattn_gate_acquire(a.gate); }
diff --git a/whisperkit_amd/csrc/decoder.hip b/whisperkit_amd/csrc/decoder.hip
--- a/whisperkit_amd/csrc/decoder.hip
+++ b/whisperkit_amd/csrc/decoder.hip
@@ -734,7 +734,7 @@
         a = base;
         a.N = d; a.K = d; a.Wt = t.o_t; a.zhi = D.zb_hi; a.zlo = D.zb_lo; a.bias = w.o_b; a.gamma_next = w.ln2_g;
         a.zhi_out = D.za_hi; a.zlo_out = D.za_lo; a.stat_out = D.stat; a.prof_kind = KK_DEC_OPROJ;
-        launch_dec32_proj(P32_RESID, a, n_bt, st);
+        launch_dec32_proj(P32_RESID, a, n_bt, st, false, db.k_slice_fold);
         a = base;
         a.N = d; a.K = d; a.Wt = t.cq_t; a.zhi = D.za_hi; a.zlo = D.za_lo; a.fold_g = t.cq_g; a.fold_c = t.cq_c; a.q = D.q; a.prof_kind = KK_DEC_CQ;
         a.gate = db.xabs ? nullptr : db.xattn_gate;
@@ -752,7 +752,7 @@
             if (db.slot_home) { xa.mapped = 1; xa.slot_home = db.slot_home; }
             launch_xabs_qk(xa, n_bt, st);
             launch_xabs_attn(xa, st);
-            launch_xabs_vup(xa, n_bt, st);
+            launch_xabs_vup(xa, n_bt, st, db.k_slice_fold);
         } else {
             at.dbg = debug_buffer() ? debug_buffer() + (size_t)KK_DEC_CROSS_ATTN * 4096 * 8 : nullptr;
             if (db.slot_home) { at.mapped = 1; at.slot_home = db.slot_home; }
@@ -761,7 +761,7 @@
         a = base;
         a.N = d; a.K = d; a.Wt = t.co_t; a.zhi = D.zb_hi; a.zlo = D.zb_lo; a.bias = w.co_b; a.gamma_next = w.ln3_g;
         a.zhi_out = D.za_hi; a.zlo_out = D.za_lo; a.stat_out = D.stat; a.prof_kind = KK_DEC_COPROJ;
-        launch_dec32_proj(P32_RESID, a, n_bt, st);
+        launch_dec32_proj(P32_RESID, a, n_bt, st, false, db.k_slice_fold);
         a = base;
         a.N = 4 * d; a.K = d; a.Wt = t.fc1_t; a.zhi = D.za_hi; a.zlo = D.za_lo; a.fold_g = t.fc1_g; a.fold_c = t.fc1_c; a.h_out = D.h; a.h_out_lo = D.h_lo; a.prof_kind = KK_DEC_FC1;
         launch_dec32_proj(P32_FC1, a, n_bt, st);
@@ -769,7 +769,7 @@
         a.N = d; a.K = 4 * d; a.Wt = t.fc2_t; a.zhi = D.h; a.zlo = D.h_lo; a.bias = w.fc2_b;
         a.gamma_next = (l + 1 < L) ? db.layers_host[l + 1].ln1_g : db.lnf_g;
         a.zhi_out = D.za_hi; a.zlo_out = D.za_lo; a.stat_out = D.stat; a.prof_kind = KK_DEC_FC2;
-        launch_dec32_proj(P32_RESID, a, n_bt, st);
+        launch_dec32_proj(P32_RESID, a, n_bt, st, false, db.k_slice_fold);
     }
     const bool fused = sample && db.fused_greedy;
     P32Args a = base;
diff --git a/whisperkit_amd/csrc/decoder32.hip b/whisperkit_amd/csrc/decoder32.hip
--- a/whisperkit_amd/csrc/decoder32.hip
+++ b/whisperkit_amd/csrc/decoder32.hip
@@ -41,34 +41,38 @@
     d32_fold_kernel<<<(N + 3) / 4, 256, 0, st>>>(W, N, K, gamma, beta, bias, g, c);
 }
 
+__device__ __forceinline__ void d32_resid_tail_gm(const float (&xn)[4], const float4 gm, bool valid, int bt, int rt, int n_rt, int n, int j, int gb, int tid,
+                                                  int d, float* x, f16* zhi, f16* zlo, float2* stat_out, float (*xs)[33]) {
+    if (valid) {
+        *reinterpret_cast<float4*>(x + (size_t)gb * d + n) = float4{xn[0], xn[1], xn[2], xn[3]};
+        const float z[4] = {gm.x * xn[0], gm.y * xn[1], gm.z * xn[2], gm.w * xn[3]};
+        f16x4 hi, lo;
+#pragma unroll
+        for (int i = 0; i < 4; ++i) { f16 h_, l_; split_hilo(z[i], h_, l_); hi[i] = h_; lo[i] = l_; }
+        const size_t o = plane_index(gb, n, d);
+        *reinterpret_cast<f16x4*>(zhi + o) = hi;
+        *reinterpret_cast<f16x4*>(zlo + o) = lo;
+    }
+    const int nl = n & 31;
+#pragma unroll
+    for (int i = 0; i < 4; ++i) xs[nl + i][j] = xn[i];
+    __syncthreads();
+    if (tid < 32) {
+        float s = 0.0f;
+#pragma unroll
+        for (int r = 0; r < 32; ++r) s += xs[r][tid];
+        const float mean = s * (1.0f / 32.0f);
+        float m2 = 0.0f;
+#pragma unroll
+        for (int r = 0; r < 32; ++r) { const float e = xs[r][tid] - mean; m2 = fmaf(e, e, m2); }
+        stat_out[((size_t)bt * n_rt + rt) * 32 + tid] = float2{mean, m2};
+    }
+}
 __device__ __forceinline__ void d32_resid_tail(const float (&xn)[4], bool valid, int bt, int rt, int n_rt, int n, int j, int gb, int tid,
                                                int d, float* x, const float* gamma_next, f16* zhi, f16* zlo, float2* stat_out,
                                                float (*xs)[33]) {
     const float4 gm = *reinterpret_cast<const float4*>(gamma_next + n);
-    if (valid) {
-        *reinterpret_cast<float4*>(x + (size_t)gb * d + n) = float4{xn[0], xn[1], xn[2], xn[3]};
-        const float z[4] = {gm.x * xn[0], gm.y * xn[1], gm.z * xn[2], gm.w * xn[3]};
-        f16x4 hi, lo;
-#pragma unroll
-        for (int i = 0; i < 4; ++i) { f16 h_, l_; split_hilo(z[i], h_, l_); hi[i] = h_; lo[i] = l_; }
-        const size_t o = plane_index(gb, n, d);
-        *reinterpret_cast<f16x4*>(zhi + o) = hi;
-        *reinterpret_cast<f16x4*>(zlo + o) = lo;
-    }
-    const int nl = n & 31;
-#pragma unroll
-    for (int i = 0; i < 4; ++i) xs[nl + i][j] = xn[i];
-    __syncthreads();
-    if (tid < 32) {
-        float s = 0.0f;
-#pragma unroll
-        for (int r = 0; r < 32; ++r) s += xs[r][tid];
-        const float mean = s * (1.0f / 32.0f);
-        float m2 = 0.0f;
-#pragma unroll
-        for (int r = 0; r < 32; ++r) { const float e = xs[r][tid] - mean; m2 = fmaf(e, e, m2); }
-        stat_out[((size_t)bt * n_rt + rt) * 32 + tid] = float2{mean, m2};
-    }
+    d32_resid_tail_gm(xn, gm, valid, bt, rt, n_rt, n, j, gb, tid, d, x, zhi, zlo, stat_out, xs);
 }
 
 template <int K>
@@ -89,305 +93,14 @@
 
 template <int MODE, bool HILO, int TC, bool NTW, int RT>
 __global__ __launch_bounds__(256, 2) void dec32_proj_kernel(const P32Args a) {
-    constexpr bool kMix = MODE == P32_LOGITS_MIXED, kLogits = MODE == P32_LOGITS || kMix;
-    constexpr bool kLN = MODE == P32_QKV || MODE == P32_Q || MODE == P32_FC1 || kLogits;
-    constexpr int kXs = kLogits ? 256 * 6 : 32 * 33;
-    __shared__ float red[RT][4][16][64];
-    __shared__ float st_l[8][32][3];
-    __shared__ float xs_raw[kXs];
-    __shared__ int last_flag;
-    const int tid = threadIdx.x, lane = tid & 63, wave = tid >> 6;
-    const int n_rt = (a.N + 31) >> 5;
-    const int n_rtp = (n_rt + RT - 1) / RT;
-    const int grp8 = blockIdx.x / (8 * a.n_bt), in8 = blockIdx.x % (8 * a.n_bt);
-    const int xw = grp8 * 8 + (in8 & 7), bt = in8 >> 3;
-    if (xw >= n_rtp * a.ks) return;
-    const int rt0 = (xw % n_rtp) * RT, ksi = xw / n_rtp;
-    const int n_mine = min(RT, n_rt - rt0);
-    const int KT = a.K >> 4;
-    const int kt0 = (ksi * 4 + wave) * a.tw;
-    const u32x4* wp[RT];
-#pragma unroll
-    for (int t = 0; t < RT; ++t) wp[t] = reinterpret_cast<const u32x4*>(a.Wt) + ((size_t)min(rt0 + t, n_rt - 1) * KT + kt0) * 64 + lane;
-    const size_t zoff = ((size_t)bt * KT + kt0) * 64 + lane;
-    const u32x4* hp = reinterpret_cast<const u32x4*>(a.zhi) + zoff;
-    const u32x4* lp = HILO ? reinterpret_cast<const u32x4*>(a.zlo) + zoff : nullptr;
-    const int j = tid & 31, sub = tid >> 5;
-    const int gb = bt * 32 + j;
-    const bool valid = gb < a.batch;
-    const int xw_dbg = xw;
-
-#define D32_STAMP(i) do { if (a.dbg && tid == 0 && bt == 0) a.dbg[(size_t)(xw_dbg & 4095) * 8 + (i)] = wall_clock64(); } while (0)
-    D32_STAMP(0);
-    float2 sp[5] = {};
-    if constexpr (kLN) {
-#pragma unroll
-        for (int i = 0; i < 5; ++i) {
-            const int idx = min(sub + 8 * i, a.n_stat - 1);
-            sp[i] = a.stat_in[((size_t)bt * a.n_stat + idx) * 32 + j];
-        }
-    }
-    constexpr bool kLateOperands = RT >= 4;
-    constexpr int NB = RT >= 4 ? 3 : 2;
-    float4 e0[RT], e1[RT];
-    int pos_l = 0, live_l = 0;
-    auto load_operands = [&]() {
-#pragma unroll
-        for (int t = 0; t < RT; ++t) {
-            const int n = min(rt0 + t, n_rt - 1) * 32 + 4 * sub;
-            if constexpr (kLN) {
-                e0[t] = *reinterpret_cast<const float4*>(a.fold_g + n);
-                e1[t] = *reinterpret_cast<const float4*>(a.fold_c + n);
-            } else {
-                e0[t] = *reinterpret_cast<const float4*>(a.bias + n);
-                e1[t] = *reinterpret_cast<const float4*>(a.x + (size_t)gb * a.d + n);
-            }
-        }
-    };
-    if constexpr (!kLateOperands) load_operands();
-    if (valid) { live_l = slot_live(a.seq + gb); if constexpr (MODE == P32_QKV) pos_l = a.seq[gb].token_index; }
-    int rules[6] = {0, 0, 0, 0, 0, 0};
-    unsigned masked4[RT];
-    int tb = 0, ws_tok = 0, eot_tok = 0, nots_tok = 0, r16 = 0;
-#pragma unroll
-    for (int t = 0; t < RT; ++t) masked4[t] = 0xffffffffu;
-    if constexpr (kLogits) {
-        if (a.cfg) r16 = a.cfg->f16_logits;
-        if (a.stats) {
-            if (valid) {
-#pragma unroll
-                for (int i = 0; i < 6; ++i) rules[i] = a.seq[gb].f_rules[i];
-            }
-            const unsigned char* sup_mask = a.sup_mask;
-            if constexpr (kMix) { if (valid) sup_mask += (size_t)seq_class(a.seq[gb].rng_lane) * plan::option_mask_stride(a.N); }
-#pragma unroll
-            for (int t = 0; t < RT; ++t) {
-                const int n = min(rt0 + t, n_rt - 1) * 32 + 4 * sub;
-                if (n + 3 < a.N) masked4[t] = *reinterpret_cast<const unsigned*>(sup_mask + n);
-                else {
-                    masked4[t] = 0;
-#pragma unroll
-                    for (int i = 0; i < 4; ++i) masked4[t] |= (unsigned)(n + i < a.N ? sup_mask[n + i] : 1) << (8 * i);
-                }
-            }
-            tb = a.cfg->time_token_begin; ws_tok = a.cfg->whitespace_token; eot_tok = a.cfg->end_token; nots_tok = a.cfg->no_timestamps_token;
-        }
-    }
-
-    f32x16 acc_h[RT], acc_l[RT];
-#pragma unroll
-    for (int t = 0; t < RT; ++t)
-#pragma unroll
-        for (int r = 0; r < 16; ++r) { acc_h[t][r] = 0.0f; acc_l[t][r] = 0.0f; }
-    auto stats_to_lds = [&]() {
-        if constexpr (kLN) {
-            float cm = sp[0].x, cM2 = sp[0].y;
-            const int mine = sub < a.n_stat ? (a.n_stat - sub + 7) >> 3 : 0;
-            if (mine > 1) chan32_k<1>(cm, cM2, sp[1].x, sp[1].y);
-            if (mine > 2) chan32_k<2>(cm, cM2, sp[2].x, sp[2].y);
-            if (mine > 3) chan32_k<3>(cm, cM2, sp[3].x, sp[3].y);
-            if (mine > 4) chan32_k<4>(cm, cM2, sp[4].x, sp[4].y);
-            st_l[sub][j][0] = 32.0f * (float)mine; st_l[sub][j][1] = cm; st_l[sub][j][2] = cM2;
-        }
-    };
-    {
-        u32x4 w_[NB][RT][TC], h_[NB][TC], l_[NB][HILO ? TC : 1];
-        auto ld = [&](u32x4 (&w)[RT][TC], u32x4 (&h)[TC], u32x4 (&l)[HILO ? TC : 1], int c) {
-#pragma unroll
-            for (int t = 0; t < RT; ++t)
-#pragma unroll
-                for (int i = 0; i < TC; ++i) w[t][i] = NTW ? __builtin_nontemporal_load(wp[t] + (size_t)(c * TC + i) * 64) : wp[t][(size_t)(c * TC + i) * 64];
-#pragma unroll
-            for (int i = 0; i < TC; ++i) h[i] = hp[(size_t)(c * TC + i) * 64];
-            if constexpr (HILO) {
-#pragma unroll
-                for (int i = 0; i < TC; ++i) l[i] = lp[(size_t)(c * TC + i) * 64];
-            }
-        };
-        auto mm = [&](const u32x4 (&w)[RT][TC], const u32x4 (&h)[TC], const u32x4 (&l)[HILO ? TC : 1]) {
-#pragma unroll
-            for (int i = 0; i < TC; ++i) {
-#pragma unroll
-                for (int t = 0; t < RT; ++t) {
-                    const f16x8 wf = __builtin_bit_cast(f16x8, w[t][i]);
-                    acc_h[t] = __builtin_amdgcn_mfma_f32_32x32x16_f16(wf, __builtin_bit_cast(f16x8, h[i]), acc_h[t], 0, 0, 0);
-                    if constexpr (HILO) acc_l[t] = __builtin_amdgcn_mfma_f32_32x32x16_f16(wf, __builtin_bit_cast(f16x8, l[i]), acc_l[t], 0, 0, 0);
-                }
-            }
-        };
-        const int nch = a.tw / TC;
-#pragma unroll
-        for (int u = 0; u + 1 < NB; ++u)
-            if (u < nch) ld(w_[u], h_[u], l_[u], u);
-        D32_STAMP(1);
-#pragma unroll 1
-        for (int c = 0; c < nch; c += NB) {
-#pragma unroll
-            for (int u = 0; u < NB; ++u) {
-                constexpr int kAhead = NB - 1;
-                if (c + u + kAhead < nch) ld(w_[(u + kAhead) % NB], h_[(u + kAhead) % NB], l_[(u + kAhead) % NB], c + u + kAhead);
-                __builtin_amdgcn_sched_barrier(0);
-                if (c + u < nch) mm(w_[u], h_[u], l_[u]);
-                if (u == 0 && c == 0) D32_STAMP(2);
-            }
-        }
-    }
-    if constexpr (kLateOperands) load_operands();
-    stats_to_lds();
-    D32_STAMP(3);
-#pragma unroll
-    for (int t = 0; t < RT; ++t)
-#pragma unroll
-        for (int r = 0; r < 16; ++r) red[t][wave][r][lane] = HILO ? fmaf(acc_l[t][r], 1.0f / 2048.0f, acc_h[t][r]) : acc_h[t][r];
-    __syncthreads();
-    D32_STAMP(4);
-    float v[RT][4];
-#pragma unroll
-    for (int t = 0; t < RT; ++t)
-#pragma unroll
-        for (int i = 0; i < 4; ++i) v[t][i] = ((red[t][0][4 * wave + i][lane] + red[t][1][4 * wave + i][lane]) + red[t][2][4 * wave + i][lane]) + red[t][3][4 * wave + i][lane];
-
-    if (a.ks > 1) {
-        float* base = a.part + (((size_t)bt * n_rt + rt0) * a.ks) * 1024 + tid * 4;
-#pragma unroll
-        for (int t = 0; t < RT; ++t) {
-            if (t < n_mine) {
-                const f32x4 pv4 = {v[t][0], v[t][1], v[t][2], v[t][3]};
-                float* mine = base + ((size_t)t * a.ks + ksi) * 1024;
-                asm volatile("global_store_dwordx4 %0, %1, off sc1\n\ts_nop 1" ::"v"(mine), "v"(pv4) : "memory");
-            }
-        }
-        asm volatile("s_waitcnt vmcnt(0)" ::: "memory");
-        __syncthreads();
-        if (tid == 0) {
-            int* cnt = a.ticket + bt * n_rt + rt0;
-            const int t = __hip_atomic_fetch_add(cnt, 1, __ATOMIC_RELAXED, __HIP_MEMORY_SCOPE_AGENT);
-            const int last = (t == a.ks - 1);
-            if (last) __hip_atomic_store(cnt, 0, __ATOMIC_RELAXED, __HIP_MEMORY_SCOPE_AGENT);
-            last_flag = last;
-        }
-        __syncthreads();
-        if (!last_flag) {
-            if constexpr (MODE == P32_Q) { if (a.gate && blockIdx.x == 0 && tid == 0) xattn_gate_acquire(a.gate); }
-            return;
-        }
-        float pv[RT][8][4];
-#pragma unroll
-        for (int t = 0; t < RT; ++t)
-#pragma unroll
-            for (int s = 0; s < 8; ++s) {
-                const float* p = base + ((size_t)(t < n_mine ? t : 0) * a.ks + (s < a.ks ? s : 0)) * 1024;
-#pragma unroll
-                for (int i = 0; i < 4; ++i) pv[t][s][i] = __hip_atomic_load(p + i, __ATOMIC_RELAXED, __HIP_MEMORY_SCOPE_AGENT);
-            }
-#pragma unroll
-        for (int t = 0; t < RT; ++t)
-#pragma unroll
-            for (int i = 0; i < 4; ++i) {
-                float x_ = pv[t][0][i];
-#pragma unroll
-                for (int s = 1; s < 8; ++s) x_ += (s < a.ks) ? pv[t][s][i] : 0.0f;
-                v[t][i] = x_;
-            }
-    }
-
-    D32_STAMP(5);
-    float mu = 0.0f, rstd = 0.0f;
-    if constexpr (kLN) {
-        float cn = 0.0f, cm = 0.0f, cM2 = 0.0f;
-#pragma unroll
-        for (int s = 0; s < 8; ++s) chan_merge(cn, cm, cM2, st_l[s][j][0], st_l[s][j][1], st_l[s][j][2]);
-        mu = cm; rstd = rsqrtf(cM2 / (float)a.d + 1e-5f);
-    }
-#pragma unroll
-  for (int t = 0; t < RT; ++t) {
-    if (t >= n_mine) break;
-    if constexpr (MODE == P32_RESID || kLogits) { if (t > 0) __syncthreads(); }
-    const int rt = rt0 + t, n = rt * 32 + 4 * sub;
-    float y[4];
-    if constexpr (kLN) {
-        const float g4[4] = {e0[t].x, e0[t].y, e0[t].z, e0[t].w}, c4[4] = {e1[t].x, e1[t].y, e1[t].z, e1[t].w};
-#pragma unroll
-        for (int i = 0; i < 4; ++i) y[i] = fmaf(rstd, v[t][i] - mu * g4[i], c4[i]);
-    }
-    if constexpr (MODE == P32_QKV) {
-        if (valid && live_l) {
-            const int d = a.d;
-            if (n < d) *reinterpret_cast<float4*>(a.q + (size_t)gb * d + n) = float4{y[0], y[1], y[2], y[3]};
-            else {
-                int c = n - d;
-                f16* dst = a.self_k;
-                if (c >= d) { c -= d; dst = a.self_v; }
-                const int pos = min(max(pos_l, 0), kMaxTok - 1);
-                *reinterpret_cast<f16x4*>(dst + (((size_t)gb * a.n_head + (c >> 6)) * kMaxTok + pos) * kHeadDim + (c & 63)) =
-                    f16x4{(f16)y[0], (f16)y[1], (f16)y[2], (f16)y[3]};
-            }
-        }
-    } else if constexpr (MODE == P32_Q) {
-        if (valid && live_l) *reinterpret_cast<float4*>(a.q + (size_t)gb * a.d + n) = float4{y[0], y[1], y[2], y[3]};
-    } else if constexpr (MODE == P32_FC1) {
-        if (valid) {
-            f16x4 hi, lo;
-#pragma unroll
-            for (int i = 0; i < 4; ++i) { f16 h_, l_; split_hilo(gelu_erf(y[i]), h_, l_); hi[i] = h_; lo[i] = l_; }
-            const size_t o = plane_index(gb, n, a.N);
-            *reinterpret_cast<f16x4*>(a.h_out + o) = hi;
-            *reinterpret_cast<f16x4*>(a.h_out_lo + o) = lo;
-        }
-    } else if constexpr (MODE == P32_RESID) {
-        const float b4[4] = {e0[t].x, e0[t].y, e0[t].z, e0[t].w}, x4[4] = {e1[t].x, e1[t].y, e1[t].z, e1[t].w};
-        float xn[4];
-#pragma unroll
-        for (int i = 0; i < 4; ++i) xn[i] = x4[i] + (v[t][i] + b4[i]);
-        d32_resid_tail(xn, valid && live_l, bt, rt, n_rt, n, j, gb, tid, a.d, a.x, a.gamma_next, a.zhi_out, a.zlo_out, a.stat_out,
-                       reinterpret_cast<float (*)[33]>(xs_raw));
-    } else {
-        if (r16) {
-#pragma unroll
-            for (int i = 0; i < 4; ++i) y[i] = (float)(f16)y[i];
-        }
-        if (a.logits && valid && live_l) {
-            float* lo = a.logits + (size_t)gb * a.N + n;
-            if (n + 3 < a.N) {
-                *reinterpret_cast<float2*>(lo) = float2{y[0], y[1]};
-                *reinterpret_cast<float2*>(lo + 2) = float2{y[2], y[3]};
-            } else {
-#pragma unroll
-                for (int i = 0; i < 4; ++i) if (n + i < a.N) lo[i] = y[i];
-            }
-        }
-        if (a.stats) {
-            SoftStat t_{-INFINITY, 0.0f, 0x7fffffff}, u_{-INFINITY, 0.0f, 0x7fffffff};
-            const int blank = rules[0], ts_active = rules[1];
-#pragma unroll
-            for (int i = 0; i < 4; ++i) {
-                const int id = n + i;
-                bool masked = ((masked4[t] >> (8 * i)) & 0xff) != 0 || id >= a.N;
-                masked |= blank && (id == ws_tok || id == eot_tok);
-                masked |= ts_active && (id == nots_tok || (id >= rules[2] && id < rules[3]) || (id >= rules[4] && id < rules[5]));
-                if (!masked) { if (id < tb) stat_merge(t_, y[i], 1.0f, id); else stat_merge(u_, y[i], 1.0f, id); }
-            }
-            float* xr = xs_raw;
-            float* rec = xr + (size_t)(sub * 32 + j) * 6;
-            rec[0] = t_.m; rec[1] = t_.s; rec[2] = __int_as_float(t_.i); rec[3] = u_.m; rec[4] = u_.s; rec[5] = __int_as_float(u_.i);
-            __syncthreads();
-            if (tid < 32 && valid && live_l) {
-                SoftStat T{-INFINITY, 0.0f, 0x7fffffff}, U{-INFINITY, 0.0f, 0x7fffffff};
-#pragma unroll
-                for (int s = 0; s < 8; ++s) {
-                    const float* r_ = xr + (size_t)(s * 32 + tid) * 6;
-                    stat_merge(T, r_[0], r_[1], __float_as_int(r_[2]));
-                    stat_merge(U, r_[3], r_[4], __float_as_int(r_[5]));
-                }
-                float* o = a.stats + ((size_t)gb * kStatBlocks + rt) * 8;
-                *reinterpret_cast<float4*>(o) = float4{T.m, T.s, __int_as_float(T.i), U.m};
-                *reinterpret_cast<float2*>(o + 4) = float2{U.s, __int_as_float(U.i)};
-            }
-        }
-    }
-  }
-    D32_STAMP(6);
-    if constexpr (MODE == P32_Q) { if (a.gate && blockIdx.x == 0 && tid == 0) xattn_gate_acquire(a.gate); }
+    constexpr int SL = 1;
+#include "dec32_proj_body.inc"
+}
+template <int TC, int RT>
+__global__ __launch_bounds__(256, 2) void dec32_proj_fold_kernel(const P32Args a) {
+    constexpr int MODE = P32_RESID, SL = 4;
+    constexpr bool HILO = true, NTW = false;
+#include "dec32_proj_body.inc"
 }
 
 
@@ -420,6 +133,25 @@
 template <int MODE, bool HILO>
 static void launch_planned(const P32Args& a, const plan::Dec32Plan& p, hipStream_t st) {
     const dim3 grid(p.grid);
+    if constexpr (MODE == P32_RESID && HILO) {
+        if (p.sl > 1) {
+#define D32_FOLD(TC_, RT_) do { dec32_proj_fold_kernel<TC_, RT_><<<grid, 256, 0, st>>>(a); return; } while (0)
+            if (p.rt == 4) D32_FOLD(1, 4);
+            if (p.rt >= 2) {
+                if (p.tc == 4) D32_FOLD(4, 2);
+                if (p.tc == 2) D32_FOLD(2, 2);
+                D32_FOLD(1, 2);
+            }
+            switch (p.tc) {
+                case 5: D32_FOLD(5, 1);
+                case 4: D32_FOLD(4, 1);
+                case 3: D32_FOLD(3, 1);
+                case 2: D32_FOLD(2, 1);
+                default: D32_FOLD(1, 1);
+            }
+#undef D32_FOLD
+        }
+    }
 #define D32_GO(TC_, RT_) do { \
         if (p.ntw) dec32_proj_kernel<MODE, HILO, TC_, true, RT_><<<grid, 256, 0, st>>>(a); \
         else dec32_proj_kernel<MODE, HILO, TC_, false, RT_><<<grid, 256, 0, st>>>(a); \
@@ -443,12 +175,13 @@
 }
 
 unsigned long long* debug_buffer();
-void launch_dec32_proj(int mode, const P32Args& a_in, int n_bt, hipStream_t st, bool mixed) {
+void launch_dec32_proj(int mode, const P32Args& a_in, int n_bt, hipStream_t st, bool mixed, int fold) {
     using namespace knob;
     P32Args a = a_in;
     a.dbg = (debug_buffer() && a.prof_kind >= 0) ? debug_buffer() + (size_t)a.prof_kind * 4096 * 8 : nullptr;
     const plan::Dec32Knobs k{once<WH_D32_KS_RESID>(), once<WH_D32_KS_FC2>(), once<WH_D32_KS_Q>(), once<WH_D32_KS_WIDE>(), once<WH_D32_TILE_KB>(), once<WH_D32_TC>(),
-                             once<WH_D32_TC_BT>(), once<WH_D32_RT2_TC>(), once<WH_D32_NTW>(), once<WH_D32_RT_BT>(), once<WH_D32_RT4_BT>(), once<WH_D32_RT4_MODES>()};
+                             once<WH_D32_TC_BT>(), once<WH_D32_RT2_TC>(), once<WH_D32_NTW>(), once<WH_D32_RT_BT>(), once<WH_D32_RT4_BT>(), once<WH_D32_RT4_MODES>(),
+                             (mode == P32_RESID && a.zlo != nullptr) ? fold : 0};
     const plan::Dec32Plan p = plan::dec32_plan(mode, a.N, a.K, n_bt, k);
     a.ks = p.ks; a.tw = p.tw; a.rt = p.rt; a.n_bt = n_bt;
     ProfScope ps_(a.prof_kind, st);
diff --git a/whisperkit_amd/csrc/internal.h b/whisperkit_amd/csrc/internal.h
--- a/whisperkit_amd/csrc/internal.h
+++ b/whisperkit_amd/csrc/internal.h
@@ -132,6 +132,7 @@
     int* beam_fin_len = nullptr;
     long long beam_rank_launches = 0, beam_loop_syncs = 0;
     int fallback_compaction = 0;
+    int k_slice_folding = 0;
     int32_t *slot_home_dev = nullptr, *slot_home_host = nullptr;
     bool pass_mapped = false; int pass_spw = 1;
     wh::Xabs xabs_pass{};
diff --git a/whisperkit_amd/csrc/kernels.h b/whisperkit_amd/csrc/kernels.h
--- a/whisperkit_amd/csrc/kernels.h
+++ b/whisperkit_amd/csrc/kernels.h
@@ -195,6 +195,7 @@
     const int* slot_home;
     int mixed;
     int owner_slots;
+    int k_slice_fold;
 };
 constexpr int kStatBlocks = 1792;
 constexpr int kMaxVocab = 52224;
@@ -237,7 +238,7 @@
     int prof_kind;
     unsigned long long* dbg;
 };
-void launch_dec32_proj(int mode, const P32Args& a, int n_bt, hipStream_t st, bool mixed = false);
+void launch_dec32_proj(int mode, const P32Args& a, int n_bt, hipStream_t st, bool mixed = false, int fold = 0);
 void launch_dec32_embed(const f16* emb, const float* pos, const SeqState* seq, int batch, int d, int n_vocab, int n_bt, float* x,
                         const float* gamma_next, f16* zhi, f16* zlo, float2* stat, hipStream_t st);
 void dec32_tile_weights(const f16* W, int N, int K, f16* out, hipStream_t st);
@@ -283,7 +284,7 @@
 void xabs_tile_wk(const f16* Wk, int d, int H, f16* out, hipStream_t st);
 void launch_xabs_qk(const XabsArgs& a, int n_bt, hipStream_t st);
 void launch_xabs_attn(const XabsArgs& a, hipStream_t st);
-void launch_xabs_vup(const XabsArgs& a, int n_bt, hipStream_t st);
+void launch_xabs_vup(const XabsArgs& a, int n_bt, hipStream_t st, int fold = 0);
 
 void launch_decoder_step(const DecodeBuffers& db, const SamplerCfg* cfg_dev, const int* suppress_dev, bool sample, hipStream_t st);
 void launch_rules_init(const SamplerCfg* cfg_dev, SeqState* seq, int batch, hipStream_t st, bool mixed = false);
diff --git a/whisperkit_amd/csrc/launch_plan.h b/whisperkit_amd/csrc/launch_plan.h
--- a/whisperkit_amd/csrc/launch_plan.h
+++ b/whisperkit_amd/csrc/launch_plan.h
@@ -64,8 +64,8 @@
     return LN_SCALAR;
 }
 
-struct Dec32Knobs { int ks_resid, ks_fc2, ks_q, ks_wide, tile_kb, tc, tc_bt, rt2_tc, ntw, rt_bt, rt4_bt, rt4_modes; };
-struct Dec32Plan { int ks, tw, rt, tc; bool ntw; unsigned grid; };
+struct Dec32Knobs { int ks_resid, ks_fc2, ks_q, ks_wide, tile_kb, tc, tc_bt, rt2_tc, ntw, rt_bt, rt4_bt, rt4_modes; int fold; };
+struct Dec32Plan { int ks, tw, rt, tc; bool ntw; unsigned grid; int sl; };
 inline Dec32Plan dec32_plan(int mode, int N, int K, int n_bt, const Dec32Knobs& k) {
     Dec32Plan p{};
     const bool fc2 = mode == P32_RESID && K > N;
@@ -94,7 +94,12 @@
         p.tc = (p.tw % 5 == 0 && tc_cap >= 5) ? 5 : (p.tw % 4 == 0 && tc_cap >= 4) ? 4 : (p.tw % 3 == 0 && tc_cap >= 3) ? 3 : (p.tw % 2 == 0) ? 2 : 1;
     }
     p.ntw = k.ntw < 0 ? n_bt == 1 : k.ntw != 0;
-    const int nx = ((n_rt + p.rt - 1) / p.rt) * p.ks;
+    p.sl = 1;
+    if (mode == P32_RESID && p.ks > 1 && k.fold > 0) {
+        p.sl = p.ks;
+        p.ntw = false;
+    }
+    const int nx = ((n_rt + p.rt - 1) / p.rt) * (p.ks / p.sl);
     p.grid = (unsigned)(((nx + 7) / 8) * 8 * n_bt);
     return p;
 }
@@ -122,11 +127,12 @@
     const int n_grp = (b1 + 3) / 4 * n_split;
     return (unsigned)((n_grp + 7) / 8 * 32);
 }
-struct XabsVupPlan { int ks; unsigned grid; };
-inline XabsVupPlan xabs_vup_plan(int d, int n_head, int n_bt) {
+struct XabsVupPlan { int ks; unsigned grid; int sl; };
+inline XabsVupPlan xabs_vup_plan(int d, int n_head, int n_bt, int fold = 0) {
     const int ks = d == 384 ? 3 : 4;
-    const int nx = n_head * ks;
-    return {ks, (unsigned)(((nx + 7) / 8) * 8 * n_bt)};
+    const int sl = fold > 0 ? ks : 1;
+    const int nx = n_head * (ks / sl);
+    return {ks, (unsigned)(((nx + 7) / 8) * 8 * n_bt), sl};
 }
 
 constexpr int kCompactLadder[] = {32, 64, 128};
diff --git a/whisperkit_amd/csrc/xabs.hip b/whisperkit_amd/csrc/xabs.hip
--- a/whisperkit_amd/csrc/xabs.hip
+++ b/whisperkit_amd/csrc/xabs.hip
@@ -359,7 +359,7 @@
 }
 
 
-template <int S, int TW>
+template <int S, int TW, bool FOLD = false>
 __global__ __launch_bounds__(256, 1) void xabs_vup_kernel(const XabsArgs a, int ks, int n_bt) {
     __shared__ float red[4][2][16][64];
     __shared__ int last_flag;
@@ -367,8 +367,8 @@
     const int d = a.d, H = a.n_head, KT = d >> 4;
     const int grp8 = blockIdx.x / (8 * n_bt), in8 = blockIdx.x % (8 * n_bt);
     const int xw = grp8 * 8 + (in8 & 7), bt = in8 >> 3;
-    if (xw >= H * ks) return;
-    const int h = xw % H, ksi = xw / H;
+    if (xw >= H * (FOLD ? 1 : ks)) return;
+    const int h = xw % H, ksi = FOLD ? 0 : xw / H;
     const int kt0 = (ksi * 4 + wave) * TW;
     const int j = lane & 31, hl = lane >> 5;
     const int gbl = min(bt * 32 + j, a.max_batch - 1);
@@ -409,6 +409,9 @@
         for (int s = 0; s < S; ++s) wn[s] *= inv;
     }
     f32x16 acc_h[2] = {{0}, {0}}, acc_l[2] = {{0}, {0}};
+    float xf[2][4] = {};
+#pragma unroll 1
+  for (int sl = 0; sl < (FOLD ? ks : 1); ++sl) {
 #pragma unroll
     for (int i = 0; i < TW; ++i) {
         float z[8] = {0, 0, 0, 0, 0, 0, 0, 0};
@@ -426,6 +429,44 @@
         acc_h[1] = __builtin_amdgcn_mfma_f32_32x32x16_f16(wf1, zh, acc_h[1], 0, 0, 0);
         acc_l[1] = __builtin_amdgcn_mfma_f32_32x32x16_f16(wf1, zl, acc_l[1], 0, 0, 0);
     }
+    if constexpr (FOLD) {
+        if (sl + 1 == ks) break;
+        const u32x4* wq = wp + (size_t)(sl + 1) * 4 * TW * 64;
+        const float* pq = pp + (size_t)(sl + 1) * 4 * TW * 2 * a.max_batch * 8;
+#pragma unroll
+        for (int i = 0; i < TW; ++i) { w0[i] = __builtin_nontemporal_load(wq + (size_t)i * 64); w1[i] = __builtin_nontemporal_load(wq + ((size_t)KT + i) * 64); }
+#pragma unroll
+        for (int i = 0; i < TW; ++i)
+#pragma unroll
+            for (int s = 0; s < S; ++s) {
+                const float* q = pq + (size_t)s * sstride + (size_t)i * 2 * a.max_batch * 8;
+                p0[i][s] = *reinterpret_cast<const f32x4*>(q);
+                p1[i][s] = *reinterpret_cast<const f32x4*>(q + 4);
+            }
+#pragma unroll
+        for (int t = 0; t < 2; ++t)
+#pragma unroll
+            for (int r = 0; r < 16; ++r) {
+                red[wave][t][r][lane] = fmaf(acc_l[t][r], 1.0f / 2048.0f, acc_h[t][r]);
+                acc_h[t][r] = 0.0f; acc_l[t][r] = 0.0f;
+            }
+        __syncthreads();
+#pragma unroll
+        for (int t = 0; t < 2; ++t)
+#pragma unroll
+            for (int i = 0; i < 4; ++i) {
+                const float vs = ((red[0][t][4 * wave + i][lane] + red[1][t][4 * wave + i][lane]) + red[2][t][4 * wave + i][lane]) + red[3][t][4 * wave + i][lane];
+                xf[t][i] = sl == 0 ? vs : xf[t][i] + vs;
+            }
+        __syncthreads();
+#pragma unroll
+        for (int i = 0; i < TW; ++i) {
+            asm volatile("" : "+v"(w0[i]), "+v"(w1[i]));
+#pragma unroll
+            for (int s = 0; s < S; ++s) asm volatile("" : "+v"(p0[i][s]), "+v"(p1[i][s]));
+        }
+    }
+  }
 #pragma unroll
     for (int t = 0; t < 2; ++t)
 #pragma unroll
@@ -437,7 +478,13 @@
     for (int t = 0; t < 2; ++t)
 #pragma unroll
         for (int i = 0; i < 4; ++i) v[t][i] = ((red[0][t][4 * wave + i][lane] + red[1][t][4 * wave + i][lane]) + red[2][t][4 * wave + i][lane]) + red[3][t][4 * wave + i][lane];
-    if (ks > 1) {
+    if constexpr (FOLD) {
+#pragma unroll
+        for (int t = 0; t < 2; ++t)
+#pragma unroll
+            for (int i = 0; i < 4; ++i) v[t][i] = xf[t][i] + v[t][i];
+    }
+    if (!FOLD && ks > 1) {
         float* base = a.kpart + (((size_t)bt * H + h) * ks) * 2048 + tid * 4;
 #pragma unroll
         for (int t = 0; t < 2; ++t) {
@@ -542,17 +589,18 @@
     }
 }
 
-void launch_xabs_vup(const XabsArgs& a, int n_bt, hipStream_t st) {
+void launch_xabs_vup(const XabsArgs& a, int n_bt, hipStream_t st, int fold) {
     ProfScope ps_(KK_DEC_XVUP, st);
-    const plan::XabsVupPlan p = plan::xabs_vup_plan(a.d, a.n_head, n_bt);
+    const plan::XabsVupPlan p = plan::xabs_vup_plan(a.d, a.n_head, n_bt, fold);
     const int ks = p.ks;
     const unsigned grid = p.grid;
-#define XVUP(S_) do { switch (a.d / 256) { \
-        case 1: xabs_vup_kernel<S_, 2><<<grid, 256, 0, st>>>(a, ks, n_bt); break; \
-        case 2: xabs_vup_kernel<S_, 2><<<grid, 256, 0, st>>>(a, ks, n_bt); break; \
-        case 3: xabs_vup_kernel<S_, 3><<<grid, 256, 0, st>>>(a, ks, n_bt); break; \
-        case 4: xabs_vup_kernel<S_, 4><<<grid, 256, 0, st>>>(a, ks, n_bt); break; \
-        default: xabs_vup_kernel<S_, 5><<<grid, 256, 0, st>>>(a, ks, n_bt); break; } } while (0)
+#define XVUP_F(S_, F_) do { switch (a.d / 256) { \
+        case 1: xabs_vup_kernel<S_, 2, F_><<<grid, 256, 0, st>>>(a, ks, n_bt); break; \
+        case 2: xabs_vup_kernel<S_, 2, F_><<<grid, 256, 0, st>>>(a, ks, n_bt); break; \
+        case 3: xabs_vup_kernel<S_, 3, F_><<<grid, 256, 0, st>>>(a, ks, n_bt); break; \
+        case 4: xabs_vup_kernel<S_, 4, F_><<<grid, 256, 0, st>>>(a, ks, n_bt); break; \
+        default: xabs_vup_kernel<S_, 5, F_><<<grid, 256, 0, st>>>(a, ks, n_bt); break; } } while (0)
+#define XVUP(S_) do { if (p.sl > 1) XVUP_F(S_, true); else XVUP_F(S_, false); } while (0)
     switch (a.n_split) {
         case 1: XVUP(1); break;
         case 2: XVUP(2); break;
@@ -560,6 +608,7 @@
         default: XVUP(4); break;
     }
 #undef XVUP
-}
-
-}
+#undef XVUP_F
+}
+
+}
```

New measurement: 2599. 1.7% lower.
